# sean-lo/OptimalMatrixCompletion.jl

Measured on AMD Instinct MI355X. Metric: B&B node-relaxations/sec, 100x100 k=1, higher is better.
Workload: dtype f64

## Files before the change

### include/omc.h

```cpp
#ifndef OMC_H
#define OMC_H

#include <stdint.h>

#ifdef __cplusplus
extern "C" {
#endif

#define OMC_VERSION 100

#define OMC_OPTIMAL 0
#define OMC_SLOW_PROGRESS 1
#define OMC_TIME_LIMIT 2
#define OMC_INFEASIBLE 3

#define OMC_CUT_LINEAR 0
#define OMC_CUT_LINEAR2 1
#define OMC_CUT_LINEAR3 2
#define OMC_DIR_LEFT 0
#define OMC_DIR_MIDDLE 1
#define OMC_DIR_RIGHT 2
#define OMC_DIR_INNER_LEFT 3
#define OMC_DIR_INNER_RIGHT 4
#define OMC_SMALLEST_1_EIGVEC 1
// ... 56 lines not shown
                    double* Y, double* U, double* X, double* Theta, double* lambda_min, double* breakpoint_x,
                    double* solve_time);

int omc_relax_stage(omc_instance* h, int B, const omc_relax_params* params, int cut_type, const int* L,
                    const double* cut_x, const double* cut_Uhat, const int8_t* cut_dir, const double* U_lower,
                    const double* U_upper);
int omc_set_node_rho_scales(omc_instance* h, int B, const double* rho_scale);
int omc_relax_solve(omc_instance* h);
int omc_state_pool_create(omc_instance* h, int capacity);
int omc_state_pool_reserve_shor(omc_instance* h, int64_t nq_max);
int omc_relax_set_warm(omc_instance* h, int B, const int* load_from, const int* save_to);
int omc_shor_warm_compat(int64_t n_parent, const int64_t* parent_idx, int64_t n_soc_parent, const int64_t* parent_soc, int64_t n_child,
                         const int64_t* child_idx, int64_t n_soc_child, const int64_t* child_soc);
int omc_last_shor_warm_stats(omc_instance* h, int64_t out[4]);
int omc_state_pool_fetch_shor(omc_instance* h, int entry, int64_t* nq, double* X, double* Theta, double* V);
int omc_relax_submit(omc_instance* h);
int omc_relax_fetch_done(omc_instance* h, int max_nodes, int* node_ids, double* objective, double* dual_bound, int* status, int* iters,
                         double* U, double* lambda_min, double* breakpoint_x, double* Y, int* n_out);
int omc_relax_hold(omc_instance* h, int on);
int omc_relax_reserve(omc_instance* h, int extra_nodes, int max_cuts);
int omc_relax_append(omc_instance* h, int B, const int* L, const double* cut_x, const double* cut_Uhat, const int8_t* cut_dir,
                     const int* load_from, const int* save_to);
int omc_relax_poll(omc_instance* h, int* running, int* nodes_done, int* nodes_total);
int omc_relax_wait(omc_instance* h);
int omc_relax_fetch(omc_instance* h, double* objective, double* dual_bound, int* status, int* iters, double* Y,
                    double* U, double* X, double* Theta, double* lambda_min, double* breakpoint_x,
                    double* solve_time);

int omc_relax_stage_shor(omc_instance* h, int B, const omc_relax_params* params, int cut_type, const int* L,
                         const double* cut_x, const double* cut_Uhat, const int8_t* cut_dir, const double* U_lower,
                         const double* U_upper, const int64_t* n_shor, const int64_t* shor_idx, const int64_t* n_soc,
                         const int64_t* soc_idx);
int omc_relax_fetch_shor(omc_instance* h, double* W );
int omc_set_shor_keep_V(omc_instance* h, int keep);
int omc_relax_fetch_shor_V(omc_instance* h, double* V);
int omc_relax_batch_shor(omc_instance* h, int B, const omc_relax_params* params, int cut_type, const int* L,
                         const double* cut_x, const double* cut_Uhat, const int8_t* cut_dir, const double* U_lower,
                         const double* U_upper, const int64_t* n_shor, const int64_t* shor_idx, const int64_t* n_soc,
                         const int64_t* soc_idx, double* objective, double* dual_bound, int* status, int* iters, double* Y,
                         double* U, double* X, double* Theta, double* W, double* lambda_min, double* breakpoint_x,
                         double* solve_time);
int omc_set_shor_penalties(omc_instance* h, double rho, double r4, double r5);
int omc_relax_reserve_shor(omc_instance* h, int64_t nq_max, int extra_lists);
int omc_relax_append_shor(omc_instance* h, int B, const int* L, const double* cut_x, const double* cut_Uhat, const int8_t* cut_dir,
                          const int64_t* n_shor, const int64_t* shor_idx, const int64_t* n_soc, const int64_t* soc_idx,
                          const int* load_from, const int* save_to);
int omc_relax_fetch_done_shor(omc_instance* h, int n_ids, const int* node_ids, double* X, double* W, double* Theta);

int omc_relax_keep_certificates(omc_instance* h, int on);
int omc_relax_fetch_certificate(omc_instance* h, int n_ids, const int* node_ids, double* Lam, double* lam, int* R, double* Q, int* r,
                                double* Psi3, double* bound);
int omc_certificate_plan(int n, int k, int nnz, int max_cuts, int nonstandard_box_rows, int64_t* out);
int omc_dual_bound_batch(omc_instance* h, int B, int cut_type, int reference_quirk_q1, const int* L, const double* cut_x,
                         const double* cut_Uhat, const int8_t* cut_dir, const double* U_lower, const double* U_upper, const double* Lam,
                         const double* lam, const double* Psi3, double* Q_out, int* r_out, double* bound);

int omc_relax_keep_shor_certificates(omc_instance* h, int on);
int omc_relax_fetch_shor_certificate(omc_instance* h, int n_ids, const int* node_ids, double* scale, double* bound, double* lam, int* R, double* Q,
                                     int* r, double* Psi3, double* Gam, double* zeta, double* xi, double* Xbar, int* nq, int64_t* nq_stride);
int omc_shor_certificate_plan(int n, int m, int k, int64_t nq_stride, int max_cuts, int nonstandard_box_rows, int64_t* out);

int omc_shor_dual_bound_batch(omc_instance* h, int B, int cut_type, int reference_quirk_q1, const int* L, const double* cut_x,
                              const double* cut_Uhat, const int8_t* cut_dir, const double* U_lower, const double* U_upper, const int64_t* n_shor,
                              const int64_t* shor_idx, const int64_t* n_soc, const int64_t* soc_idx, int sanitise, int64_t nq_stride,
                              const double* scale, const double* lam, const double* Psi3, const double* Gam, const double* zeta, const double* xi,
                              const double* Xbar, double* bound, double* defects, double* terms);
int omc_shor_dual_bound_plan(int n, int m, int k, int B, int64_t nq_stride, int max_cuts, int nonstandard_box_rows, int sanitise, int64_t* out);
int omc_last_shor_dual_bound_ms(omc_instance* h, double* ms);

int omc_shor_index_build(omc_instance* h, int where, int64_t nq, const int64_t* shor_idx, int64_t n_soc, const int64_t* soc_idx, int64_t* counts,
                         double* r4, uint64_t* hash, int* mi, int* kid, int* cptr, int* cent, int* v1ptr, int* v1ent, int* v2ptr, int* v2ent,
                         int* slackrow, uint8_t* eclass, uint8_t* ctype);
int omc_shor_index_plan(int n, int m, int64_t nq, int64_t* out);
int omc_last_shor_index_stats(omc_instance* h, double* out);

int omc_altmin_batch(omc_instance* h, int B, int cut_type, int reference_quirk_q1, const int* L,
                     const double* cut_x, const double* cut_Uhat, const int8_t* cut_dir, const double* U_initial,
                     double eps, int max_iters, double time_limit, double* U, double* V, int* converged,
                     int* n_iters, double* objectives, double* solve_time);

int omc_altmin_master_objectives(omc_instance* h, int B, double* objective);
int omc_altmin_plan(int n, int m, int k, int max_cuts, int nolds, int64_t* out);

int omc_evaluate_objective(omc_instance* h, int B, const double* X, double* objective);

int omc_separation_batch(omc_instance* h, int B, int breakpoints, const double* Y, const double* U,
                         double* eigvals, double* x, int* feasible);

int omc_round_Y_batch(omc_instance* h, int B, const double* Y, double* U_rounded);
int omc_left_singular_batch(omc_instance* h, int B, const double* X, double* U_out);

int omc_psd_project_batch(omc_instance* h, int B, int N, const double* M, double lo, double hi, int algo,
                          const double* V0, double* P, double* evals, double* V);
int omc_column_prox_batch(omc_instance* h, int B, int mode, int algo, const double* Y, const double* alpha_old, const double* rho_f,
                          const double* s0, double* alpha, double* s, double* objcol, double* c0col, int* nfact);
int omc_row_project_batch(omc_instance* h, int B, int R, int Rmax, int which, const double* G, const double* c, const double* lam0,
                          double* lam, int* overflow);
int omc_colprox_plan(int n, int cmax, int block_min, int64_t* out);
int omc_last_cone_multi_stats(omc_instance* h, int64_t* out);
int omc_plain_multi_plan(int n, int plain_multi_min, int64_t* out);
double omc_plain_multi_tau(void);
int omc_last_plain_multi_stats(omc_instance* h, int64_t* out);
int omc_cone_multi_budget(int interval_max);
#define OMC_HARVEST_NONE 0
#define OMC_HARVEST_SYNC 1
#define OMC_HARVEST_ASYNC 2
int omc_harvest_plan(int nlive, int nfin, int pending, int check_index, int async_min_live);

int omc_shor_count(omc_instance* h, int n_classes, const int* num_entries_present, int64_t* count_per_class);
int omc_shor_indexes(omc_instance* h, int n_classes, const int* num_entries_present, int64_t capacity, int64_t* out,
                     int64_t* count);
int omc_violated_shor_minors(omc_instance* h, const double* X, int n_classes, const int* num_entries_present,
                             int64_t n_existing, const int64_t* existing, int n_minors, double* scores,
                             int64_t* minors, int* n_out);
int omc_shor_last_stats(omc_instance* h, double* ms, int64_t* candidates);
int omc_shor_last_select_stats(omc_instance* h, int64_t out[4]);

#define OMC_COMM_ID_BYTES 128
int omc_comm_unique_id(void* id_out);
int omc_comm_init(omc_instance* h, int rank, int world_size, const void* id);
int omc_allreduce_bounds(omc_instance* h, double* ub, double* lb, int* owner);
int omc_bcast_incumbent(omc_instance* h, int root, double* X);
int omc_allgather_records(omc_instance* h, const double* rows, int cnt, int width, double* out, int out_capacity_rows, int* counts);
int omc_comm_destroy(omc_instance* h);

#define OMC_KERNEL_COLPROX 0
#define OMC_KERNEL_CONE 1
#define OMC_KERNEL_GLOBAL 2
#define OMC_KERNEL_CHECK 3
#define OMC_KERNEL_SETUP 4
#define OMC_KERNEL_SMALL 5
#define OMC_KERNEL_ACCEL 6
#define OMC_KERNEL_CONESUB 7
#define OMC_KERNEL_CHECK_COL 8
#define OMC_KERNEL_CHECK_BUILD 9
#define OMC_KERNEL_HARVEST 10
#define OMC_KERNEL_SHOR_BIGCONE 11
#define OMC_KERNEL_SHOR_MINORS 12
#define OMC_KERNEL_SHOR_COLS 13
#define OMC_KERNEL_NCLASS 14
int omc_last_solver_info(omc_instance* h, double* info);
#define OMC_RES_CONE_SUB 0
#define OMC_RES_CONE_SUB_CERT 1
#define OMC_RES_CONE_SUB_SEP 2
#define OMC_RES_GLOBAL 3
#define OMC_RES_SMALL 4
#define OMC_RES_COLPROX_PAIR 5
#define OMC_RES_COLPROX_WIDE 6
#define OMC_RES_COLPROX 7
#define OMC_RES_CONE_WS 8
#define OMC_RES_CONE 9
#define OMC_RES_N 10
int omc_kernel_residency(omc_instance* h, int* out);
int omc_last_subspace_stats(omc_instance* h, int64_t* out);
int omc_last_shor_subspace_stats(omc_instance* h, int64_t* out);
int omc_tuning_set(omc_instance* h, const char* name, const char* value);
int omc_tuning_reload_env(omc_instance* h);
int omc_debug_stamps(omc_instance* h, double* out32);
int omc_debug_diag(omc_instance* h, double* out);
int omc_debug_aa(omc_instance* h, int* accepted, int* rejected);
int omc_debug_residuals(omc_instance* h, double* rp, double* rd);
int omc_last_kernel_stats(omc_instance* h, int64_t* launches , double* ms ,
                          int64_t* units );
#define OMC_HOST_CHECK_WAIT 0
#define OMC_HOST_CHECK_SCAN 1
#define OMC_HOST_LIST 2
#define OMC_HOST_EVENT_DRAIN 3
#define OMC_HOST_HARVEST_FLAGS 4
#define OMC_HOST_HARVEST_ENQUEUE 5
#define OMC_HOST_HARVEST_WAIT 6
#define OMC_HOST_HARVEST_BOOK 7
#define OMC_HOST_SETUP_ENQUEUE 8
#define OMC_HOST_CHECK_TOTAL 9
#define OMC_HOST_HARVEST_TOTAL 10
#define OMC_HOST_ASYNC_HARVESTS 11
#define OMC_HOST_QUIET_INTERVALS 12
#define OMC_HOST_BODY_RECORDS 13
#define OMC_HOST_BODY_WAITS 14
#define OMC_HOST_NPHASE 15
int omc_last_host_phases(omc_instance* h, double* ms , int64_t* count );

#ifdef __cplusplus
}
#endif
#endif
```

### optimalmatrixcompletion.jl_amd/_lib.py

```python
from __future__ import annotations

import ctypes as C
import os

import numpy as np

_HERE = os.path.dirname(os.path.abspath(__file__))
LIB_PATH = os.environ.get("OMC_AMD_LIB") or os.path.join(_HERE, "lib", "libomc_hip.so")

EXPORTS = [
    "omc_relax_params_default", "omc_last_error", "omc_version", "omc_device_count", "omc_instance_create",
    "omc_instance_create_bits", "omc_instance_destroy", "omc_relax_batch", "omc_relax_stage", "omc_relax_solve",
    "omc_relax_fetch", "omc_relax_submit", "omc_relax_poll", "omc_relax_wait", "omc_altmin_batch", "omc_evaluate_objective", "omc_separation_batch", "omc_round_Y_batch",
    "omc_last_kernel_stats", "omc_last_host_phases", "omc_kernel_residency", "omc_last_solver_info", "omc_last_subspace_stats", "omc_set_node_rho_scales", "omc_left_singular_batch", "omc_psd_project_batch", "omc_column_prox_batch", "omc_row_project_batch", "omc_colprox_plan", "omc_last_cone_multi_stats", "omc_cone_multi_budget", "omc_plain_multi_plan", "omc_plain_multi_tau", "omc_last_plain_multi_stats", "omc_harvest_plan", "omc_relax_reserve", "omc_relax_append", "omc_relax_fetch_done", "omc_relax_hold", "omc_debug_stamps", "omc_tuning_set", "omc_tuning_reload_env", "omc_debug_residuals", "omc_debug_diag", "omc_debug_aa",
    "omc_shor_count", "omc_shor_indexes", "omc_violated_shor_minors", "omc_shor_last_stats", "omc_shor_last_select_stats",
    "omc_relax_stage_shor", "omc_relax_fetch_shor", "omc_relax_batch_shor", "omc_set_shor_penalties", "omc_set_shor_keep_V", "omc_relax_fetch_shor_V", "omc_last_shor_subspace_stats", "omc_state_pool_create", "omc_relax_set_warm",
    "omc_state_pool_reserve_shor", "omc_shor_warm_compat", "omc_last_shor_warm_stats", "omc_state_pool_fetch_shor",
    "omc_relax_reserve_shor", "omc_relax_append_shor", "omc_relax_fetch_done_shor",
    "omc_relax_keep_certificates", "omc_relax_fetch_certificate", "omc_certificate_plan", "omc_dual_bound_batch",
    "omc_relax_keep_shor_certificates", "omc_relax_fetch_shor_certificate", "omc_shor_certificate_plan",
    "omc_shor_dual_bound_batch", "omc_shor_dual_bound_plan", "omc_last_shor_dual_bound_ms",
    "omc_shor_index_build", "omc_shor_index_plan", "omc_last_shor_index_stats",
    "omc_altmin_master_objectives", "omc_altmin_plan", "omc_comm_unique_id", "omc_comm_init", "omc_allreduce_bounds", "omc_bcast_incumbent", "omc_allgather_records", "omc_comm_destroy",
]


class RelaxParams(C.Structure):
    _fields_ = [("eps_gap", C.c_double), ("eps_feas", C.c_double), ("max_iters", C.c_int), ("check_every", C.c_int),
                ("rho_scale", C.c_double), ("rho_f_ratio", C.c_double), ("relax", C.c_double), ("time_limit", C.c_double),
                ("reference_quirk_q1", C.c_int), ("breakpoints", C.c_int), ("stall_checks", C.c_int), ("bump_max", C.c_int), ("bump_ratio", C.c_double),
                ("bump_factor", C.c_double), ("bump_after", C.c_int), ("bump_window", C.c_int), ("slots", C.c_int),
                ("accel", C.c_int), ("aa_mem", C.c_int), ("aa_every", C.c_int), ("aa_start", C.c_int), ("aa_reg", C.c_double), ("aa_safeguard", C.c_double), ("first_wins", C.c_int),
                ("early_stop_after", C.c_int), ("early_stop_factor", C.c_double)]


class OmcError(RuntimeError):
    def __init__(self, code, msg):
        super().__init__(f"libomc_hip error {code}: {msg}")
        self.code = code


_lib = None


def load():
    global _lib
    if _lib is not None:
        return _lib
    if not os.path.exists(LIB_PATH):
        raise OmcError(-100, f"{LIB_PATH} not found: build it first (__graft_entry__.build()); there is no CPU fallback")
    lib = C.CDLL(LIB_PATH)
    dp = C.POINTER(C.c_double); ip = C.POINTER(C.c_int); vp = C.c_void_p
    lib.omc_last_error.restype = C.c_char_p
    lib.omc_version.restype = C.c_int
    lib.omc_device_count.restype = C.c_int
    lib.omc_relax_params_default.argtypes = [C.POINTER(RelaxParams)]
    lib.omc_instance_create.argtypes = [C.c_int, C.c_int, C.c_int, vp, vp, C.c_double, C.c_int, C.POINTER(vp)]
    lib.omc_instance_create_bits.argtypes = [C.c_int, C.c_int, C.c_int, vp, vp, C.c_double, C.c_int, C.POINTER(vp)]
    lib.omc_instance_destroy.argtypes = [vp]
    lib.omc_instance_destroy.restype = None
    lib.omc_relax_batch.argtypes = [vp, C.c_int, C.POINTER(RelaxParams), C.c_int] + [vp] * 17
    lib.omc_relax_stage.argtypes = [vp, C.c_int, C.POINTER(RelaxParams), C.c_int] + [vp] * 6
    lib.omc_relax_solve.argtypes = [vp]
    lib.omc_relax_stage_shor.argtypes = [vp, C.c_int, C.POINTER(RelaxParams), C.c_int] + [vp] * 10
    lib.omc_relax_fetch_shor.argtypes = [vp, vp]
    lib.omc_relax_batch_shor.argtypes = [vp, C.c_int, C.POINTER(RelaxParams), C.c_int] + [vp] * 22
    lib.omc_set_shor_penalties.argtypes = [vp, C.c_double, C.c_double, C.c_double]
    lib.omc_set_shor_keep_V.argtypes = [vp, C.c_int]
    lib.omc_relax_fetch_shor_V.argtypes = [vp, vp]
    lib.omc_last_shor_subspace_stats.argtypes = [vp, vp]
    lib.omc_state_pool_create.argtypes = [vp, C.c_int]
    lib.omc_relax_set_warm.argtypes = [vp, C.c_int, vp, vp]
    lib.omc_state_pool_reserve_shor.argtypes = [vp, C.c_int64]
    lib.omc_shor_warm_compat.argtypes = [C.c_int64, vp, C.c_int64, vp, C.c_int64, vp, C.c_int64, vp]
    lib.omc_last_shor_warm_stats.argtypes = [vp, vp]
    lib.omc_state_pool_fetch_shor.argtypes = [vp, C.c_int, vp, vp, vp, vp]
    lib.omc_relax_submit.argtypes = [vp]
    lib.omc_relax_poll.argtypes = [vp, vp, vp, vp]
    lib.omc_relax_wait.argtypes = [vp]
    lib.omc_relax_fetch.argtypes = [vp] + [vp] * 11
    lib.omc_altmin_batch.argtypes = [vp, C.c_int, C.c_int, C.c_int, vp, vp, vp, vp, vp, C.c_double, C.c_int, C.c_double,
                                     vp, vp, vp, vp, vp, vp]
    lib.omc_evaluate_objective.argtypes = [vp, C.c_int, vp, vp]
    lib.omc_separation_batch.argtypes = [vp, C.c_int, C.c_int, vp, vp, vp, vp, vp]
    lib.omc_round_Y_batch.argtypes = [vp, C.c_int, vp, vp]
    lib.omc_last_kernel_stats.argtypes = [vp, vp, vp, vp]
    lib.omc_last_solver_info.argtypes = [vp, vp]
    if hasattr(lib, "omc_last_host_phases"):
        lib.omc_last_host_phases.argtypes = [vp, vp, vp]
    if hasattr(lib, "omc_kernel_residency"):
        lib.omc_kernel_residency.argtypes = [vp, vp]
    lib.omc_last_subspace_stats.argtypes = [vp, vp]
    lib.omc_set_node_rho_scales.argtypes = [vp, C.c_int, vp]
    lib.omc_debug_stamps.argtypes = [vp, vp]
    lib.omc_left_singular_batch.argtypes = [vp, C.c_int, vp, vp]
    lib.omc_psd_project_batch.argtypes = [vp, C.c_int, C.c_int, vp, C.c_double, C.c_double, C.c_int, vp, vp, vp, vp]
    if hasattr(lib, "omc_column_prox_batch"):
        lib.omc_column_prox_batch.argtypes = [vp, C.c_int, C.c_int, C.c_int] + [vp] * 9
        lib.omc_colprox_plan.argtypes = [C.c_int, C.c_int, C.c_int, vp]
    if hasattr(lib, "omc_row_project_batch"):
        lib.omc_row_project_batch.argtypes = [vp, C.c_int, C.c_int, C.c_int, C.c_int] + [vp] * 5
    lib.omc_last_cone_multi_stats.argtypes = [vp, vp]
    lib.omc_cone_multi_budget.argtypes = [C.c_int]
    if hasattr(lib, "omc_plain_multi_plan"):
        lib.omc_plain_multi_plan.argtypes = [C.c_int, C.c_int, vp]
        lib.omc_plain_multi_tau.argtypes = []
        lib.omc_plain_multi_tau.restype = C.c_double
        lib.omc_last_plain_multi_stats.argtypes = [vp, vp]
    if hasattr(lib, "omc_harvest_plan"):
        lib.omc_harvest_plan.argtypes = [C.c_int] * 5
    lib.omc_relax_reserve.argtypes = [vp, C.c_int, C.c_int]
    lib.omc_relax_hold.argtypes = [vp, C.c_int]
    lib.omc_relax_fetch_done.argtypes = [vp, C.c_int, vp, vp, vp, vp, vp, vp, vp, vp, vp, vp]
    lib.omc_relax_append.argtypes = [vp, C.c_int, vp, vp, vp, vp, vp, vp]
    lib.omc_relax_reserve_shor.argtypes = [vp, C.c_int64, C.c_int]
    lib.omc_relax_append_shor.argtypes = [vp, C.c_int] + [vp] * 10
    lib.omc_relax_fetch_done_shor.argtypes = [vp, C.c_int, vp, vp, vp, vp]
    if hasattr(lib, "omc_relax_keep_certificates"):
        lib.omc_relax_keep_certificates.argtypes = [vp, C.c_int]
        lib.omc_relax_fetch_certificate.argtypes = [vp, C.c_int] + [vp] * 8
        lib.omc_certificate_plan.argtypes = [C.c_int] * 5 + [vp]
        lib.omc_dual_bound_batch.argtypes = [vp, C.c_int, C.c_int, C.c_int] + [vp] * 12
    if hasattr(lib, "omc_relax_keep_shor_certificates"):
        lib.omc_relax_keep_shor_certificates.argtypes = [vp, C.c_int]
        lib.omc_relax_fetch_shor_certificate.argtypes = [vp, C.c_int] + [vp] * 14
        lib.omc_shor_certificate_plan.argtypes = [C.c_int, C.c_int, C.c_int, C.c_int64, C.c_int, C.c_int, vp]
    if hasattr(lib, "omc_shor_dual_bound_batch"):
        lib.omc_shor_dual_bound_batch.argtypes = [vp, C.c_int, C.c_int, C.c_int] + [vp] * 10 + [C.c_int, C.c_int64] + [vp] * 10
        lib.omc_shor_dual_bound_plan.argtypes = [C.c_int] * 4 + [C.c_int64, C.c_int, C.c_int, C.c_int, vp]
        lib.omc_last_shor_dual_bound_ms.argtypes = [vp, vp]
    if hasattr(lib, "omc_shor_index_build"):
        lib.omc_shor_index_build.argtypes = [vp, C.c_int, C.c_int64, vp, C.c_int64] + [vp] * 15
        lib.omc_shor_index_plan.argtypes = [C.c_int, C.c_int, C.c_int64, vp]
        lib.omc_last_shor_index_stats.argtypes = [vp, vp]
    lib.omc_tuning_set.argtypes = [vp, C.c_char_p, C.c_char_p]
    lib.omc_tuning_reload_env.argtypes = [vp]
    lib.omc_debug_residuals.argtypes = [vp, vp, vp]
    lib.omc_debug_diag.argtypes = [vp, vp]
    lib.omc_debug_aa.argtypes = [vp, vp, vp]
    lib.omc_shor_count.argtypes = [vp, C.c_int, vp, vp]
    lib.omc_shor_indexes.argtypes = [vp, C.c_int, vp, C.c_int64, vp, vp]
    lib.omc_violated_shor_minors.argtypes = [vp, vp, C.c_int, vp, C.c_int64, vp, C.c_int, vp, vp, vp]
    lib.omc_shor_last_stats.argtypes = [vp, vp, vp]
    lib.omc_shor_last_select_stats.argtypes = [vp, vp]
    lib.omc_altmin_master_objectives.argtypes = [vp, C.c_int, vp]
    lib.omc_altmin_plan.argtypes = [C.c_int, C.c_int, C.c_int, C.c_int, C.c_int, vp]
    lib.omc_comm_unique_id.argtypes = [vp]
    lib.omc_comm_init.argtypes = [vp, C.c_int, C.c_int, vp]
    lib.omc_allreduce_bounds.argtypes = [vp, vp, vp, vp]
    lib.omc_bcast_incumbent.argtypes = [vp, C.c_int, vp]
    lib.omc_allgather_records.argtypes = [vp, vp, C.c_int, C.c_int, vp, C.c_int, vp]
    lib.omc_comm_destroy.argtypes = [vp]
    _lib = lib
    return lib


def check(rc):
    if rc != 0:
        raise OmcError(rc, load().omc_last_error().decode("utf-8", "replace"))


def ptr(a):
    return None if a is None else a.ctypes.data_as(C.c_void_p)


def f64(a, order="F"):
    return np.require(np.asarray(a, dtype=np.float64), requirements=["ALIGNED"] + (["F_CONTIGUOUS"] if order == "F" else ["C_CONTIGUOUS"]))
```

### optimalmatrixcompletion.jl_amd/api.py

```python
from __future__ import annotations

import atexit
import weakref
import ctypes as C

import numpy as np

from . import _lib, certificate
from ._lib import RelaxParams, OmcError

CUT_TYPES = {"linear": 0, "linear2": 1, "linear3": 2}
DIR_CODES = {"left": 0, "middle": 1, "right": 2, "inner_left": 3, "inner_right": 4}
BREAKPOINTS = {"smallest_1_eigvec": 1, "smallest_2_eigvec": 2}
STATUS_NAMES = {0: "OPTIMAL", 1: "SLOW_PROGRESS", 2: "TIME_LIMIT", 3: "INFEASIBLE"}
KERNEL_CLASSES = ["colprox", "cone", "global", "check", "setup", "small", "accel", "cone_sub", "check_col", "check_build", "harvest",
                  "shor_bigcone", "shor_minors", "shor_cols"]
HOST_PHASES = ["check_wait", "check_scan", "list", "event_drain", "harvest_flags", "harvest_enqueue", "harvest_wait", "harvest_book",
               "setup_enqueue", "check_total", "harvest_total", "async_harvests", "quiet_intervals", "body_records", "body_waits"]
HOST_BODY_COUNTS = ("body_records", "body_waits")
RESIDENCY_KERNELS = ["k_cone_sub<0>", "k_cone_sub<1>", "k_cone_sub<2>", "k_global", "k_small", "k_colprox_pair", "k_colprox_wide", "k_colprox",
                     "k_cone_ws", "k_cone"]


def default_params(**kw) -> RelaxParams:
# ... 264 lines not shown

    def reserve_shor(self, nq_max, extra_lists):
        _lib.check(self._lib.omc_relax_reserve_shor(self._h, int(nq_max), int(extra_lists)))
        self._reserved_nq = int(nq_max)

    def append_shor(self, nodes, shor_info, disjunctive_cuts_type="linear", load_from=None, save_to=None):
        n, k = self.n, self.k
        if len(shor_info) != len(nodes):
            raise ValueError("one Shor_info per node")
        L, cx, cU, cd = _pack_cuts(nodes, n, k, disjunctive_cuts_type)
        lf = None if load_from is None else np.ascontiguousarray(np.asarray(load_from, dtype=np.int32))
        sv = None if save_to is None else np.ascontiguousarray(np.asarray(save_to, dtype=np.int32))
        if (lf is not None and lf.shape != (len(nodes),)) or (sv is not None and sv.shape != (len(nodes),)):
            raise ValueError("load_from / save_to must hold one pool index per node")
        nsh, nso, shi, soi = _pack_shor(shor_info)
        _lib.check(self._lib.omc_relax_append_shor(self._h, len(nodes), _lib.ptr(L), _lib.ptr(cx), _lib.ptr(cU), _lib.ptr(cd), _lib.ptr(nsh),
                                                   _lib.ptr(shi), _lib.ptr(nso), _lib.ptr(soi), _lib.ptr(lf), _lib.ptr(sv)))
        self._B += len(nodes)

    def fetch_done_shor(self, ids, want_W=False, want_Theta=False):
        n, m = self.n, self.m
        idv = np.ascontiguousarray(np.asarray(list(ids), dtype=np.int32))
        c = len(idv)
        X = np.zeros((max(c, 1), n * m)); W = np.zeros((max(c, 1), n * m)) if want_W else None; Th = np.zeros((max(c, 1), m * m)) if want_Theta else None
        _lib.check(self._lib.omc_relax_fetch_done_shor(self._h, c, _lib.ptr(idv), _lib.ptr(X), _lib.ptr(W), _lib.ptr(Th)))
        out = []
        for i in range(c):
            d = dict(node=int(idv[i]), X=X[i].reshape((n, m), order="F"))
            if want_W:
                d["W"] = W[i].reshape((n, m), order="F")
            if want_Theta:
                d["Theta"] = Th[i].reshape((m, m), order="F")
            out.append(d)
        return out

    def hold(self, on=True):
        _lib.check(self._lib.omc_relax_hold(self._h, 1 if on else 0))

    def fetch_done(self, max_nodes=4096, want_Y=False):
        n, k = self.n, self.k
        key = (int(max_nodes), bool(want_Y))
        if getattr(self, "_fd_key", None) != key:
            self._fd_key = key
            self._fd = (np.zeros(max_nodes, np.int32), np.zeros(max_nodes), np.zeros(max_nodes), np.zeros(max_nodes, np.int32), np.zeros(max_nodes, np.int32),
                        np.zeros((max_nodes, n * k)), np.zeros((max_nodes, 2)), np.zeros((max_nodes, n)), np.zeros(1, np.int32),
                        np.zeros((max_nodes, n * n)) if want_Y else None)
        ids, obj, lb, st, it, U, ev, bx, cnt, Y = self._fd
        _lib.check(self._lib.omc_relax_fetch_done(self._h, int(max_nodes), _lib.ptr(ids), _lib.ptr(obj), _lib.ptr(lb), _lib.ptr(st), _lib.ptr(it),
                                                  _lib.ptr(U), _lib.ptr(ev), _lib.ptr(bx), _lib.ptr(Y), _lib.ptr(cnt)))
        out = []
        for i in range(int(cnt[0])):
            d = dict(node=int(ids[i]), objective=float(obj[i]), dual_bound=float(lb[i]), status_code=int(st[i]), termination_status=STATUS_NAMES[int(st[i])],
                     feasible=int(st[i]) != 3, iters=int(it[i]), U=U[i].reshape((n, k), order="F").copy(), lambda_min=ev[i].copy(), breakpoint_vec=bx[i].copy())
            if want_Y:
                d["Y"] = Y[i].reshape((n, n), order="F").copy()
            out.append(d)
        return out

    def solve(self):
        _lib.check(self._lib.omc_relax_solve(self._h))

    def submit(self):
        _lib.check(self._lib.omc_relax_submit(self._h))

    def poll(self):
        r = np.zeros(3, np.int32)
        _lib.check(self._lib.omc_relax_poll(self._h, _lib.ptr(r[0:1]), _lib.ptr(r[1:2]), _lib.ptr(r[2:3])))
        return dict(running=bool(r[0]), nodes_done=int(r[1]), nodes_total=int(r[2]))

    def wait(self):
        _lib.check(self._lib.omc_relax_wait(self._h))

    def fetch(self, want_Y=True, want_X=True, want_Theta=False):
        B, n, m, k = self._B, self.n, self.m, self.k
        obj = np.zeros(B); lb = np.zeros(B); st = np.zeros(B, np.int32); it = np.zeros(B, np.int32)
        Y = np.zeros((B, n * n)) if want_Y else None
        U = np.zeros((B, n * k))
        X = np.zeros((B, n * m)) if want_X else None
        Th = np.zeros((B, m * m)) if want_Theta else None
        lmin = np.zeros((B, 2)); bx = np.zeros((B, n)); tm = np.zeros(B)
        _lib.check(self._lib.omc_relax_fetch(self._h, _lib.ptr(obj), _lib.ptr(lb), _lib.ptr(st), _lib.ptr(it), _lib.ptr(Y),
                                             _lib.ptr(U), _lib.ptr(X), _lib.ptr(Th), _lib.ptr(lmin), _lib.ptr(bx), _lib.ptr(tm)))
        out = []
        for b in range(B):
            r = {
                "objective": float(obj[b]), "dual_bound": float(lb[b]), "termination_status": STATUS_NAMES[int(st[b])],
                "status_code": int(st[b]), "feasible": int(st[b]) != 3, "iters": int(it[b]), "solve_time": float(tm[b]),
                "U": U[b].reshape((n, k), order="F"), "lambda_min": lmin[b].copy(), "breakpoint_vec": bx[b].copy(),
            }
            if want_Y: r["Y"] = Y[b].reshape((n, n), order="F")
            if want_X: r["X"] = X[b].reshape((n, m), order="F")
            if want_Theta: r["Theta"] = Th[b].reshape((m, m), order="F")
            out.append(r)
        return out

    def matrix_completion_SDP_relaxation(self, nodes, disjunctive_cuts_type="linear", params=None, U_lower=None, U_upper=None,
                                         want_Y=True, want_X=True, want_Theta=False, rho_scales=None, add_Shor_valid_inequalities=False,
                                         shor_info=None, shor_penalties=None, want_V=False, load_from=None, save_to=None):
        if add_Shor_valid_inequalities:
            if shor_info is None:
                raise ValueError("add_Shor_valid_inequalities = true needs node.Shor_info (OMC.jl:1508)")
            self.stage_shor(nodes, shor_info, disjunctive_cuts_type, params, U_lower, U_upper, shor_penalties, keep_V=(want_V and self.k == 1),
                            load_from=load_from, save_to=save_to)
            self.solve()
            out = self.fetch(want_Y, want_X, want_Theta)
            for r, Wb in zip(out, self.fetch_shor()):
                r["W"] = Wb
            if want_V and self.k == 1:
                for r, Vb, (mi, _) in zip(out, self.fetch_shor_V(), shor_info):
                    r["V"] = Vb[:len(np.asarray(mi).reshape(-1, 4))]
            elif want_V:
                for r, (mi, _) in zip(out, shor_info):
                    r.update(shor_rank_k_extension(self.k, r["X"], r["W"], mi))
            return out
        self.stage(nodes, disjunctive_cuts_type, params, U_lower, U_upper, rho_scales, load_from, save_to)
        self.solve()
        return self.fetch(want_Y, want_X, want_Theta)

    def kernel_stats(self):
        nc = len(KERNEL_CLASSES); la = np.zeros(nc, np.int64); ms = np.zeros(nc); un = np.zeros(nc, np.int64)
        _lib.check(self._lib.omc_last_kernel_stats(self._h, _lib.ptr(la), _lib.ptr(ms), _lib.ptr(un)))
        return {KERNEL_CLASSES[i]: dict(launches=int(la[i]), ms=float(ms[i]), units=int(un[i])) for i in range(nc)}

    def host_phases(self):
        if not hasattr(self._lib, "omc_last_host_phases"):
            raise OmcError(-100, "this build of the library has no omc_last_host_phases")
        ms = np.zeros(len(HOST_PHASES)); cnt = np.zeros(len(HOST_PHASES), np.int64)
        _lib.check(self._lib.omc_last_host_phases(self._h, _lib.ptr(ms), _lib.ptr(cnt)))
        return {HOST_PHASES[i]: dict(ms=float(ms[i]), count=int(cnt[i])) for i in range(len(HOST_PHASES)) if HOST_PHASES[i] not in HOST_BODY_COUNTS}

    def event_counts(self):
        if not hasattr(self._lib, "omc_last_host_phases"):
            raise OmcError(-100, "this build of the library has no omc_last_host_phases")
        ms = np.zeros(len(HOST_PHASES)); cnt = np.zeros(len(HOST_PHASES), np.int64)
        _lib.check(self._lib.omc_last_host_phases(self._h, _lib.ptr(ms), _lib.ptr(cnt)))
        return {name[len("body_"):]: int(cnt[HOST_PHASES.index(name)]) for name in HOST_BODY_COUNTS}

    def subspace_stats(self):
        out = np.zeros(8, np.int64)
        _lib.check(self._lib.omc_last_subspace_stats(self._h, _lib.ptr(out)))
        return dict(calls=int(out[0]), power_steps=int(out[1]), fallbacks=int(out[2]), seeds=int(out[3]), fail_positive=int(out[4]),
                    fail_steps=int(out[5]), fail_cholesky=int(out[6]), ritz_passes=int(out[7]))

    def shor_subspace_stats(self):
        out = np.zeros(8, np.int64)
        _lib.check(self._lib.omc_last_shor_subspace_stats(self._h, _lib.ptr(out)))
        return dict(calls=int(out[0]), power_steps=int(out[1]), fallbacks=int(out[2]), seeds=int(out[3]), fail_positive=int(out[4]),
                    fail_steps=int(out[5]), fail_cholesky=int(out[6]), ritz_passes=int(out[7]))

    def kernel_residency(self):
        out = np.zeros(len(RESIDENCY_KERNELS), np.int32)
        _lib.check(self._lib.omc_kernel_residency(self._h, _lib.ptr(out)))
        return {nm: int(v) for nm, v in zip(RESIDENCY_KERNELS, out)}

    def solver_info(self):
        info = np.zeros(8)
        _lib.check(self._lib.omc_last_solver_info(self._h, _lib.ptr(info)))
        return dict(solve_seconds=info[0], jacobi_sweeps=int(info[1]), rho=info[2], r_max=int(info[3]), cone_lds=bool(info[4]),
                    global_lds=bool(info[5]), small_lds=bool(info[6]), R_max=int(info[7]))

    def keep_certificates(self, on=True):
        _lib.check(self._lib.omc_relax_keep_certificates(self._h, 1 if on else 0))

    def certificate_plan(self, max_cuts=0, nonstandard_box_rows=0):
        return certificate_plan(self.n, self.k, int(self.indices.sum()), max_cuts, nonstandard_box_rows)

    def _support(self):
        cols, rows = np.nonzero(self.indices.T)
        return rows, cols

    def fetch_certificate(self, ids):
        n, m, k = self.n, self.m, self.k
        idv = np.ascontiguousarray(np.asarray(list(ids), dtype=np.int32))
        c = len(idv)
        info = self.solver_info()
        Rmax, rmax = max(info["R_max"], 1), max(info["r_max"], 1)
        rows, cols = self._support()
        nnz = rows.size
        ps = (rmax + k) ** 2
        Lam = np.zeros((max(c, 1), max(nnz, 1))); lam = np.zeros((max(c, 1), Rmax)); R = np.zeros(max(c, 1), np.int32)
        Q = np.zeros((max(c, 1), n * rmax)); r = np.zeros(max(c, 1), np.int32); Psi = np.zeros((max(c, 1), ps)); bd = np.zeros(max(c, 1))
        if nnz:
            Lam = np.zeros((max(c, 1), nnz))
        _lib.check(self._lib.omc_relax_fetch_certificate(self._h, c, _lib.ptr(idv), _lib.ptr(Lam), _lib.ptr(lam), _lib.ptr(R), _lib.ptr(Q),
                                                         _lib.ptr(r), _lib.ptr(Psi), _lib.ptr(bd)))
        out = []
        for i in range(c):
            ri = int(r[i]); N3 = ri + k
            dense = np.zeros((n, m)); dense[rows, cols] = Lam[i, :nnz]
            out.append(certificate.Certificate(Lam=dense, lam=lam[i, :int(R[i])].copy(), Q=Q[i, :n * ri].reshape((n, ri), order="F").copy(),
                                               Psi3=Psi[i, :N3 * N3].reshape((N3, N3), order="F").copy(), bound=float(bd[i])))
        return out

    def keep_shor_certificates(self, on=True):
        _lib.check(self._lib.omc_relax_keep_shor_certificates(self._h, 1 if on else 0))

    def shor_certificate_plan(self, nq_stride, max_cuts=0, nonstandard_box_rows=0):
        return shor_certificate_plan(self.n, self.m, self.k, nq_stride, max_cuts, nonstandard_box_rows)

    def fetch_shor_certificate(self, ids):
        n, m, k = self.n, self.m, self.k
        idv = np.ascontiguousarray(np.asarray(list(ids), dtype=np.int32))
        c = len(idv); c1 = max(c, 1)
        stride = np.zeros(1, np.int64)
        _lib.check(self._lib.omc_relax_fetch_shor_certificate(self._h, 0, None, *([None] * 12), _lib.ptr(stride)))
        ns = int(stride[0])
        info = self.solver_info()
        Rmax, rmax = max(info["R_max"], 1), max(info["r_max"], 1)
        ps = (rmax + k) ** 2
        sc = np.zeros(c1); bd = np.zeros(c1); lam = np.zeros((c1, Rmax)); R = np.zeros(c1, np.int32); Q = np.zeros((c1, n * rmax)); r = np.zeros(c1, np.int32)
        Psi = np.zeros((c1, ps)); Gam = np.zeros((c1, 15 * max(ns, 1))); zeta = np.zeros((c1, m)); xi = np.zeros((c1, n * m)); Xb = np.zeros((c1, n * m))
        nq = np.zeros(c1, np.int32)
        _lib.check(self._lib.omc_relax_fetch_shor_certificate(self._h, c, _lib.ptr(idv), _lib.ptr(sc), _lib.ptr(bd), _lib.ptr(lam), _lib.ptr(R), _lib.ptr(Q),
                                                              _lib.ptr(r), _lib.ptr(Psi), _lib.ptr(Gam) if ns else None, _lib.ptr(zeta), _lib.ptr(xi), _lib.ptr(Xb),
                                                              _lib.ptr(nq), None))
        out = []
        for i in range(c):
            ri = int(r[i]); N3 = ri + k
            G = certificate.unpack_gam(Gam[i, :15 * ns].reshape(15, ns), int(nq[i])) if ns else np.zeros((0, 5, 5))
            out.append(certificate.ShorCertificate(scale=float(sc[i]), lam=lam[i, :int(R[i])].copy(), Q=Q[i, :n * ri].reshape((n, ri), order="F").copy(),
                                                   Psi3=Psi[i, :N3 * N3].reshape((N3, N3), order="F").copy(), Gam=G, zeta=zeta[i].copy(),
                                                   xi=xi[i].reshape((n, m), order="F").copy(), Xbar=Xb[i].reshape((n, m), order="F").copy(),
                                                   bound=float(bd[i])))
        return out

    def _bounds_flat(self, B, U_lower, U_upper):
        lo = hi = None
        if U_lower is not None:
            lo = np.ascontiguousarray(np.stack([np.asfortranarray(np.asarray(u, float)).ravel(order="F") for u in U_lower]))
        if U_upper is not None:
            hi = np.ascontiguousarray(np.stack([np.asfortranarray(np.asarray(u, float)).ravel(order="F") for u in U_upper]))
        for a in (lo, hi):
            if a is not None and a.shape != (B, self.n * self.k):
                raise ValueError("U_lower / U_upper: one (n, k) matrix per node")
        return lo, hi

    def row_basis(self, nodes, disjunctive_cuts_type="linear", U_lower=None, U_upper=None, reference_quirk_q1=True):
        n, k, B = self.n, self.k, len(nodes)
        L, cx, cU, cd = _pack_cuts(nodes, n, k, disjunctive_cuts_type)
        lo, hi = self._bounds_flat(B, U_lower, U_upper)
        args = (self._h, B, CUT_TYPES[disjunctive_cuts_type], int(bool(reference_quirk_q1)), _lib.ptr(L), _lib.ptr(cx), _lib.ptr(cU), _lib.ptr(cd),
                _lib.ptr(lo), _lib.ptr(hi), None, None, None)
        r = np.zeros(B, np.int32)
        _lib.check(self._lib.omc_dual_bound_batch(*args, None, _lib.ptr(r), None))
        rmax = max(1, int(r.max()))
        Q = np.zeros((B, n * rmax))
        _lib.check(self._lib.omc_dual_bound_batch(*args, _lib.ptr(Q), _lib.ptr(r), None))
        return [Q[b, :n * int(r[b])].reshape((n, int(r[b])), order="F").copy() for b in range(B)]

    def dual_bound(self, nodes, certs, disjunctive_cuts_type="linear", U_lower=None, U_upper=None, reference_quirk_q1=True):
        n, m, k, B = self.n, self.m, self.k, len(nodes)
        if len(certs) != B:
            raise ValueError("one certificate per node")
        L, cx, cU, cd = _pack_cuts(nodes, n, k, disjunctive_cuts_type)
        lo, hi = self._bounds_flat(B, U_lower, U_upper)
        dlo, dhi = certificate.default_U_bounds(n, k)
        Rb = []
        for b in range(B):
            lb_ = dlo if lo is None else lo[b]; hb_ = dhi if hi is None else hi[b]
            Rb.append(1 + int((np.asarray(lb_) > -1.0).sum()) + int((np.asarray(hb_) < 1.0).sum()) + int(L[b]) * (2 * k + 1))
        rb = [int(np.asarray(c.Q).shape[1]) for c in certs]
        Rmax, rmax = max(Rb), max(1, max(rb))
        rows, cols = self._support()
        nnz = rows.size
        ps = (rmax + k) ** 2
        Lam = np.zeros((B, max(nnz, 1))); lam = np.zeros((B, Rmax)); Psi = np.zeros((B, ps))
        for b, c in enumerate(certs):
            if np.asarray(c.Lam).shape != (n, m) or len(c.lam) != Rb[b] or np.asarray(c.Psi3).shape != (rb[b] + k, rb[b] + k):
                raise ValueError(f"certificate {b}: Lam must be n x m, lam hold {Rb[b]} multipliers and Psi3 be of order r + k")
            Lam[b, :nnz] = np.asarray(c.Lam, float)[rows, cols]; lam[b, :Rb[b]] = c.lam
            Psi[b, :(rb[b] + k) ** 2] = np.asarray(c.Psi3, float).ravel(order="F")
        r = np.zeros(B, np.int32); bd = np.zeros(B)
        _lib.check(self._lib.omc_dual_bound_batch(self._h, B, CUT_TYPES[disjunctive_cuts_type], int(bool(reference_quirk_q1)), _lib.ptr(L), _lib.ptr(cx),
                                                  _lib.ptr(cU), _lib.ptr(cd), _lib.ptr(lo), _lib.ptr(hi), None, None, None, None, _lib.ptr(r), None))
        if [int(v) for v in r] != rb:
            raise ValueError(f"Q of the certificates has {rb} columns, the library's row basis {[int(v) for v in r]}: build Psi3 in the basis of row_basis()")
        _lib.check(self._lib.omc_dual_bound_batch(self._h, B, CUT_TYPES[disjunctive_cuts_type], int(bool(reference_quirk_q1)), _lib.ptr(L), _lib.ptr(cx),
                                                  _lib.ptr(cU), _lib.ptr(cd), _lib.ptr(lo), _lib.ptr(hi), _lib.ptr(Lam), _lib.ptr(lam), _lib.ptr(Psi),
                                                  None, None, _lib.ptr(bd)))
        return bd

    def shor_dual_bound(self, nodes, shor_info, certs, disjunctive_cuts_type="linear", U_lower=None, U_upper=None, reference_quirk_q1=True,
                        sanitise=True, want_defects=False, want_terms=False, nq_stride=None):
        if not hasattr(self._lib, "omc_shor_dual_bound_batch"):
            raise _lib.OmcError(-100, "this libomc_hip.so has no omc_shor_dual_bound_batch")
        n, m, k, B = self.n, self.m, self.k, len(nodes)
        if len(certs) != B or len(shor_info) != B:
            raise ValueError("one certificate and one (minors, SOC list) pair per node")
        L, cx, cU, cd = _pack_cuts(nodes, n, k, disjunctive_cuts_type)
        lo, hi = self._bounds_flat(B, U_lower, U_upper)
        nsh, nso, shi, soi = _pack_shor(shor_info)
        dlo, dhi = certificate.default_U_bounds(n, k)
        Rb = []
        for b in range(B):
            lb_ = dlo if lo is None else lo[b]; hb_ = dhi if hi is None else hi[b]
            Rb.append(1 + int((np.asarray(lb_) > -1.0).sum()) + int((np.asarray(hb_) < 1.0).sum()) + int(L[b]) * (2 * k + 1))
        rb = [int(np.asarray(c.Q).shape[1]) for c in certs]
        Rmax, rmax = max(Rb), max(1, max(rb))
        ns = int(nsh.max()) if nq_stride is None else int(nq_stride)
        ps = (rmax + k) ** 2
        sc = np.zeros(B); lam = np.zeros((B, Rmax)); Psi = np.zeros((B, ps)); Gam = np.zeros((B, 15, max(ns, 1)))
        zeta = np.zeros((B, m)); xi = np.zeros((B, n * m)); Xb = np.zeros((B, n * m))
        for b, c in enumerate(certs):
            G = np.asarray(c.Gam, float).reshape(-1, 5, 5)
            if len(c.lam) != Rb[b] or np.asarray(c.Psi3).shape != (rb[b] + k, rb[b] + k) or len(G) != int(nsh[b]):
                raise ValueError(f"certificate {b}: lam must hold {Rb[b]} multipliers, Psi3 be of order r + k and Gam hold {int(nsh[b])} blocks")
# ... 286 lines not shown
```

### optimalmatrixcompletion.jl_amd/csrc/omc_api.cpp

```cpp
#include <hip/hip_runtime.h>
#include <stdint.h>
#include <limits.h>
#include <stdio.h>
#include <stdlib.h>
#include <string.h>
#include <math.h>
#include <string>
#include <vector>
#include <algorithm>
#include <atomic>
#include <thread>
#include <mutex>
#include <execinfo.h>
#include <signal.h>
#include <unistd.h>

#include "omc_altmin.h"
#include "omc_api_internal.h"

thread_local std::string g_err;

static void knob_set(Tuning& t, const Knob& kb, const char* value) {
  if (kb.flag) t.*kb.flag = value != nullptr;
  else t.*kb.num = value ? atoi(value) : Tuning{}.*kb.num;
// ... 382 lines not shown
  if (!(w.rho > 0.0)) w.rho = 1.0;
  w.clip_hi = 1.0; w.inv_s2 = 1.0; w.shor = 0;
  w.rho_f_ratio = P.rho_f_ratio;
  w.bump_max = P.bump_max; w.bump_ratio = P.bump_ratio; w.bump_factor = P.bump_factor; w.bump_after = P.bump_after;
  w.bump_gap = P.bump_window * std::max(1, P.check_every);
  w.accel = P.accel ? 1 : 0; w.aa_mem = std::max(2, std::min(P.aa_mem, AA_MAXMEM)); w.aa_every = std::max(1, P.aa_every);
  w.aa_start = std::max(2, P.aa_start); w.aa_reg = P.aa_reg; w.aa_safeguard = P.aa_safeguard;
  {
    std::vector<double> hr((size_t)B + extra_nodes, w.rho);
    if (h->rho_scale_per_node.size() == (size_t)B)
      for (int b = 0; b < B; ++b) hr[b] = w.rho / P.rho_scale * h->rho_scale_per_node[b];
    h->rho_scale_per_node.clear();
    int r0 = upload(h->brhon, hr.data(), sizeof(double) * hr.size(), h->stream); if (r0) return r0;
    HIPCHK(hipStreamSynchronize(h->stream));
    w.rho_node = h->brhon.as<double>();
    BIND(h->brho, w.rho_b, (size_t)S);
  }
  w.relax = P.relax; w.eps_gap = P.eps_gap; w.eps_feas = P.eps_feas;
  w.check_every = std::max(1, P.check_every); w.early_stop_after = P.early_stop_after; w.early_stop_factor = (P.first_wins ? 0.0 : P.early_stop_factor);
  const StageDims sd = {(size_t)S, (size_t)B + (size_t)extra_nodes, (size_t)n, (size_t)m, (size_t)k, (size_t)h->nnz, (size_t)rmax, (size_t)Rmax};
  {
    ENS_CARVE(h->bgap, [&](Carve& c) { walk_gap(c, sd, w); });
    BIND(h->bvotes, w.slow_votes, (size_t)S);
    ENS(h->bslotlist, sizeof(int) * (size_t)S);
    w.slot_list = nullptr;
  }
  std::vector<double> wY((size_t)n * n);
  for (size_t e = 0; e < (size_t)n * n; ++e) wY[e] = shor ? 3.0 : P.rho_f_ratio * h->Ncnt[e] + 2.0;
  int rc_ = 0;
  if ((rc_ = upload(h->dwY, wY.data(), sizeof(double) * n * n, h->stream))) return rc_;
  w.col_ptr = h->dcol_ptr.as<int>(); w.col_idx = h->dcol_idx.as<int>(); w.col_val = h->dcol_val.as<double>();
  {
    const bool pair_on = !h->tun.no_colprox_pair && mode.colprox_force != 2;
    if ((rc_ = build_colprox_lists(h, mode.colprox_force == 1 ? INT_MAX : mode.colprox_force == 2 ? 1 : h->tun.colprox_block_min, pair_on))) return rc_;
    w.cp_pair = pair_on ? 1 : 0;
  }
  w.cp_nblock = h->nblock; w.cp_block = h->nblock ? h->dblock.as<int>() : nullptr;
  w.cp_nslab = h->nslab; w.cp_slab = h->nslab ? h->dslab.as<int>() : nullptr;
  w.cp_isblock = (h->nblock + h->nslab) ? h->disblock.as<unsigned char>() : nullptr; w.cp_nrest = h->nrest; w.cp_nfact = nullptr;
  w.cone_512 = h->tun.cone_512 ? 1 : 0; w.cp_series = CP_SERIES; w.cp_maxpass = CP_MAXPASS; w.cp_xcd = h->tun.colprox_no_xcd ? 0 : 1;
  w.cp_dpp = h->tun.colprox_dpp ? 1 : 0;
  w.cp_nsolo = h->nsolo; w.cp_solo = h->nsolo ? h->dsolo.as<int>() : nullptr;
  w.cp_nwide = h->nwide; w.cp_wide = h->nwide ? h->dwide.as<int>() : nullptr;
  w.Ncnt = h->dNcnt.as<double>(); w.wY1 = h->dwY.as<double>();
  w.row_ptr = h->drow_ptr.as<int>(); w.row_idx = h->drow_idx.as<int>();
  const size_t sB = (size_t)S;
  const size_t sN = (size_t)B + (size_t)extra_nodes;
  hipStream_t s0 = h->stream;
  const size_t nn = (size_t)n * n, nk = (size_t)n * k, nz = (size_t)h->nnz;
  BIND(h->bY, w.Y, sB * nn); BIND(h->bYp, w.Yp, sB * nn); BIND(h->bU, w.U, sB * nk);
  BIND(h->bD1, w.D1, sB * nn); BIND(h->bD3, w.D3, sB * nn); BIND(h->bW1, w.W1, sB * nn); BIND(h->bE3, w.E3, sB * nn);
  BIND(h->bdS, w.dS, sB * rmax * rmax);
  ENS_CARVE(h->bsm, [&](Carve& c) { walk_small_cone(c, sd, w); });
  BIND(h->balpha, w.alpha, sB * nz); BIND(h->balphaX, w.alphaX, sB * nz); BIND(h->bsval, w.sval, sB * m);
  BIND(h->bMchk, w.Mchk, sB * nn);
  size_t chk_bytes = 0;
  ENS_CARVE(h->bchk, [&](Carve& c) { walk_check(c, sd, w); }, &chk_bytes);
  BIND(h->bG, w.G, sB * Rmax * Rmax); BIND(h->blam, w.lam, sB * Rmax);
  ENS_CARVE(h->bscal, [&](Carve& c) { walk_scalars(c, sd, w); });
  BIND(h->bbx, w.bx, sB * n);
  ENS_CARVE(h->bint, [&](Carve& c) { walk_slot_ints(c, sd, w); });
  w.np16 = (n + 15) & ~15;
  const size_t pp = (size_t)w.np16 * w.np16, p16 = (size_t)w.np16 * 16;
  BIND(h->bMbuf, w.Mbuf, sB * pp); BIND(h->bVrow, w.Vrow, sB * pp);
  BIND(h->blamD, w.lamD, sB * m * n, s0);
  w.lamDX = nullptr;
  if (n > 144 || shor) BIND(h->blamDX, w.lamDX, sB * m * n, s0);
  {
    size_t subS_bytes = 0, subI_bytes = 0;
    BIND(h->bXs, w.Xs, sB * p16, s0);
    ENS_CARVE(h->bsubS, [&](Carve& c) { walk_sub_doubles(c, sd, w); }, &subS_bytes);
    ENS_CARVE(h->bsubI, [&](Carve& c) { walk_sub_ints(c, sd, w); }, &subI_bytes);
    HIPCHK(hipMemsetAsync(h->bsubS.p, 0, subS_bytes, s0));
    HIPCHK(hipMemsetAsync(h->bsubI.p, 0, subI_bytes, s0));
    w.ws_phase = 0;
    w.sub_guard = SUB_GUARD; w.sub_qmax = h->tun.sub_qmax; w.sub_chunk = SUB_CHUNK;
    w.sub_tol = SUB_TOL; w.sub_adapt = SUB_ADAPT; w.sub_debug = h->tun.sub_debug;
    w.sub_enable = 0;
    size_t subSC_bytes = 0, subIC_bytes = 0;
    BIND(h->bXsC, w.XsC, sB * p16, s0);
    ENS_CARVE(h->bsubSC, [&](Carve& c) { walk_subC_doubles(c, sd, w); }, &subSC_bytes);
    ENS_CARVE(h->bsubIC, [&](Carve& c) { walk_subC_ints(c, sd, w); }, &subIC_bytes);
    HIPCHK(hipMemsetAsync(h->bsubSC.p, 0, subSC_bytes, s0));
    HIPCHK(hipMemsetAsync(h->bsubIC.p, 0, subIC_bytes, s0));
    w.cert_enable = 0;
  }
  BIND(h->bMbufC, w.MbufC, sB * pp, s0); BIND(h->bVrowC, w.VrowC, sB * pp, s0); BIND(h->bchkS, w.fro2c, sB); BIND(h->bchkI, w.vvalidC, sB, s0);
  w.Yx = nullptr;
  if (!shor && !P.accel) BIND(h->bYx, w.Yx, sB * nn);
  w.skip_yp = (w.Yx && !h->tun.dense_proj) ? 1 : 0;
  ENS_CARVE(h->bobjcol, [&](Carve& c) { walk_objcol(c, sd, w); });
  if (w.accel) {
    w.aa_dim = 4 * n * n + 2 * rmax * k + k * k + h->nnz;
    const size_t ring = sB * (size_t)(w.aa_mem + 1) * w.aa_dim;
    size_t aaI_bytes = 0;
    BIND(h->baaF, w.aa_F, ring); BIND(h->baaG, w.aa_G, ring); BIND(h->baaZ, w.aa_zin, sB * (size_t)w.aa_dim); BIND(h->baaS, w.aa_fn, sB);
    ENS_CARVE(h->baaI, [&](Carve& c) { walk_aa_ints(c, sd, w); }, &aaI_bytes);
    HIPCHK(hipMemsetAsync(h->baaI.p, 0, aaI_bytes, s0));
  }
  HIPCHK(hipMemsetAsync(w.ws_need, 0, sizeof(int), s0));
  {
    size_t map_bytes = 0;
    ENS_CARVE(h->bslotint, [&](Carve& c) { walk_slot_map(c, sd, w.node_of, w.init, w.fin); }, &map_bytes);
    std::vector<int> hs(map_bytes / sizeof(int));
    int *h_node = nullptr, *h_init = nullptr, *h_fin = nullptr;
    { Carve hc(hs.data()); walk_slot_map(hc, sd, h_node, h_init, h_fin); }
    for (size_t b = 0; b < sB; ++b) { h_node[b] = (int)b; h_init[b] = 1; h_fin[b] = 1; }
    HIPCHK(hipMemcpyAsync(h->bslotint.p, hs.data(), map_bytes, hipMemcpyHostToDevice, h->stream));
    HIPCHK(hipStreamSynchronize(h->stream));
    BIND(h->boY, w.oY, sN * nn); BIND(h->boU, w.oU, sN * nk); BIND(h->boal, w.oalphaX, sN * nz); BIND(h->bobx, w.obx, sN * n);
    ENS_CARVE(h->boscal, [&](Carve& c) { walk_out_scalars(c, sd, w); });
    ENS_CARVE(h->boint, [&](Carve& c) { walk_out_ints(c, sd, w); });
  }
  if ((h->keep_cert && !shor) || (h->keep_shor_cert && shor)) {
    const size_t cnnz = shor ? 0 : (size_t)h->nnz;
    size_t cbD_bytes = 0, cbI_bytes = 0, ocD_bytes = 0;
    ENS_CARVE(h->bcbD, [&](Carve& c) { walk_cert_slot(c, sd, cnnz, w); }, &cbD_bytes);
    ENS_CARVE(h->bcbI, [&](Carve& c) { walk_cert_flags(c, sd, w); }, &cbI_bytes);
    ENS_CARVE(h->bocD, [&](Carve& c) { walk_cert_node(c, sd, cnnz, w); }, &ocD_bytes);
    BIND(h->bocI, w.ocHave, sN, s0);
    HIPCHK(hipMemsetAsync(h->bcbD.p, 0, cbD_bytes, s0)); HIPCHK(hipMemsetAsync(h->bcbI.p, 0, cbI_bytes, s0));
    HIPCHK(hipMemsetAsync(h->bocD.p, 0, ocD_bytes, s0));
    if (shor) { w.cbLam = nullptr; w.ocLam = nullptr; }
  }
  w.load_from = nullptr; w.save_to = nullptr;
  const bool warm_ok = !shor || mode.warm_filtered;
  if (h->pool_cap > 0 && warm_ok && extra_nodes > 0) {
    if (h->warm_load.size() != (size_t)B) h->warm_load.assign(B, -1);
    if (h->warm_save.size() != (size_t)B) h->warm_save.assign(B, -1);
    h->warm_load.resize(sN, -1); h->warm_save.resize(sN, -1);
  } else if (extra_nodes == 0) {
    if (h->warm_load.size() != (size_t)B) h->warm_load.clear();
    if (h->warm_save.size() != (size_t)B) h->warm_save.clear();
  }
  h->save_host.assign(sN, -1);
  if (h->pool_cap > 0 && !shor && h->warm_load.size() == sN) {
    std::lock_guard<std::mutex> lk(h->sig_mu);
    for (int& e : h->warm_load) if (e >= 0 && (size_t)e < h->pool_sig.size() && h->pool_sig[e].kind == 2) e = -1;
  }
  if (h->pool_cap > 0 && warm_ok && (h->warm_load.size() == sN || h->warm_save.size() == sN)) {
    if (h->warm_save.size() == sN) h->save_host = h->warm_save;
    if (h->warm_load.size() == sN) { if ((rc_ = upload(h->bwarmL, h->warm_load.data(), sizeof(int) * sN, h->stream))) return rc_; w.load_from = h->bwarmL.as<int>(); }
    if (h->warm_save.size() == sN) { if ((rc_ = upload(h->bwarmS, h->warm_save.data(), sizeof(int) * sN, h->stream))) return rc_; w.save_to = h->bwarmS.as<int>(); }
    HIPCHK(hipStreamSynchronize(h->stream));
    w.pY = h->pY.as<double>(); w.pD1 = h->pD1.as<double>(); w.pD3 = h->pD3.as<double>(); w.pU = h->pU.as<double>(); w.palpha = h->palpha.as<double>();
    w.psval = h->psval.as<double>(); w.pXs = h->pXs.as<double>(); w.ptheta = h->ptheta.as<double>(); w.pscal = h->pscal.as<double>();
  }
  h->warm_load.clear(); h->warm_save.clear();
  BIND(h->bQb, w.Qb, sN * n * rmax); BIND(h->brr, w.rr, sN); BIND(h->bR, w.R, sN);
  BIND(h->brkind, w.rkind, sN * Rmax); BIND(h->brcut, w.rcut, sN * Rmax); BIND(h->brbi, w.rbi, sN * Rmax); BIND(h->brbj, w.rbj, sN * Rmax);
  BIND(h->brcoef, w.rcoef, sN * Rmax * k); BIND(h->brrhs, w.rrhs, sN * Rmax); BIND(h->bcutx, w.cutx, sN * w.Lmax * n);
  if ((rc_ = put_descriptors(w, pk, B, sN, 0, L, cut_x, h->stream))) return rc_;
  w.geo = omc_plan_geometry(n, w.np16, k, rmax, Rmax, h->cmax, h->tun.global_nolds, h->tun.cone_multi_min, h->tun.plain_multi_min);
  BIND(h->bmwstat, w.mw_stat, sB * 4, s0);
  w.mw_budget = MAX_SWEEPS; w.ev_out = nullptr;
  w.pmw_stat = nullptr;
  if (w.geo.plain_mw) BIND(h->bpmwstat, w.pmw_stat, sB * 4, s0);
  geom_set_cpblock(w.geo, h->cpb_cl, h->cpb_cs);
  w.geo.cp_scratch_stride = h->crest_max > w.geo.cp_lds_c ? cp_body_layout(h->crest_max).doubles : 0;
  if (w.geo.cpb_slab_stride && !shor) BIND(h->bcpb, w.cp_bslab, sB * h->nslab * w.geo.cpb_slab_stride);
  if (w.geo.cp_scratch_stride) BIND(h->bcp, w.cp_scratch, sB * m * w.geo.cp_scratch_stride);
  if (w.geo.ws.slab_stride) BIND(h->bcone, w.cone_scratch, sB * w.geo.ws.slab_stride);
  if (w.geo.glob.slab_stride) BIND(h->bglob, w.glob_scratch, sB * w.geo.glob.slab_stride);
  if (w.geo.small.slab_stride) BIND(h->bsmall, w.small_scratch, sB * w.geo.small.slab_stride);
  w.sub_enable = (w.geo.ws_lpp && n >= 48 && w.geo.sub_lds <= OMC_MAX_DYN_LDS && !h->tun.no_subspace) ? 1 : 0;
  w.sub_zscratch = nullptr;
  if (w.sub_enable && w.np16 > 512) BIND(h->bsubz, w.sub_zscratch, sB * 16 * (size_t)(w.np16 + 2));
  w.cert_enable = (w.sub_enable && w.np16 > 512) ? 1 : 0;
  if (!w.sub_enable) w.sep_done = nullptr;
  if (!(!shor && w.sub_enable && w.geo.glob.use_lds && glob_w1_fits(n) && !h->tun.dense_proj)) w.w1_fac = nullptr;
  HIPCHK(hipMemsetAsync(w.sweeps, 0, sizeof(int) * S, s0));
  HIPCHK(hipMemsetAsync(w.stamps, 0, (size_t)((char*)h->bchk.p + chk_bytes - (char*)w.stamps), s0));
  HIPCHK(hipStreamSynchronize(h->stream));
  h->staged = true;
  return 0;
}

int omc_relax_stage(omc_instance* h, int B, const omc_relax_params* params, int cut_type, const int* L,
                    const double* cut_x, const double* cut_Uhat, const int8_t* cut_dir, const double* U_lower,
                    const double* U_upper) {
  return stage_base(h, B, params, cut_type, L, cut_x, cut_Uhat, cut_dir, U_lower, U_upper, StageMode{});
}

int omc_set_node_rho_scales(omc_instance* h, int B, const double* rho_scale) {
  if (!h || B <= 0 || !rho_scale) return fail(OMC_ERR_ARGUMENT, "NULL argument");
  for (int b = 0; b < B; ++b) if (!(rho_scale[b] > 0.0)) return fail(OMC_ERR_ARGUMENT, "rho_scale must be positive");
  h->rho_scale_per_node.assign(rho_scale, rho_scale + B);
  return 0;
}

int omc_state_pool_create(omc_instance* h, int capacity) {
  if (!h) return fail(OMC_ERR_ARGUMENT, "handle is NULL");
  if (capacity < 0) return fail(OMC_ERR_ARGUMENT, "capacity must be non-negative");
  HIPCHK(hipSetDevice(h->device));
  const size_t c = (size_t)capacity, n = h->n, k = h->k, np16 = (h->n + 15) & ~15;
  if (capacity > 0) {
    ENS(h->pY, c * n * n * 8); ENS(h->pD1, c * n * n * 8); ENS(h->pD3, c * n * n * 8); ENS(h->pU, c * n * k * 8); ENS(h->palpha, c * (size_t)h->nnz * 8);
    ENS(h->psval, c * (size_t)h->m * 8); ENS(h->pXs, c * np16 * 16 * 8); ENS(h->ptheta, c * 16 * 8); ENS(h->pscal, c * 4 * 8);
  }
  h->pool_cap = capacity;
  { std::lock_guard<std::mutex> lk(h->sig_mu); h->pool_sig.assign(c, omc_instance::PoolSig{}); }
  h->pool_shor = false; h->pool_nqmax = 0;
  return 0;
}

int omc_relax_set_warm(omc_instance* h, int B, const int* load_from, const int* save_to) {
  if (!h || B <= 0) return fail(OMC_ERR_ARGUMENT, "omc_relax_set_warm: bad arguments");
  if (h->pool_cap <= 0) return fail(OMC_ERR_ARGUMENT, "omc_relax_set_warm: no state pool (omc_state_pool_create)");
  h->warm_load.clear(); h->warm_save.clear();
  for (int b = 0; b < B; ++b) {
    if (load_from && load_from[b] >= h->pool_cap) return fail(OMC_ERR_ARGUMENT, "load_from index beyond the pool");
    if (save_to && save_to[b] >= h->pool_cap) return fail(OMC_ERR_ARGUMENT, "save_to index beyond the pool");
  }
  if (load_from) h->warm_load.assign(load_from, load_from + B);
  if (save_to) h->warm_save.assign(save_to, save_to + B);
  return 0;
}

int omc_relax_reserve(omc_instance* h, int extra_nodes, int max_cuts) {
  if (!h) return fail(OMC_ERR_ARGUMENT, "handle is NULL");
  if (extra_nodes < 0 || max_cuts < 0) return fail(OMC_ERR_ARGUMENT, "omc_relax_reserve: negative argument");
  h->reserve_nodes = extra_nodes; h->reserve_cuts = max_cuts;
  return 0;
}

int append_nodes(omc_instance* h, const char* who, int B2, const int* L, const double* cut_x, const double* cut_Uhat, const int8_t* cut_dir,
                 const int* load_from, const int* save_to, const ShorAppendLists* lists) {
  const std::string pre = std::string(who) + ": ";
  HIPCHK(hipSetDevice(h->device));
  std::lock_guard<std::mutex> lk(h->append_mu);
  if (h->append_closed) return fail(OMC_ERR_ARGUMENT, pre + "the solve of this batch has ended (stage a new batch)");
  const OmcWS& w = h->ws;
  const int first = h->Btot_live.load();
  if (first + B2 > h->node_cap) return fail(OMC_ERR_ARGUMENT, pre + (lists ? "beyond the node capacity given to omc_relax_reserve" : "beyond the capacity given to omc_relax_reserve"));
  NodePack pk;
  { int rcp = pack_nodes(h, h->params, h->staged_cut_type, B2, L, cut_x, cut_Uhat, cut_dir, nullptr, nullptr, pk); if (rcp) return rcp; }
  if (pk.Rmax > w.Rmax || pk.rmax > w.rmax || pk.Lmax > w.Lmax) return fail(OMC_ERR_ARGUMENT, pre + "a node has more cuts than omc_relax_reserve allowed for");
  if ((load_from || save_to) && !(w.load_from && w.save_to))
    return fail(OMC_ERR_ARGUMENT, pre + (lists ? "warm-start indices need a state pool with its Shor extension (omc_state_pool_reserve_shor) before the batch was staged"
                                               : "warm-start indices need a state pool created before the batch was staged"));
  for (int b = 0; b < B2; ++b) {
    if (load_from && load_from[b] >= h->pool_cap) return fail(OMC_ERR_ARGUMENT, "load_from index beyond the pool");
    if (save_to && save_to[b] >= h->pool_cap) return fail(OMC_ERR_ARGUMENT, "save_to index beyond the pool");
  }
  std::vector<int> lfv, svv;
  ShorGrouping grouping;
  if (!h->append_stream) HIPCHK(hipStreamCreateWithFlags(&h->append_stream, hipStreamNonBlocking));
  if (lists) {
    if (w.load_from && w.save_to) {
      lfv.assign(B2, -1); svv.assign(B2, -1);
      if (load_from) lfv.assign(load_from, load_from + B2);
      if (save_to) svv.assign(save_to, save_to + B2);
    }
    int rcl = shor_append_plan(h, first, B2, *lists, lfv, svv, grouping); if (rcl) return rcl;
  } else {
    if (load_from) {
      lfv.assign(load_from, load_from + B2);
      std::lock_guard<std::mutex> lk2(h->sig_mu);
      for (int& e : lfv) if (e >= 0 && (size_t)e < h->pool_sig.size() && h->pool_sig[e].kind == 2) e = -1;
    }
    if (save_to) svv.assign(save_to, save_to + B2);
  }
  hipStream_t as = h->append_stream;
  const size_t f = (size_t)first;
  ShorGroupImages img;
  if (lists) { int rcw = shor_append_write(h, grouping, first, as, img); if (rcw) return rcw; }
  { int rc = put_descriptors(w, pk, B2, B2, f, L, cut_x, as); if (rc) return rc; }
  std::vector<double> hrho(B2, w.rho);
  HIPCHK(hipMemcpyAsync(const_cast<double*>(w.rho_node) + f, hrho.data(), 8 * (size_t)B2, hipMemcpyHostToDevice, as));
  if (!lfv.empty()) HIPCHK(hipMemcpyAsync(const_cast<int*>(w.load_from) + f, lfv.data(), sizeof(int) * B2, hipMemcpyHostToDevice, as));
  if (!svv.empty()) {
    HIPCHK(hipMemcpyAsync(const_cast<int*>(w.save_to) + f, svv.data(), sizeof(int) * B2, hipMemcpyHostToDevice, as));
    for (int b = 0; b < B2; ++b) h->save_host[f + b] = svv[b];
  }
  HIPCHK(hipStreamSynchronize(as));
  if (lists) shor_append_commit(h, grouping);
  h->Btot_live.store(first + B2); h->Btot = first + B2;
  if (!h->worker_running.load()) { h->ws.Btot = first + B2; if (lists) h->sh.Btot = first + B2; }
  return 0;
}

int omc_relax_append(omc_instance* h, int B2, const int* L, const double* cut_x, const double* cut_Uhat, const int8_t* cut_dir,
                     const int* load_from, const int* save_to) {
  if (!h || !h->staged) return fail(OMC_ERR_ARGUMENT, "omc_relax_append: nothing staged");
  if (B2 <= 0) return fail(OMC_ERR_ARGUMENT, "B must be positive");
  if (h->shor_on) return fail(OMC_ERR_UNSUPPORTED, "omc_relax_append: the staged batch is in Shor mode (omc_relax_append_shor)");
  return append_nodes(h, "omc_relax_append", B2, L, cut_x, cut_Uhat, cut_dir, load_from, save_to, nullptr);
}

int omc_relax_hold(omc_instance* h, int on) {
  if (!h) return fail(OMC_ERR_ARGUMENT, "handle is NULL");
  h->hold.store(on ? 1 : 0);
  return 0;
}

int omc_relax_fetch_done(omc_instance* h, int max_nodes, int* node_ids, double* objective, double* dual_bound, int* status, int* iters,
                         double* U, double* lambda_min, double* breakpoint_x, double* Y, int* n_out) {
  if (!h || !h->staged || !node_ids || !n_out) return fail(OMC_ERR_ARGUMENT, "omc_relax_fetch_done: nothing staged or NULL argument");
  if (max_nodes < 0) return fail(OMC_ERR_ARGUMENT, "max_nodes is negative");
  HIPCHK(hipSetDevice(h->device));
  std::vector<int> ids;
  {
    std::lock_guard<std::mutex> lk(h->done_mu);
    const size_t avail = h->done_q.size() - h->done_read, take = std::min(avail, (size_t)max_nodes);
    ids.assign(h->done_q.begin() + h->done_read, h->done_q.begin() + h->done_read + take);
    h->done_read += take;
// ... 29 lines not shown
  for (size_t i = 0; i < upto; ++i) if ((size_t)h->done_q[i] < seen.size()) seen[h->done_q[i]] = 1;
  for (int i = 0; i < n_ids; ++i)
    if (ids[i] < 0 || (size_t)ids[i] >= seen.size() || !seen[ids[i]])
      return fail(OMC_ERR_ARGUMENT, std::string(who) + ": node " + std::to_string(ids[i]) +
                                        (upto_read_only ? " is out of range or has not been returned by omc_relax_fetch_done"
                                                        : " is out of range or has not finished (omc_relax_fetch_done has not returned it)"));
  return 0;
}

int require_certificates(const OmcWS& w, int n_ids, const int* ids, hipStream_t fs, const char* who) {
  std::vector<int> have(n_ids, 0);
  for (int i = 0; i < n_ids; ++i) HIPCHK(hipMemcpyAsync(&have[i], w.ocHave + ids[i], sizeof(int), hipMemcpyDeviceToHost, fs));
  HIPCHK(hipStreamSynchronize(fs));
  for (int i = 0; i < n_ids; ++i)
    if (!have[i]) return fail(OMC_ERR_ARGUMENT, std::string(who) + ": node " + std::to_string(ids[i]) + " never reached a rigorous check (no certificate)");
  return 0;
}

int omc_relax_submit(omc_instance* h) {
  if (!h || !h->staged) return fail(OMC_ERR_ARGUMENT, "omc_relax_submit: nothing staged");
  if (h->worker.joinable()) return fail(OMC_ERR_ARGUMENT, "omc_relax_submit: a solve is already in flight (call omc_relax_wait first)");
  h->nodes_done.store(0); h->worker_running.store(1); h->worker_rc = 0; h->worker_err.clear();
  h->worker = std::thread([h]() {
    const int rc = omc_relax_solve(h);
    h->worker_rc = rc;
    if (rc) h->worker_err = g_err;
    h->worker_running.store(0);
  });
  return 0;
}

int omc_relax_poll(omc_instance* h, int* running, int* nodes_done, int* nodes_total) {
  if (!h) return fail(OMC_ERR_ARGUMENT, "handle is NULL");
  if (running) *running = h->worker_running.load();
  if (nodes_done) *nodes_done = h->nodes_done.load();
  if (nodes_total) *nodes_total = h->Btot_live.load();
  return 0;
}

int omc_relax_wait(omc_instance* h) {
  if (!h) return fail(OMC_ERR_ARGUMENT, "handle is NULL");
  if (!h->worker.joinable()) return fail(OMC_ERR_ARGUMENT, "omc_relax_wait: no solve in flight");
  h->worker.join();
  if (h->worker_rc) g_err = h->worker_err;
  return h->worker_rc;
}

int omc_relax_fetch(omc_instance* h, double* objective, double* dual_bound, int* status, int* iters, double* Y,
                    double* U, double* X, double* Theta, double* lambda_min, double* breakpoint_x, double* solve_time) {
  if (!h || !h->staged) return fail(OMC_ERR_ARGUMENT, "omc_relax_fetch: nothing staged");
  HIPCHK(hipSetDevice(h->device));
  const OmcWS& w = h->ws;
  const size_t B = w.Btot, n = w.n, m = w.m, k = w.k;
  hipStream_t s = h->stream;
  if (objective) HIPCHK(hipMemcpyAsync(objective, w.oobj, 8 * B, hipMemcpyDeviceToHost, s));
  if (dual_bound) HIPCHK(hipMemcpyAsync(dual_bound, w.olb, 8 * B, hipMemcpyDeviceToHost, s));
  if (status) HIPCHK(hipMemcpyAsync(status, w.ostatus, 4 * B, hipMemcpyDeviceToHost, s));
  if (iters) HIPCHK(hipMemcpyAsync(iters, w.oiters, 4 * B, hipMemcpyDeviceToHost, s));
  if (Y) HIPCHK(hipMemcpyAsync(Y, w.oY, 8 * B * n * n, hipMemcpyDeviceToHost, s));
  if (U) HIPCHK(hipMemcpyAsync(U, w.oU, 8 * B * n * k, hipMemcpyDeviceToHost, s));
  if (lambda_min) HIPCHK(hipMemcpyAsync(lambda_min, w.olmin, 8 * 2 * B, hipMemcpyDeviceToHost, s));
  if (breakpoint_x) HIPCHK(hipMemcpyAsync(breakpoint_x, w.obx, 8 * B * n, hipMemcpyDeviceToHost, s));
  if (h->shor_on) {
    if (X) HIPCHK(hipMemcpyAsync(X, h->sh.oX, 8 * B * n * m, hipMemcpyDeviceToHost, s));
    if (Theta) HIPCHK(hipMemcpyAsync(Theta, h->sh.oTh, 8 * B * m * m, hipMemcpyDeviceToHost, s));
  } else if (X || Theta) {
    double *dX = nullptr, *dTh = nullptr;
    BIND(h->bXout, dX, B * n * m);
    omc_launch_make_X(&w, dX, s);
    if (X) HIPCHK(hipMemcpyAsync(X, dX, 8 * B * n * m, hipMemcpyDeviceToHost, s));
    if (Theta) {
      BIND(h->bThout, dTh, B * m * m);
      omc_launch_make_Theta(&w, dX, dTh, s);
      HIPCHK(hipMemcpyAsync(Theta, dTh, 8 * B * m * m, hipMemcpyDeviceToHost, s));
    }
  }
  HIPCHK(hipStreamSynchronize(s));
  if (solve_time) for (size_t b = 0; b < B; ++b) solve_time[b] = h->last_solve_seconds;
  return 0;
}

int omc_relax_batch(omc_instance* h, int B, const omc_relax_params* params, int cut_type, const int* L,
                    const double* cut_x, const double* cut_Uhat, const int8_t* cut_dir, const double* U_lower,
                    const double* U_upper, double* objective, double* dual_bound, int* status, int* iters, double* Y,
                    double* U, double* X, double* Theta, double* lambda_min, double* breakpoint_x, double* solve_time) {
  int rc = omc_relax_stage(h, B, params, cut_type, L, cut_x, cut_Uhat, cut_dir, U_lower, U_upper);
  if (rc) return rc;
  rc = omc_relax_solve(h);
  if (rc) return rc;
  return omc_relax_fetch(h, objective, dual_bound, status, iters, Y, U, X, Theta, lambda_min, breakpoint_x, solve_time);
}

int omc_debug_residuals(omc_instance* h, double* rp, double* rd) {
  if (!h || !rp || !rd || !h->ws.rp) return fail(OMC_ERR_ARGUMENT, "nothing staged");
  HIPCHK(hipMemcpy(rp, h->ws.rp, 8 * (size_t)h->ws.B, hipMemcpyDeviceToHost));
  HIPCHK(hipMemcpy(rd, h->ws.rd, 8 * (size_t)h->ws.B, hipMemcpyDeviceToHost));
  return 0;
}

int omc_tuning_set(omc_instance* h, const char* name, const char* value) {
  if (!h || !name) return fail(OMC_ERR_ARGUMENT, "omc_tuning_set: handle or name is NULL");
  for (const Knob& kb : OMC_KNOBS) if (!strcmp(kb.name, name)) { knob_set(h->tun, kb, value); return 0; }
  return fail(OMC_ERR_ARGUMENT, "omc_tuning_set: unknown knob");
}

int omc_tuning_reload_env(omc_instance* h) {
  if (!h) return fail(OMC_ERR_ARGUMENT, "handle is NULL");
  tuning_from_env(h->tun);
  return 0;
}

int omc_debug_stamps(omc_instance* h, double* out32) {
  if (!h || !out32 || !h->ws.stamps) return fail(OMC_ERR_ARGUMENT, "no stamps");
  if (h->tun.sub_debug == 3 && h->ws.B >= 8) {
    HIPCHK(hipMemcpy(out32, h->ws.stamps, 96 * 8, hipMemcpyDeviceToHost));
    return 0;
  }
  HIPCHK(hipMemcpy(out32, h->ws.stamps, 32 * 8, hipMemcpyDeviceToHost));
  return 0;
}

int omc_debug_aa(omc_instance* h, int* accepted, int* rejected) {
  if (!h || !accepted || !rejected || !h->ws.accel || !h->ws.aa_nacc) return fail(OMC_ERR_ARGUMENT, "acceleration is off or nothing staged");
  HIPCHK(hipMemcpy(accepted, h->ws.aa_nacc, 4 * (size_t)h->ws.B, hipMemcpyDeviceToHost));
  HIPCHK(hipMemcpy(rejected, h->ws.aa_nrej, 4 * (size_t)h->ws.B, hipMemcpyDeviceToHost));
  return 0;
}

int omc_debug_diag(omc_instance* h, double* out ) {
  if (!h || !out || !h->ws.stamps) return fail(OMC_ERR_ARGUMENT, "no diagnostics");
  HIPCHK(hipMemcpy(out, h->ws.stamps + 32, 8 * 8 * (size_t)h->ws.B, hipMemcpyDeviceToHost));
  return 0;
}

int omc_last_host_phases(omc_instance* h, double* ms, int64_t* count) {
  if (!h || !ms || !count) return fail(OMC_ERR_ARGUMENT, "NULL argument");
  for (int q = 0; q < OMC_HOST_NPHASE; ++q) { ms[q] = h->host_ms[q]; count[q] = h->host_cnt[q]; }
  return 0;
}

int omc_last_solver_info(omc_instance* h, double* info) {
  if (!h || !info) return fail(OMC_ERR_ARGUMENT, "NULL argument");
  info[0] = h->last_solve_seconds; info[1] = (double)h->total_sweeps; info[2] = h->ws.rho; info[3] = (double)h->ws.rmax;
  info[4] = (double)h->ws.geo.cone.use_lds; info[5] = (double)h->ws.geo.glob.use_lds; info[6] = (double)h->ws.geo.small.use_lds; info[7] = (double)h->ws.Rmax;
  return 0;
}

int omc_last_subspace_stats(omc_instance* h, int64_t* out) {
  if (!h || !out) return fail(OMC_ERR_ARGUMENT, "NULL argument");
  for (int q = 0; q < 8; ++q) out[q] = h->sub_tot[q];
  return 0;
}

int omc_kernel_residency(omc_instance* h, int* out) {
  if (!h || !out) return fail(OMC_ERR_ARGUMENT, "NULL argument");
  if (!h->ws.geo.sub_lds) return fail(OMC_ERR_ARGUMENT, "omc_kernel_residency: nothing staged yet (the geometry is planned by omc_relax_stage)");
  HIPCHK(hipSetDevice(h->device));
  omc_query_residency(&h->ws, out);
  return 0;
}

int omc_last_kernel_stats(omc_instance* h, int64_t* launches, double* ms, int64_t* units) {
  if (!h) return fail(OMC_ERR_ARGUMENT, "handle is NULL");
  for (int c = 0; c < OMC_KERNEL_NCLASS; ++c) {
    if (launches) launches[c] = h->launches[c];
    if (ms) ms[c] = h->ms[c];
    if (units) units[c] = h->units[c];
  }
  return 0;
}
```

### optimalmatrixcompletion.jl_amd/csrc/omc_api_shor.cpp

```cpp
#include <hip/hip_runtime.h>
#include <stdint.h>
#include <string.h>
#include <math.h>
#include <algorithm>
#include <string>
#include <vector>

#include "omc_api_internal.h"
#include <chrono>
#include <mutex>
#include <unordered_map>

#include "omc_shor_relax.h"
#include "omc_shor_index.h"

static uint64_t fnv1a(const void* p, size_t bytes, uint64_t hsh) {
  const uint8_t* c = (const uint8_t*)p;
  for (size_t e = 0; e < bytes; ++e) { hsh ^= c[e]; hsh *= 1099511628211ull; }
  return hsh;
}
static constexpr uint64_t FNV_SEED = 1469598103934665603ull;

static int shor_warm_rule(int64_t n_parent, int64_t n_soc_parent, int64_t n_child, int64_t n_soc_child, bool same_head, bool same_soc) {
  if (n_parent < 0 || n_child < 0 || n_parent > n_child || !same_head) return 0;
// ... 456 lines not shown
    HIPCHK(back(mi, w.mi, 16 * q)); HIPCHK(back(kid, w.kid, 16 * q)); HIPCHK(back(cptr, w.cptr, 4 * (nm + 1))); HIPCHK(back(cent, w.cent, 16 * q));
    HIPCHK(back(v1ptr, w.v1ptr, 4 * ((size_t)G.nv1 + 1))); HIPCHK(back(v1ent, w.v1ent, 8 * q));
    HIPCHK(back(v2ptr, w.v2ptr, 4 * ((size_t)G.nv2 + 1))); HIPCHK(back(v2ent, w.v2ent, 8 * q));
    HIPCHK(back(slackrow, w.slackrow, 4 * m)); HIPCHK(back(eclass, w.eclass, nm)); HIPCHK(back(ctype, w.ctype, m));
    HIPCHK(hipStreamSynchronize(s));
  }
  if (counts) { counts[0] = G.nq; counts[1] = G.nv1; counts[2] = G.nv2; counts[3] = where == 1 ? (int64_t)h->shidx_stats[4] : 0; }
  if (r4) *r4 = G.r4;
  if (hash) *hash = G.hash;
  return 0;
}

int omc_relax_stage_shor(omc_instance* h, int B, const omc_relax_params* params, int cut_type, const int* L, const double* cut_x,
                         const double* cut_Uhat, const int8_t* cut_dir, const double* U_lower, const double* U_upper,
                         const int64_t* n_shor, const int64_t* shor_idx, const int64_t* n_soc, const int64_t* soc_idx) {
  if (!h) return fail(OMC_ERR_ARGUMENT, "handle is NULL");
  if (B <= 0) return fail(OMC_ERR_ARGUMENT, "B must be positive");
  if (!n_shor || !n_soc) return fail(OMC_ERR_ARGUMENT, "n_shor / n_soc is NULL");
  if (h->keep_shor_cert && h->k > 1)
    return fail(OMC_ERR_UNSUPPORTED, "omc_relax_stage_shor: Shor-mode certificates are kept (omc_relax_keep_shor_certificates) and rank k > 1 has no certificate layout (its minors are vacuous, quirk Q5)");
  if (h->keep_cert && !h->keep_shor_cert) return fail(OMC_ERR_UNSUPPORTED, "omc_relax_stage_shor: certificates are kept (omc_relax_keep_certificates) and the Shor-mode bound has multipliers the certificate layout does not hold");
  const int n = h->n, m = h->m;
  if ((long long)n * m >= (1ll << 30)) return fail(OMC_ERR_UNSUPPORTED, "Shor mode: n * m too large for the 32-bit index structures");
  ShorGrouping grp;
  { int rc0 = shor_list_offsets(B, n_shor, shor_idx, n_soc, soc_idx, grp.so, grp.co); if (rc0) return rc0; }
  for (int q = 0; q < 5; ++q) h->shidx_stats[q] = 0.0;
  h->sh_index_min = h->k == 1 ? std::max(h->tun.shor_index_device_min, 0) : 0;
  if (h->sh_index_min > 0) {
    HIPCHK(hipSetDevice(h->device));
    grp.index_min = h->sh_index_min; grp.stream = h->stream;
    if (h->reserve_shor_set) {
      int64_t nq_all = h->reserve_shor_nq;
      for (int b = 0; b < B; ++b) nq_all = std::max(nq_all, n_shor[b]);
      grp.room_nq = (size_t)nq_all;
      grp.room_ints = (size_t)h->reserve_shor_lists * shor_stage_ints((size_t)nq_all, (size_t)n * m, (size_t)m);
      grp.room_bytes = (size_t)h->reserve_shor_lists * shor_stage_bytes((size_t)n * m, (size_t)m);
      if (grp.room_ints) { int rcr = shor_index_room(h, grp.room_nq, grp.room_ints, grp.room_bytes, true); if (rcr) return rcr; }
    }
  }
  { int rc0 = group_shor_lists(h, B, n_shor, shor_idx, n_soc, soc_idx, nullptr, grp); if (rc0) return rc0; }
  const std::vector<size_t>& so = grp.so; const std::vector<size_t>& co = grp.co;
  const std::vector<ShorGroupHost>& gh = grp.groups; const std::vector<int>& node_group = grp.node_group;
  const int NG = (int)gh.size();
  int nqmax = grp.nqmax, nv1max = grp.nv1max, nv2max = grp.nv2max;
  const size_t tot_int = grp.tot_int, tot_byte = grp.tot_byte;
  const bool res_set = h->reserve_shor_set; const int64_t res_nq = res_set ? h->reserve_shor_nq : 0; const int res_lists = res_set ? h->reserve_shor_lists : 0;
  h->reserve_shor_set = false; h->reserve_shor_nq = 0; h->reserve_shor_lists = 0;
  if (h->k > 1) {
    bool all_free = true;
    for (int g = 0; g < NG && all_free; ++g) for (int j = 0; j < m; ++j) if (gh[g].ctype[j] != 0) { all_free = false; break; }
    if (all_free && !h->tun.shor_explicit) {
      h->warm_load.clear(); h->warm_save.clear();
      int rc0 = omc_relax_stage(h, B, params, cut_type, L, cut_x, cut_Uhat, cut_dir, U_lower, U_upper);
      if (rc0) return rc0;
      h->shor_via_base = true;
      h->shor_slackrow = gh[0].slackrow;
      return 0;
    }
  }
  for (int q = 0; q < 4; ++q) h->shor_warm_stats[q] = 0;
  StageMode mode;
  mode.shor = true;
  const int extra_nodes = h->reserve_nodes;
  if (h->pool_cap > 0 && h->pool_shor && h->k == 1 && (h->warm_load.size() == (size_t)B || h->warm_save.size() == (size_t)B || extra_nodes > 0)) {
    std::lock_guard<std::mutex> lk(h->sig_mu);
    h->node_sig.assign((size_t)B + (size_t)extra_nodes, omc_instance::PoolSig{});
    for (int b = 0; b < B; ++b) {
      omc_instance::PoolSig& sg = h->node_sig[b];
      sg.kind = 2; sg.nq = n_shor[b]; sg.nsoc = n_soc[b]; sg.hlist = gh[node_group[b]].hash;
      sg.hsoc = n_soc[b] > 0 ? fnv1a(soc_idx + 2 * co[b], 16 * (size_t)n_soc[b], FNV_SEED) : 0;
      shor_warm_filter(h, sg, shor_idx + 4 * so[b], h->warm_load.size() == (size_t)B ? &h->warm_load[b] : nullptr,
                       h->warm_save.size() == (size_t)B ? &h->warm_save[b] : nullptr);
    }
    mode.warm_filtered = true;
  } else {
    h->warm_load.clear(); h->warm_save.clear();
  }
  int rc = stage_base(h, B, params, cut_type, L, cut_x, cut_Uhat, cut_dir, U_lower, U_upper, mode);
  if (rc) return rc;
  h->staged = false;
  OmcWS& w = h->ws;
  const int S = w.B, N = n + m;
  hipStream_t s = h->stream;
  if (res_set) {
    nqmax = (int)std::max<int64_t>(nqmax, res_nq);
    nv1max = std::max(nv1max, 2 * nqmax); nv2max = std::max(nv2max, 2 * nqmax);
  }
  const size_t int_cap = tot_int + (size_t)res_lists * shor_stage_ints((size_t)res_nq, (size_t)n * m, (size_t)m);
  const size_t byte_cap = tot_byte + (size_t)res_lists * shor_stage_bytes((size_t)n * m, (size_t)m);
  ShWS& sh = h->sh;
  memset(&sh, 0, sizeof(sh));
  {
    int *arena_int = nullptr, *node_group_dev = nullptr; uint8_t* arena_byte = nullptr; ShorGroupDev* groups_dev = nullptr;
    BIND(h->sgInts, arena_int, int_cap); BIND(h->sgBytes, arena_byte, byte_cap);
    BIND(h->sgGroups, groups_dev, (size_t)NG + (size_t)res_lists); BIND(h->sgNodeGroup, node_group_dev, (size_t)h->node_cap);
    sh.groups = groups_dev; sh.node_group = node_group_dev;
    ShorGroupImages img;
    if ((rc = upload_shor_groups(h, grp, arena_int, arena_byte, groups_dev, node_group_dev, s, img))) return rc;
    HIPCHK(hipStreamSynchronize(s));
  }
  h->sh_byhash = std::move(grp.byhash); h->sh_lists = std::move(grp.lists);
  h->sh_group_cap = NG + res_lists; h->sh_int_used = tot_int; h->sh_int_cap = int_cap; h->sh_byte_used = tot_byte; h->sh_byte_cap = byte_cap;
  const double sc = shor_scale(h);
  {
    std::vector<double> Ah((size_t)n * m);
    for (size_t e = 0; e < Ah.size(); ++e) Ah[e] = h->A[e] * sc;
    if ((rc = upload(h->sAh, Ah.data(), 8 * Ah.size(), s))) return rc;
    HIPCHK(hipStreamSynchronize(s));
  }
  const size_t sB = (size_t)S, sN = (size_t)h->node_cap, nm = (size_t)n * m;
  const int NPb = (N + 15) & ~15;
  const int nmb = std::max(1, (nqmax + 255) / 256);
  const size_t nq1 = (size_t)std::max(nqmax, 1), nv11 = (size_t)std::max(nv1max, 1), nv21 = (size_t)std::max(nv2max, 1);
  BIND(h->sX, sh.X, sB * nm); BIND(h->sW, sh.W, sB * nm); BIND(h->sTh, sh.Th, sB * m * m);
  BIND(h->sV1, sh.V1, sB * nv11); BIND(h->sV2, sh.V2, sB * nv21); BIND(h->sV3, sh.V3, sB * nq1);
  BIND(h->sD0, sh.D0, sB * N * N); BIND(h->sP0, sh.P0, sB * N * N); BIND(h->sMbufB, sh.MbufB, sB * NPb * NPb, s); BIND(h->sVrowB, sh.VrowB, sB * NPb * NPb, s);
  BIND(h->sTq, sh.Tq, sB * 15 * nq1); BIND(h->sPq, sh.Pq, sB * 15 * nq1); BIND(h->sNq, sh.Nq, sB * 15 * nq1);
  BIND(h->sD5x, sh.D5x, sB * nm); BIND(h->sD5t, sh.D5t, sB * m); BIND(h->snu5, sh.nu5, sB * m); BIND(h->sP5x, sh.P5x, sB * nm);
  BIND(h->scolpart, sh.colpart, sB * m * 4); BIND(h->sminpart, sh.minpart, sB * nmb, s); BIND(h->sminpart2, sh.minpart2, sB * nmb, s);
  ENS_CARVE(h->sfroB, [&](Carve& c) { walk_shor_fro(c, sB, sh); }); BIND(h->svvB, sh.vvalidB, sB); BIND(h->se1, sh.e1, sB * nv11); BIND(h->se2, sh.e2, sB * nv21);
  BIND(h->soX, sh.oX, sN * nm, s); BIND(h->soW, sh.oW, sN * nm, s); BIND(h->soTh, sh.oTh, sN * m * m, s);
  sh.n = n; sh.m = m; sh.k = h->k; sh.N = N; sh.NPb = NPb; sh.S = S; sh.Btot = B; sh.nqmax = nqmax; sh.nv1max = nv1max; sh.nv2max = nv2max; sh.nmb = nmb;
  sh.rx = w.relax; sh.r4 = h->shor_r4; sh.r5 = h->shor_r5; sh.gamma = h->gamma; sh.sc = sc;
  sh.node_of = w.node_of; sh.done = w.done; sh.init = w.init; sh.fin = w.fin; sh.rho_b = w.rho_b; sh.bfac = w.bfac;
  sh.Ah = h->sAh.as<double>(); sh.mask = h->dmask.as<uint8_t>();
  sh.Y = w.Y; sh.Yp = w.Yp; sh.rp = w.rp; sh.rd = w.rd;
  sh.objcol = w.objcol; sh.c0col = w.c0col; sh.lamDX = w.lamDX;
  sh.oV = nullptr;
  if (w.load_from || w.save_to) {
    const ShorPoolLayout PL = shor_pool_layout(n, m, (int)h->pool_nqmax);
    sh.load_from = w.load_from; sh.save_to = w.save_to; sh.pscal = w.pscal; sh.pY = w.pY; sh.rho_node = w.rho_node;
    sh.pS = h->pShor.as<double>(); sh.pShdr = h->pShorHdr.as<long long>(); sh.pstride = PL.stride; sh.pnq = (int)h->pool_nqmax;
    BIND(h->sloadpart, sh.loadpart, sB * NPb * 2);
  }
  if (h->keep_shor_cert) {
    size_t cb_bytes = 0, oc_bytes = 0;
    if (carve_ensure(h->scbD, [&](Carve& c) { walk_shor_cert(c, sB, nq1, m, nm, sh.cbGam, sh.cbZeta, sh.cbXi, sh.cbXbar); }, &cb_bytes) ||
        carve_ensure(h->socD, [&](Carve& c) { walk_shor_cert(c, sN, nq1, m, nm, sh.ocGam, sh.ocZeta, sh.ocXi, sh.ocXbar); }, &oc_bytes) ||
        bind(h->socNq, sh.ocNq, sN)) {
      (void)hipGetLastError();
      return fail(OMC_ERR_ALLOC, "omc_relax_stage_shor: the Shor-mode certificates need " + std::to_string(cb_bytes / sB) + " bytes per slot (" + std::to_string(S) +
                                 ") and per node of the capacity (" + std::to_string(h->node_cap) + "), which the device does not have (" + g_err + ")");
    }
    HIPCHK(hipMemsetAsync(h->scbD.p, 0, cb_bytes, s)); HIPCHK(hipMemsetAsync(h->socD.p, 0, oc_bytes, s)); HIPCHK(hipMemsetAsync(sh.ocNq, 0, sN * sizeof(int), s));
    sh.cert_flag = w.cert_flag; sh.cb_rho = w.cb_rho;
  }
  if (h->shor_keep_V) BIND(h->soV, sh.oV, sN * 5 * nq1, s);
  w.shor = 1; w.shN = N; w.shP0 = sh.P0; w.shD0 = sh.D0; w.inv_s2 = 1.0 / (sc * sc);
  OmcWS& wb = h->wbig;
  wb = w;
  wb.n = N; wb.np16 = NPb; wb.Mbuf = sh.MbufB; wb.Vrow = sh.VrowB; wb.vvalid = sh.vvalidB; wb.fro2 = sh.fro2B; wb.W1 = sh.P0;
  wb.sub_enable = 0; wb.cert_enable = 0; wb.ws_mode = 0; wb.clip_hi = 1e300; wb.sub_debug = 0; wb.ws_first = nullptr; wb.ws_need = nullptr; wb.ws_phase = 0;
  wb.geo = omc_plan_geometry(N, NPb, wb.k, wb.rmax, wb.Rmax, h->cmax, h->tun.global_nolds, h->tun.cone_multi_min, MW_MAX_ORDER + 1);
  BIND(h->sbigmw, wb.mw_stat, sB * 4, s);
  if (wb.geo.ws.slab_stride) BIND(h->sbigscr, wb.cone_scratch, sB * wb.geo.ws.slab_stride);
  wb.trM = sh.trB;
  if (wb.geo.ws_lpp && N >= 48 && wb.geo.sub_lds <= OMC_MAX_DYN_LDS && !h->tun.no_subspace && !h->tun.shor_no_subspace) {
    size_t subI_bytes = 0;
    BIND(h->sXsB, wb.Xs, sB * NPb * 16, s); BIND(h->ssubSB, wb.sub_theta, sB * 16, s);
    ENS_CARVE(h->ssubIB, [&](Carve& c) { walk_shor_sub_ints(c, sB, sh, wb); }, &subI_bytes);
    HIPCHK(hipMemsetAsync(h->ssubIB.p, 0, subI_bytes, s));
    wb.sub_enable = 1;
    wb.sub_zscratch = nullptr;
    if (NPb > 512) BIND(h->bsubz, wb.sub_zscratch, sB * 16 * (size_t)(NPb + 2));
    wb.ws_first = nullptr; wb.ws_need = nullptr; wb.ws_phase = 0; wb.sub_on = sh.sub_onB; wb.cone_done = sh.cone_doneB; wb.sub_wait = sh.sub_waitB; wb.sub_nfail = sh.sub_nfailB;
    wb.sep_done = nullptr;
  }
  HIPCHK(hipStreamSynchronize(s));
  h->shor_on = true;
  h->staged = true;
  return 0;
}

int omc_set_shor_keep_V(omc_instance* h, int keep) {
  if (!h) return fail(OMC_ERR_ARGUMENT, "handle is NULL");
  h->shor_keep_V = keep != 0;
  return 0;
}

int omc_relax_fetch_shor_V(omc_instance* h, double* V) {
  if (!h || !h->staged || !h->shor_on) return fail(OMC_ERR_ARGUMENT, "omc_relax_fetch_shor_V: no Shor-mode batch staged");
  if (!h->sh.oV) return fail(OMC_ERR_ARGUMENT, "omc_relax_fetch_shor_V: V was not kept (call omc_set_shor_keep_V(h, 1) before staging)");
  if (!V) return fail(OMC_ERR_ARGUMENT, "V is NULL");
  HIPCHK(hipSetDevice(h->device));
  HIPCHK(hipMemcpyAsync(V, h->sh.oV, 8 * (size_t)h->sh.Btot * 5 * (size_t)std::max(h->sh.nqmax, 1), hipMemcpyDeviceToHost, h->stream));
  HIPCHK(hipStreamSynchronize(h->stream));
  return 0;
}

int omc_last_shor_subspace_stats(omc_instance* h, int64_t* out) {
  if (!h || !out) return fail(OMC_ERR_ARGUMENT, "NULL argument");
  for (int q = 0; q < 8; ++q) out[q] = h->big_sub_tot[q];
  return 0;
}

int omc_relax_fetch_shor(omc_instance* h, double* W) {
  if (h && h->staged && h->shor_via_base) {
    if (!W) return 0;
    const size_t B = h->ws.Btot, n = h->n, m = h->m;
    std::vector<double> X(B * n * m), Th(B * m * m);
    int rc = omc_relax_fetch(h, nullptr, nullptr, nullptr, nullptr, nullptr, nullptr, X.data(), Th.data(), nullptr, nullptr, nullptr);
    if (rc) return rc;
    for (size_t b = 0; b < B; ++b)
      for (size_t j = 0; j < m; ++j) {
        double s2 = 0.0;
        for (size_t i = 0; i < n; ++i) { const double x = X[(b * m + j) * n + i]; W[(b * m + j) * n + i] = x * x; s2 += x * x; }
        W[(b * m + j) * n + h->shor_slackrow[j]] += Th[(b * m + j) * m + j] - s2;
      }
    return 0;
  }
  if (!h || !h->staged || !h->shor_on) return fail(OMC_ERR_ARGUMENT, "omc_relax_fetch_shor: no Shor-mode batch staged");
  HIPCHK(hipSetDevice(h->device));
  if (W) HIPCHK(hipMemcpyAsync(W, h->sh.oW, 8 * (size_t)h->sh.Btot * h->n * h->m, hipMemcpyDeviceToHost, h->stream));
  HIPCHK(hipStreamSynchronize(h->stream));
  return 0;
}

int omc_relax_batch_shor(omc_instance* h, int B, const omc_relax_params* params, int cut_type, const int* L, const double* cut_x,
                         const double* cut_Uhat, const int8_t* cut_dir, const double* U_lower, const double* U_upper,
                         const int64_t* n_shor, const int64_t* shor_idx, const int64_t* n_soc, const int64_t* soc_idx, double* objective,
                         double* dual_bound, int* status, int* iters, double* Y, double* U, double* X, double* Theta, double* W,
                         double* lambda_min, double* breakpoint_x, double* solve_time) {
  int rc = omc_relax_stage_shor(h, B, params, cut_type, L, cut_x, cut_Uhat, cut_dir, U_lower, U_upper, n_shor, shor_idx, n_soc, soc_idx);
  if (rc) return rc;
  rc = omc_relax_solve(h);
  if (rc) return rc;
  rc = omc_relax_fetch(h, objective, dual_bound, status, iters, Y, U, X, Theta, lambda_min, breakpoint_x, solve_time);
  if (rc) return rc;
  return omc_relax_fetch_shor(h, W);
}

int omc_relax_append_shor(omc_instance* h, int B2, const int* L, const double* cut_x, const double* cut_Uhat, const int8_t* cut_dir,
                          const int64_t* n_shor, const int64_t* shor_idx, const int64_t* n_soc, const int64_t* soc_idx,
                          const int* load_from, const int* save_to) {
  if (!h) return fail(OMC_ERR_ARGUMENT, "handle is NULL");
  if (h->k > 1) return fail(OMC_ERR_UNSUPPORTED, "omc_relax_append_shor: rank k > 1 is not supported (a batch served by the base engine takes omc_relax_append)");
  if (!h->staged) return fail(OMC_ERR_ARGUMENT, "omc_relax_append_shor: nothing staged");
  if (!h->shor_on) return fail(OMC_ERR_ARGUMENT, "omc_relax_append_shor: the staged batch is not in Shor mode (omc_relax_append)");
  if (B2 <= 0) return fail(OMC_ERR_ARGUMENT, "B must be positive");
  if (!n_shor || !n_soc) return fail(OMC_ERR_ARGUMENT, "n_shor / n_soc is NULL");
  const ShorAppendLists lists = {n_shor, shor_idx, n_soc, soc_idx};
  return append_nodes(h, "omc_relax_append_shor", B2, L, cut_x, cut_Uhat, cut_dir, load_from, save_to, &lists);
}

int shor_append_plan(omc_instance* h, int first, int B2, const ShorAppendLists& l, std::vector<int>& load, std::vector<int>& save, ShorGrouping& g) {
  const ShWS& sh = h->sh;
  const ShorKnownLists known = {&h->sh_byhash, &h->sh_lists, h->sh_group_cap, h->sh_int_cap - h->sh_int_used, h->sh_byte_cap - h->sh_byte_used,
                                sh.nqmax, sh.nv1max, sh.nv2max};
  { int rc0 = shor_list_offsets(B2, l.n_shor, l.shor_idx, l.n_soc, l.soc_idx, g.so, g.co); if (rc0) return rc0; }
  g.index_min = h->sh_index_min; g.stream = h->append_stream; g.grow = false;
  { int rc0 = group_shor_lists(h, B2, l.n_shor, l.shor_idx, l.n_soc, l.soc_idx, &known, g); if (rc0) return rc0; }
  if (load.empty()) return 0;
  const int NG0 = (int)h->sh_lists.size();
  std::lock_guard<std::mutex> lk2(h->sig_mu);
  for (int b = 0; b < B2; ++b) {
    omc_instance::PoolSig sg;
    sg.kind = 2; sg.nq = l.n_shor[b]; sg.nsoc = l.n_soc[b];
    sg.hlist = g.node_group[b] < NG0 ? h->sh_lists[g.node_group[b]].hlist : g.lists[g.node_group[b] - NG0].hlist;
    sg.hsoc = l.n_soc[b] > 0 ? fnv1a(l.soc_idx + 2 * g.co[b], 16 * (size_t)l.n_soc[b], FNV_SEED) : 0;
    shor_warm_filter(h, sg, l.shor_idx + 4 * g.so[b], &load[b], &save[b]);
    h->node_sig[(size_t)first + b] = sg;
  }
  return 0;
}

int shor_append_write(omc_instance* h, const ShorGrouping& g, int first, hipStream_t s, ShorGroupImages& img) {
  return upload_shor_groups(h, g, h->sgInts.as<int>() + h->sh_int_used, h->sgBytes.as<uint8_t>() + h->sh_byte_used,
                            h->sgGroups.as<ShorGroupDev>() + h->sh_lists.size(), h->sgNodeGroup.as<int>() + first, s, img);
}

void shor_append_commit(omc_instance* h, ShorGrouping& g) {
  for (size_t q = 0; q < g.lists.size(); ++q) {
    h->sh_byhash[g.hashes[q]].push_back((int)h->sh_lists.size());
    h->sh_lists.push_back(std::move(g.lists[q]));
  }
  h->sh_int_used += g.tot_int; h->sh_byte_used += g.tot_byte;
}

int omc_relax_fetch_done_shor(omc_instance* h, int n_ids, const int* node_ids, double* X, double* W, double* Theta) {
  if (!h) return fail(OMC_ERR_ARGUMENT, "handle is NULL");
  if (!h->staged || !h->shor_on) return fail(OMC_ERR_ARGUMENT, "omc_relax_fetch_done_shor: no Shor-mode batch staged");
  if (n_ids < 0 || (n_ids > 0 && !node_ids)) return fail(OMC_ERR_ARGUMENT, "omc_relax_fetch_done_shor: bad arguments");
  if (n_ids == 0) return 0;
  { int rcf = require_finished_ids(h, n_ids, node_ids, true, "omc_relax_fetch_done_shor"); if (rcf) return rcf; }
  HIPCHK(hipSetDevice(h->device));
  if (!h->fetch_stream) HIPCHK(hipStreamCreateWithFlags(&h->fetch_stream, hipStreamNonBlocking));
  hipStream_t fs = h->fetch_stream;
  const size_t nm = (size_t)h->n * h->m, mm = (size_t)h->m * h->m;
  for (int i = 0; i < n_ids; ++i) {
    const size_t nb = (size_t)node_ids[i];
    if (X) HIPCHK(hipMemcpyAsync(X + i * nm, h->sh.oX + nb * nm, 8 * nm, hipMemcpyDeviceToHost, fs));
    if (W) HIPCHK(hipMemcpyAsync(W + i * nm, h->sh.oW + nb * nm, 8 * nm, hipMemcpyDeviceToHost, fs));
    if (Theta) HIPCHK(hipMemcpyAsync(Theta + i * mm, h->sh.oTh + nb * mm, 8 * mm, hipMemcpyDeviceToHost, fs));
  }
  HIPCHK(hipStreamSynchronize(fs));
  return 0;
}
```

### optimalmatrixcompletion.jl_amd/csrc/omc_device.hip

```cpp
#include <hip/hip_runtime.h>
#include <type_traits>
#include <stdint.h>
#include "omc_device.h"
#include "omc.h"

#include "omc_wave.h"


#ifdef OMC_STAMPS
#define STAMP(slot) do { __syncthreads(); if (blockIdx.x == 0 && threadIdx.x == 0) { long long t_ = __builtin_amdgcn_s_memtime(); w.stamps[slot] += (double)(t_ - t_prev_); t_prev_ = t_; } } while (0)
#define STAMP_BEGIN() long long t_prev_ = __builtin_amdgcn_s_memtime()
#define DIAG_T0() long long t_diag0_ = __builtin_amdgcn_s_memtime()
#define DIAG_ADD(cls, b, v) atomicAdd(&w.stamps[32 + (size_t)(cls) * w.B + (b)], (double)(v))
#define DIAG_CYC(cls, b) DIAG_ADD(cls, b, __builtin_amdgcn_s_memtime() - t_diag0_)
#define WSTAMP_BEGIN() long long tw_prev_ = __builtin_amdgcn_s_memtime()
#define WSTAMP_BEGIN2() tw_prev_ = __builtin_amdgcn_s_memtime()
#define WSTAMP(slot) do { if (b == 0 && j == 0 && lane == 0) { long long t_ = __builtin_amdgcn_s_memtime(); w.stamps[slot] += (double)(t_ - tw_prev_); tw_prev_ = t_; } } while (0)
#else
#define WSTAMP_BEGIN() do {} while (0)
#define WSTAMP_BEGIN2() do {} while (0)
#define WSTAMP(slot) do {} while (0)
#define STAMP(slot) do {} while (0)
#define STAMP_BEGIN() do {} while (0)
#define DIAG_T0() do {} while (0)
// ... 935 lines not shown
          for (int i = 0; i < R2; ++i) {
            if (RPL2 || i < rpl2) { cp_[i] = gp[i * LPP]; cq_[i] = gq[i * LPP]; gm0 += cp_[i].x * cq_[i].x; gm1 += cp_[i].y * cq_[i].y; }
          }
          double gm = (LPP == 64) ? wave_sum(gm0 + gm1) : group_sum_dpp<(LPP == 64) ? 16 : LPP>(gm0 + gm1);
          const double a = ev[p], bb = ev[q];
          const double g2 = gm * gm, ab = a * bb;
          if (g2 > tau2 * ab && ab > 0.0) {
            const float df = (float)(bb - a), gf = (float)gm;
            const float rtf = __builtin_sqrtf(df * df + 4.0f * gf * gf);
            const float den = (df >= 0.0f) ? (df + rtf) : (df - rtf);
            const double tt = (den != 0.0f) ? (double)((2.0f * gf) / den) : 0.0;
            const double cs = rsqrt(1.0 + tt * tt), sn = cs * tt;
#pragma unroll
            for (int i = 0; i < R2; ++i) {
              if (RPL2 || i < rpl2) {
                double2v np_, nq_;
                np_.x = cs * cp_[i].x - sn * cq_[i].x; np_.y = cs * cp_[i].y - sn * cq_[i].y;
                nq_.x = sn * cp_[i].x + cs * cq_[i].x; nq_.y = sn * cp_[i].y + cs * cq_[i].y;
                gp[i * LPP] = np_; gq[i * LPP] = nq_;
              }
            }
            if (lg == 0) { ev[p] = a - tt * gm; ev[q] = bb + tt * gm; }
#ifdef OMC_STAMPS
            if (lg == 0 && b == 0 && !evals_only) atomicAdd(&w.stamps[32 + (size_t)6 * w.B + (sweeps < 8 ? sweeps : 7)], 1.0);
#endif
            if (g2 > tau * ab) big = 1;
          }
        }
        __syncthreads();
      }
      if (!__syncthreads_or(big)) { ++sweeps; break; }
    }
    if (tid == 0) w.sweeps[b] += sweeps;
#ifdef OMC_STAMPS
    if (tid == 0 && b == 0 && !evals_only) atomicAdd(&w.stamps[32 + (size_t)7 * w.B + (sweeps < 8 ? sweeps : 7)], 1.0);
#endif
  }
  STAMP(1);
  for (int t = wv; t < N; t += nw) {
    double a = 0.0;
    for (int r = lane; r < Nrp; r += WAVE) { double x = Gm[(size_t)t * ld + r]; a += x * x; }
    a = wave_sum(a);
    if (lane == 0) ev[t] = a;
  }
  __syncthreads();
  for (int e = tid; e < N * N; e += T) {
    int t = e % N, kk = e / N;
    Vr[(size_t)kk * NP + t] = Gm[(size_t)t * ld + kk] * rsqrt(ev[t]);
  }
  if (tid == 0) vvalid[b] = 1;
  STAMP(2);
  if (evals_only) {
    if (w.cert_enable && N >= 3 * SUBP) {
      double* lam_s = (double*)(sel + Np + (Np & 1));
      for (int t = tid; t < N; t += T) lam_s[t] = sqrt(ev[t]) - sigma;
      __syncthreads();
      if (tid == 0) {
        for (int j = 0; j < SUBP; ++j) {
          int bi = -1; double bl = 1e300;
          for (int t = 0; t < N; ++t) {
            bool used = false;
            for (int q = 0; q < j; ++q) if (s_top[q] == t) used = true;
            if (!used && lam_s[t] < bl) { bl = lam_s[t]; bi = t; }
          }
          s_top[j] = bi;
          w.sub_thetaC[(size_t)b * SUBP + j] = -bl;
        }
        w.sub_onC[b] = 1;
      }
      __syncthreads();
      double* Xg = w.XsC + (size_t)b * NP * SUBP;
      for (int e = tid; e < SUBP * NP; e += T) {
        const int j = e / NP, r = e - j * NP;
        Xg[e] = (r < N) ? Gm[(size_t)s_top[j] * ld + r] * rsqrt(ev[s_top[j]]) : 0.0;
      }
    }
    if (tid == 0) {
      const int k = w.k;
      double best[8]; const int kk2 = (k < 8) ? k : 8;
      for (int i = 0; i < kk2; ++i) best[i] = 1e300;
      for (int t = 0; t < N; ++t) {
        double lamv = sqrt(ev[t]) - sigma;
        for (int i = 0; i < kk2; ++i) if (lamv < best[i]) { const double tmp = best[i]; best[i] = lamv; lamv = tmp; }
      }
      double s2 = 0.0;
      for (int i = 0; i < kk2; ++i) s2 += fmin(best[i], 0.0);
      w.evsum[b] = s2;
    }
    return;
  }
  double* lamv_s = (double*)(sel + Np + (Np & 1));
  for (int t = tid; t < N; t += T) lamv_s[t] = sqrt(ev[t]) - sigma;
  __syncthreads();
  const double hi = w.clip_hi;
  if (tid == 0) {
    int ndef = 0, nkeep = 0;
    for (int t = 0; t < N; ++t) {
      const double lamv = lamv_s[t];
      if (lamv < 0.0 || lamv > hi) ++ndef;
      if (lamv > 0.0) ++nkeep;
    }
    s_nkeep = nkeep;
    if (w.sub_debug == 3) { const int mn = (ndef < nkeep) ? ndef : nkeep; atomicAdd(&w.stamps[32 + ((ndef < 31) ? ndef : 31)], 1.0); atomicAdd(&w.stamps[64 + ((mn < 31) ? mn : 31)], 1.0); }
    int c = 0;
    if (ndef <= nkeep) {
      for (int t = 0; t < N; ++t) {
        const double lamv = lamv_s[t];
        if (lamv < 0.0) { sel[c] = t; wgt[c] = -lamv; ++c; }
        else if (lamv > hi) { sel[c] = t; wgt[c] = -(lamv - hi); ++c; }
      }
      s_base = 1.0;
    } else {
      for (int t = 0; t < N; ++t) {
        const double lamv = lamv_s[t];
        if (lamv > 0.0) { sel[c] = t; wgt[c] = fmin(lamv, hi); ++c; }
      }
      s_base = 0.0;
    }
    s_nsel = c;
  }
  __syncthreads();
  if (w.sub_enable) {
    const bool seed = s_nkeep <= SUBP - w.sub_guard && N >= 3 * SUBP;
    if (w.sub_debug == 3 && tid == 0) atomicAdd(&w.stamps[(s_nkeep < 31) ? s_nkeep : 31], 1.0);
    if (seed) {
      for (int t = tid; t < N; t += T) {
        const double lt = lamv_s[t];
        int rk = 0;
        for (int u = 0; u < N; ++u) { const double lu = lamv_s[u]; rk += (lu > lt || (lu == lt && u < t)) ? 1 : 0; }
        if (rk < SUBP) { s_top[rk] = t; w.sub_theta[(size_t)b * SUBP + rk] = lt; }
      }
      __syncthreads();
      double* Xg = w.Xs + (size_t)b * NP * SUBP;
      for (int e = tid; e < SUBP * NP; e += T) {
        const int j = e / NP, r = e - j * NP;
        Xg[e] = (r < N) ? Gm[(size_t)s_top[j] * ld + r] * rsqrt(ev[s_top[j]]) : 0.0;
      }
      if (tid == 0) atomicAdd(&w.sub_stat[8 * b + 3], 1);
    }
    if (tid == 0) w.sub_on[b] = seed ? 1 : 0;
  }
  for (int c2 = tid; c2 < s_nsel; c2 += T) wgt[c2] /= ev[sel[c2]];
  __syncthreads();
  double* Wout = w.W1 + (size_t)b * n * n;
  auto entry2 = [&](int i, int j) { return Mb[(size_t)j * NP + i]; };
  auto store = [&](int i, int j, double v, double) { Wout[(size_t)j * n + i] = v; Wout[(size_t)i * n + j] = v; };
  STAMP(3);
  spectral_rebuild(Gm, ld, N, sel, wgt, s_nsel, s_base, entry2, store);
  STAMP(4);
  if (tid == 0) { DIAG_CYC(2, b); DIAG_ADD(3, b, 1); if (w.ws_phase == 1) w.cone_done[b] = 1; }
}


template <int MODE>
__global__ void __launch_bounds__(256, 2) k_cone_sub(OmcWS w) {
  extern __shared__ double smem[];
  __shared__ int s_flag, s_nsel, s_cond;
  __shared__ double s_shift, s_cs[SUBP];
  const int b = (MODE == 0) ? slot_of(w, blockIdx.x) : (int)blockIdx.x, tid = threadIdx.x, T = blockDim.x;
  if (MODE == 2) {
    if (!w.fin[b] || !w.sub_on[b]) return;
  } else {
    if (w.done[b]) return;
    if (MODE == 0) {
      if (w.ws_first) {
        if (w.ws_first[b]) { if (threadIdx.x == 0 && w.sub_wait[b] > 0) w.sub_wait[b] -= 1; return; }
      } else {
        if (!w.sub_on[b]) return;
        if (w.sub_wait[b] > 0) { if (threadIdx.x == 0) w.sub_wait[b] -= 1; return; }
      }
    } else {
      if (!w.sub_onC[b]) { if (threadIdx.x == 0) w.confirm[b] = 1; return; }
    }
  }
  const SubLayout L = sub_layout(w.np16);
  const int n = w.n, NP = w.np16, nt = NP >> 4, LD = L.LD;
  const int wv = tid >> 6, lane = tid & 63, li = lane & 15, lk = lane >> 4;
  double* Xa = smem;
  double* Za = L.zglob ? w.sub_zscratch + (size_t)b * SUBP * LD : Xa + L.Za;
  double* Cs = Xa + L.Cs, *Hs = Xa + L.Hs, *Gj = Xa + L.Gj, *th = Xa + L.th, *evj = Xa + L.evj, *red = Xa + L.red, *wgt = Xa + L.wgt;
  int* sel = (int*)(Xa + L.sel);
  const double* Mb = ((MODE == 1) ? w.MbufC : w.Mbuf) + (size_t)b * NP * NP;
  double* Xg = ((MODE == 1) ? w.XsC : w.Xs) + (size_t)b * NP * SUBP;
  double* thg = ((MODE == 1) ? w.sub_thetaC : w.sub_theta) + (size_t)b * SUBP;
  constexpr double sgn = (MODE == 1) ? -1.0 : 1.0;
  const double fro2 = (MODE == 1) ? w.fro2c[b] : w.fro2[b], nF = sqrt(fro2), trM = (MODE == 1) ? -w.trMc[b] : w.trM[b];
  const double tol_eff = (MODE == 2) ? 1e-11 : (MODE == 1) ? 1e-9 : fmin(1e-6, fmax(w.sub_tol, w.sub_adapt * w.rd[b] / fmax(nF, 1e-300)));
  for (int e = tid; e < SUBP * NP; e += T) { const int j = e / NP, r = e - j * NP; Xa[(size_t)j * LD + r] = Xg[e]; }
  if (tid < SUBP) th[tid] = thg[tid];
  __syncthreads();

  auto mul_MX = [&](double shift, bool back, bool scaled) {
    const double* Xi = Xa + (back ? L.Za : 0);
    double* Zo = back ? Xa : Za;
    for (int tb = 0; tb < nt; tb += 12) {
      const int b0 = tb + wv;
      if (b0 >= nt) break;
      const int t0 = b0, t1 = (b0 + 4 < nt) ? b0 + 4 : b0, t2 = (b0 + 8 < nt) ? b0 + 8 : b0;
      const bool v1 = b0 + 4 < nt, v2 = b0 + 8 < nt;
      double4v acc0 = {0.0, 0.0, 0.0, 0.0}, acc1 = acc0, acc2 = acc0;
      const unsigned m0 = (t0 << 4) + li, m1 = (t1 << 4) + li, m2 = (t2 << 4) + li;
      const double* Xb = Xi + (size_t)li * LD;
      double a0[4], a1[4], a2[4];
#pragma unroll
      for (int u = 0; u < 4; ++u) { const unsigned o = (unsigned)(4 * u + lk) * (unsigned)NP; a0[u] = Mb[m0 + o]; a1[u] = Mb[m1 + o]; a2[u] = Mb[m2 + o]; }
      for (int k0 = 0; k0 < NP; k0 += 16) {
#pragma unroll
        for (int u = 0; u < 4; ++u) {
          const double x0 = sgn * a0[u], x1 = sgn * a1[u], x2 = sgn * a2[u], bv = Xb[k0 + 4 * u + lk];
          int kn = k0 + 16 + 4 * u + lk;
          kn = (kn < NP) ? kn : kn - NP;
          const unsigned o = (unsigned)kn * (unsigned)NP;
          a0[u] = Mb[m0 + o]; a1[u] = Mb[m1 + o]; a2[u] = Mb[m2 + o];
          acc0 = __builtin_amdgcn_mfma_f64_16x16x4f64(x0, bv, acc0, 0, 0, 0);
          acc1 = __builtin_amdgcn_mfma_f64_16x16x4f64(x1, bv, acc1, 0, 0, 0);
          if (nt > 8) acc2 = __builtin_amdgcn_mfma_f64_16x16x4f64(x2, bv, acc2, 0, 0, 0);
        }
      }
      const double cs = scaled ? s_cs[li] : 1.0;
#pragma unroll
      for (int r = 0; r < 4; ++r) {
        const size_t a = (size_t)li * LD + lk + 4 * r;
        const double z0 = acc0[r] + shift * Xi[a + (t0 << 4)];
        Zo[a + (t0 << 4)] = scaled ? cs * z0 : z0;
        if (v1) { const double z1 = acc1[r] + shift * Xi[a + (t1 << 4)]; Zo[a + (t1 << 4)] = scaled ? cs * z1 : z1; }
        if (v2) { const double z2 = acc2[r] + shift * Xi[a + (t2 << 4)]; Zo[a + (t2 << 4)] = scaled ? cs * z2 : z2; }
      }
    }
  };
  auto gram = [&](const double* P, const double* Q) {
    double4v acc = {0.0, 0.0, 0.0, 0.0};
    const double* Pa = P + (size_t)li * LD;
    const double* Qa = Q + (size_t)li * LD;
    for (int u = wv; u < (NP >> 2); u += 4) {
      const int row = 4 * u + lk;
      acc = __builtin_amdgcn_mfma_f64_16x16x4f64(Pa[row], Qa[row], acc, 0, 0, 0);
    }
#pragma unroll
    for (int r = 0; r < 4; ++r) Cs[wv * 256 + (lk + 4 * r) * 16 + li] = acc[r];
    __syncthreads();
    Hs[(tid >> 4) * 17 + (tid & 15)] = (Cs[tid] + Cs[256 + tid]) + (Cs[512 + tid] + Cs[768 + tid]);
    __syncthreads();
  };

  int steps = 0, ok = 0, fail = 0, nrr = 0;
  const int qmax = (MODE == 2) ? 4 * w.sub_qmax : w.sub_qmax, chunk = w.sub_chunk;
  const bool prof = (w.sub_debug == 2) && b == 0;
  long long tprev = prof ? __builtin_amdgcn_s_memtime() : 0;
#define SUBSTAMP(slot) do { if (prof) { __syncthreads(); if (tid == 0) { const long long t_ = __builtin_amdgcn_s_memtime(); w.stamps[slot] += (double)(t_ - tprev); tprev = t_; } } } while (0)
  SUBSTAMP(0);
  bool skip_steps = (MODE == 2);
  while (true) {
    if (wv == 0 && !skip_steps) {
      const double tj = (lane < SUBP) ? th[lane] : 0.0;
      const double st = wave_sum(tj), st2 = wave_sum(tj * tj);
      const double nr = (double)(n - SUBP);
      const double mu = (trM - st) / nr;
      const double var = fmax((fro2 - st2) / nr - mu * mu, 0.0);
      double hi = (lane < SUBP && tj > mu) ? tj : 1e300, lo_t = (lane < SUBP && !(tj > mu)) ? tj : 1e300;
      for (int o = 32; o > 0; o >>= 1) { hi = fmin(hi, __shfl_xor(hi, o, WAVE)); lo_t = fmin(lo_t, __shfl_xor(lo_t, o, WAVE)); }
      if (hi > 1e299) hi = mu;
      double lo = fmax(mu - sqrt(var * (nr - 1.0)), mu - 3.0 * sqrt(var));
      if (lo_t < 1e299) lo = fmin(lo, lo_t - 0.05 * (hi - lo_t));
      double tmax = (lane < SUBP) ? tj : -1e300;
      for (int o = 32; o > 0; o >>= 1) tmax = fmax(tmax, __shfl_xor(tmax, o, WAVE));
      const double sh = -0.5 * (lo + hi);
      if (lane < SUBP) s_cs[lane] = 1.0 / fmax(fabs(tj + sh), 1e-3 * fmax(fabs(tmax + sh), 1e-300));
      if (lane == 0) s_shift = sh;
    }
    __syncthreads();
    const double shift = s_shift;
    SUBSTAMP(1);
    for (int c = 0; c < chunk && !fail && !skip_steps; ++c) {
      const bool inner = MODE != 2 && c + 1 < chunk, pp = MODE == 0 && !L.zglob, back = inner && pp && c > 0 && ((chunk - 1 - c) & 1);
      const bool copy = inner && !back && (!pp || ((chunk - 1 - c) & 1));
      mul_MX(shift, back, inner && !copy);
      __syncthreads();
      SUBSTAMP(2);
      if (inner) {
        if (copy) {
          for (int e = tid; e < SUBP * NP; e += T) { const int j = e / NP, r = e - j * NP; Xa[(size_t)j * LD + r] = s_cs[j] * Za[(size_t)j * LD + r]; }
          __syncthreads();
        }
        SUBSTAMP(5);
        ++steps;
        continue;
      }
      for (int pass = 0; pass < 2; ++pass) {
        gram(Za, Za);
        SUBSTAMP(3);
        if (wv == 0) {
          double c[SUBP], dinv[SUBP];
          const int i = (lane < SUBP) ? lane : SUBP - 1;
#pragma unroll
          for (int q = 0; q < SUBP; ++q) c[q] = Hs[i * 17 + q];
          int bad = 0;
          double dmin = 1e300, dmax = 0.0;
#pragma unroll
          for (int j = 0; j < SUBP; ++j) {
            const double d = readlane_d(c[j], j);
            if (!(d > 1e-280)) bad = 1;
            dmin = fmin(dmin, d); dmax = fmax(dmax, d);
            const double inv = rsqrt(fmax(d, 1e-280));
            dinv[j] = inv;
            const double lj = c[j] * inv;
#pragma unroll
            for (int q = j + 1; q < SUBP; ++q) c[q] = fma(-lj, readlane_d(lj, q), c[q]);
            c[j] = lj;
          }
          double z[SUBP];
#pragma unroll
          for (int r = 0; r < SUBP; ++r) {
            double v = (r == i) ? 1.0 : 0.0;
#pragma unroll
            for (int q = 0; q < SUBP; ++q) if (q < r) v = fma(-readlane_d(c[q], r), z[q], v);
            z[r] = v * dinv[r];
          }
          if (lane < SUBP) {
#pragma unroll
            for (int r = 0; r < SUBP; ++r) Hs[r * 17 + lane] = (r >= lane) ? z[r] : 0.0;
          }
          if (lane == 0) { s_flag = bad; s_cond = (pass == 0 && dmin < 1e-6 * dmax) ? 1 : 0; }
        }
        __syncthreads();
        SUBSTAMP(4);
        if (s_flag) { fail = 3; break; }
        const bool again = s_cond != 0;
        {
          double* Xo = again ? Za : Xa;
          for (int ti = wv; ti < nt; ti += 4) {
            const int i0 = ti << 4;
            double4v a1 = {0.0, 0.0, 0.0, 0.0};
#pragma unroll
            for (int u = 0; u < 4; ++u)
              a1 = __builtin_amdgcn_mfma_f64_16x16x4f64(Za[(size_t)(4 * u + lk) * LD + i0 + li], Hs[li * 17 + 4 * u + lk], a1, 0, 0, 0);
            WAVE_SYNC();
#pragma unroll
            for (int r = 0; r < 4; ++r) Xo[(size_t)li * LD + i0 + lk + 4 * r] = a1[r];
          }
        }
        __syncthreads();
        SUBSTAMP(5);
        if (!again) break;
      }
      if (fail) break;
      ++steps;
    }
    if (fail) break;
    skip_steps = false;
    mul_MX(0.0, false, false);
    __syncthreads();
    gram(Xa, Za);
    SUBSTAMP(6);
    {
      const int i = tid >> 4, j = tid & 15;
      const double hv = 0.5 * (Hs[i * 17 + j] + Hs[j * 17 + i]);
      const double f2 = block_sum(hv * hv, red);
      if (tid == 0) s_shift = 1.5 * sqrt(f2) + 1e-300;
      __syncthreads();
      Gj[j * 17 + i] = hv + ((i == j) ? s_shift : 0.0);
      __syncthreads();
      if (wv == 0) {
        jacobi16_fast(Gj, evj, 17, 1e-13, 12);
        if (lane < 16) { double a = 0.0;
#pragma unroll
          for (int r = 0; r < 16; ++r) { const double x = Gj[lane * 17 + r]; a += x * x; }
          evj[lane] = a; }
      }
      __syncthreads();
    }
    const double sigma = s_shift;
    if (tid < SUBP) th[tid] = sqrt(evj[tid]) - sigma;
    __syncthreads();
    SUBSTAMP(7);
    Hs[(tid >> 4) * 17 + (tid & 15)] = Gj[(tid & 15) * 17 + (tid >> 4)] * rsqrt(evj[tid & 15]);
    __syncthreads();
    {
      for (int ti = wv; ti < nt; ti += 4) {
        const int i0 = ti << 4;
        double4v a1 = {0.0, 0.0, 0.0, 0.0}, a2 = {0.0, 0.0, 0.0, 0.0};
#pragma unroll
        for (int u = 0; u < 4; ++u) {
          const double bw = Hs[(4 * u + lk) * 17 + li];
          a1 = __builtin_amdgcn_mfma_f64_16x16x4f64(Xa[(size_t)(4 * u + lk) * LD + i0 + li], bw, a1, 0, 0, 0);
          a2 = __builtin_amdgcn_mfma_f64_16x16x4f64(Za[(size_t)(4 * u + lk) * LD + i0 + li], bw, a2, 0, 0, 0);
        }
        WAVE_SYNC();
#pragma unroll
        for (int r = 0; r < 4; ++r) { const size_t a = (size_t)li * LD + i0 + lk + 4 * r; Xa[a] = a1[r]; Za[a] = a2[r]; }
      }
      __syncthreads();
    }
    SUBSTAMP(8);
    for (int c = 0; c < 4; ++c) {
      const int t = 4 * wv + c;
      const double tv = th[t];
      double a = 0.0;
      for (int r = lane; r < NP; r += WAVE) { const double d = Za[(size_t)t * LD + r] - tv * Xa[(size_t)t * LD + r]; a += d * d; }
      a = wave_sum(a);
      if (lane == 0) evj[t] = sqrt(a);
    }
    __syncthreads();
// ... 1547 lines not shown
    const int i = e % n, j = e / n;
    double v = 0.0;
    for (int rr = 0; rr < R; ++rr) {
      const double lv = lam[rr];
      if (lv != 0.0 && w.rkind[(size_t)b * w.Rmax + rr] == ROW_CUT) {
        const double* x = cutx + (size_t)w.rcut[(size_t)b * w.Rmax + rr] * n;
        v += lv * x[i] * x[j];
      }
    }
    if (Psi) for (int a = 0; a < r; ++a) v -= T1[(size_t)a * n + i] * Q[(size_t)a * n + j];
    M[e] = v;
  }
  for (int e = tid; e < n * k; e += T) {
    const int i = e % n, j = e / n;
    double cu = 0.0;
    for (int rr = 0; rr < R; ++rr) { const double lv = lam[rr]; if (lv != 0.0) cu += lv * rowU_entry(w, b, rr, i, j); }
    cU[e] = cu;
  }
  __syncthreads();
  if (w.lamDX) {
    double* D = w.lamDX + (size_t)b * m * n;
    if (Lam) {
      for (int j = tid; j < m; j += T) {
        const int off = w.col_ptr[j], c = w.col_ptr[j + 1] - off;
        for (int p = 0; p < c; ++p) D[(size_t)j * n + w.col_idx[off + p]] = Lam[off + p];
      }
      __syncthreads();
      __threadfence_block();
    }
    mfma_LLt<1>(D, n, m, [&](int i, int j, double v) {
      const double t = 0.5 * g * v;
      M[(size_t)j * n + i] -= t;
      if (i != j) M[(size_t)i * n + j] -= t;
    });
    __syncthreads();
  } else {
    for (int j = 0; j < m; ++j) {
      const int off = w.col_ptr[j], c = w.col_ptr[j + 1] - off;
      for (int e = tid; e < c * c; e += T) {
        const int p = e % c, q = e / c;
        M[(size_t)w.col_idx[off + q] * n + w.col_idx[off + p]] -= 0.5 * g * Lam[off + p] * Lam[off + q];
      }
      __syncthreads();
    }
  }
  if (poison) {
    for (int e = tid; e < n * n; e += T) M[e] = (e % n == e / n) ? -1.0 : 0.0;
    __syncthreads();
  }
  double pen = 0.0;
  for (int j = 0; j < k; ++j) {
    double acc = 0.0;
    for (int a = tid; a < r; a += T) {
      double cv = Psi ? -2.0 * Psi[(size_t)(r + j) * N3 + a] : 0.0;
      for (int i = 0; i < n; ++i) cv += Q[(size_t)a * n + i] * cU[(size_t)j * n + i];
      acc += cv * cv;
    }
    pen += sqrt(block_sum(acc, red));
  }
  const int NP = w.np16;
  double fr2 = 0.0;
  for (int e = tid; e < n * n; e += T) {
    const int i = e % n, j = e / n;
    const double mv = 0.5 * (M[e] + M[(size_t)i * n + j]);
    w.MbufC[(size_t)b * NP * NP + (size_t)j * NP + i] = mv; fr2 += mv * mv;
  }
  fr2 = block_sum(fr2, red);
  if (tid == 0) {
    double cst = 0.0;
    for (int rr = 0; rr < R; ++rr)
      if (w.rkind[(size_t)b * w.Rmax + rr] != ROW_TRACE) cst -= lam[rr] * w.rrhs[(size_t)b * w.Rmax + rr];
    if (Psi) for (int j = 0; j < k; ++j) cst -= Psi[(size_t)(r + j) * N3 + r + j];
    w.c0[b] = c0; w.cpen[b] = pen; w.cst[b] = cst; w.fro2c[b] = fr2;
  }
}

template <int LPP>
static void launch_ws_lds(const OmcWS* w, hipStream_t s) {
  const size_t lds_bytes = w->geo.ws.lds_bytes;
  switch (w->geo.ws_rpl2) {
    case 4: hipLaunchKernelGGL((k_cone_ws<LPP, true, 4>), dim3(w->nB), dim3(512), lds_bytes, s, *w); break;
    case 5: hipLaunchKernelGGL((k_cone_ws<LPP, true, 5>), dim3(w->nB), dim3(512), lds_bytes, s, *w); break;
    case 6: hipLaunchKernelGGL((k_cone_ws<LPP, true, 6>), dim3(w->nB), dim3(512), lds_bytes, s, *w); break;
    case 7: hipLaunchKernelGGL((k_cone_ws<LPP, true, 7>), dim3(w->nB), dim3(512), lds_bytes, s, *w); break;
    case 8: hipLaunchKernelGGL((k_cone_ws<LPP, true, 8>), dim3(w->nB), dim3(512), lds_bytes, s, *w); break;
    default: hipLaunchKernelGGL((k_cone_ws<LPP, true, 0>), dim3(w->nB), dim3(512), lds_bytes, s, *w); break;
  }
}
static int residency_of(const void* kern, int threads, size_t lds) {
  int nb = 0;
  return hipOccupancyMaxActiveBlocksPerMultiprocessor(&nb, kern, threads, lds) == hipSuccess ? nb : -1;
}
template <int LPP>
static const void* ws_lds_kernel(int rpl2) {
  switch (rpl2) {
    case 4: return (const void*)k_cone_ws<LPP, true, 4>;
    case 5: return (const void*)k_cone_ws<LPP, true, 5>;
    case 6: return (const void*)k_cone_ws<LPP, true, 6>;
    case 7: return (const void*)k_cone_ws<LPP, true, 7>;
    case 8: return (const void*)k_cone_ws<LPP, true, 8>;
    default: return (const void*)k_cone_ws<LPP, true, 0>;
  }
}
__global__ void __launch_bounds__(256) k_gram_XXt(OmcWS w, const double* X) {
  const int b = blockIdx.x, n = w.n;
  double* Y = w.Y + (size_t)b * n * n;
  mfma_LLt<1>(X + (size_t)b * n * w.m, n, w.m, [&](int i, int j, double v) { Y[(size_t)j * n + i] = v; Y[(size_t)i * n + j] = v; });
}
extern "C" {
void omc_launch_gram_XXt(const OmcWS* w, const double* X, int B, hipStream_t s) { hipLaunchKernelGGL(k_gram_XXt, dim3(B), dim3(256), 0, s, *w, X); }
void omc_launch_setup(const OmcWS* w, hipStream_t s) { hipLaunchKernelGGL(k_setup, dim3(w->B), dim3(256), 0, s, *w); }
void omc_launch_setup_gram(const OmcWS* w, const int* jobs, int njobs, int nnodes, hipStream_t s) {
  const int chunks = gram_chunks(w->Rmax);
  if (njobs <= 0 || chunks <= 0) return;
  for (int q0 = 0; q0 < njobs; q0 += 65535) {
    const int nq = njobs - q0 < 65535 ? njobs - q0 : 65535;
    hipLaunchKernelGGL(k_setup_gram, dim3(chunks, nq), dim3(256), 0, s, *w, jobs + 2 * (size_t)q0, nq, nnodes);
  }
}
void omc_launch_colprox(const OmcWS* w, int mode, hipStream_t s) {
  const int wpb = 4;
  omc_launch_colprox_block(w, mode, s);
  if (mode == 0 && !w->cp_pair && w->cp_nrest == 0) return;
  if (mode == 0 && w->cp_pair) {
    omc_launch_colprox_sweep(w, s);
    if (w->cp_nsolo == 0) return;
  }
  const int waves = w->nB * ((mode == 0 && w->cp_pair) ? w->cp_nsolo : w->m);
  const int blocks = (waves + wpb - 1) / wpb;
  hipLaunchKernelGGL(k_colprox, dim3(blocks), dim3(wpb * 64), (size_t)wpb * w->geo.cp_lds_doubles * sizeof(double), s, *w, mode);
}
void omc_launch_cone(const OmcWS* w, int mode, hipStream_t s) {
  if (w->geo.plain_mw && (mode == CONE_SEP || mode == CONE_TOPK)) { omc_launch_cone_plain_mw(w, mode, s); return; }
  if (w->geo.cone.use_lds) hipLaunchKernelGGL(k_cone<true>, dim3(w->nB), dim3(512), w->geo.cone.lds_bytes, s, *w, mode);
  else hipLaunchKernelGGL(k_cone<false>, dim3(w->nB), dim3(512), 0, s, *w, mode);
}
void omc_launch_cone_ws(const OmcWS* w, hipStream_t s) {
  if (w->geo.mw) { omc_launch_cone_mw(w, s); return; }
  const int lpp = w->geo.ws_lpp, rpl2 = w->geo.ws_rpl2;
  if (w->geo.ws.use_lds) {
    if (lpp == 16) launch_ws_lds<16>(w, s);
    else if (lpp == 8) launch_ws_lds<8>(w, s);
    else launch_ws_lds<4>(w, s);
  } else {
    if (lpp == 64) {
      if (rpl2 == 8) hipLaunchKernelGGL((k_cone_ws<64, false, 8, 1024>), dim3(w->nB), dim3(1024), 0, s, *w);
      else hipLaunchKernelGGL((k_cone_ws<64, false, 0, 1024>), dim3(w->nB), dim3(1024), 0, s, *w);
    } else if (rpl2 == 7 && !w->cone_512) hipLaunchKernelGGL((k_cone_ws<16, false, 7, 1024>), dim3(w->nB), dim3(1024), 0, s, *w);
    else if (rpl2 == 8 && !w->cone_512) hipLaunchKernelGGL((k_cone_ws<16, false, 8, 1024>), dim3(w->nB), dim3(1024), 0, s, *w);
    else hipLaunchKernelGGL((k_cone_ws<16, false, 0>), dim3(w->nB), dim3(512), 0, s, *w);
  }
}
void omc_launch_cone_sub(const OmcWS* w, hipStream_t s) {
  hipLaunchKernelGGL(k_cone_sub<0>, dim3(w->nB), dim3(256), w->geo.sub_lds, s, *w);
}
void omc_launch_sep_sub(const OmcWS* w, hipStream_t s) {
  hipLaunchKernelGGL(k_sep_prepare, dim3(w->B), dim3(256), 0, s, *w);
  hipLaunchKernelGGL(k_cone_sub<2>, dim3(w->B), dim3(256), w->geo.sub_lds, s, *w);
}
void omc_launch_cert_sub(const OmcWS* w, hipStream_t s) {
  hipLaunchKernelGGL(k_cone_sub<1>, dim3(w->B), dim3(256), w->geo.sub_lds, s, *w);
}
void omc_launch_small(const OmcWS* w, int mode, hipStream_t s) {
  if (w->geo.small.use_lds) hipLaunchKernelGGL(k_small<true>, dim3(w->nB), dim3(256), w->geo.small.lds_bytes, s, *w, mode);
  else hipLaunchKernelGGL(k_small<false>, dim3(w->nB), dim3(256), 0, s, *w, mode);
}
void omc_launch_global(const OmcWS* w, hipStream_t s) {
  if (w->geo.glob.use_lds) hipLaunchKernelGGL(k_global<true>, dim3(w->nB), dim3(512), w->geo.glob.lds_bytes, s, *w);
  else hipLaunchKernelGGL(k_global<false>, dim3(w->nB), dim3(512), 0, s, *w);
}
void omc_launch_row_project(int B, int R, int Rmax, int which, const double* G, const double* c, double* lam, int* overflow, hipStream_t s) {
  if (which) hipLaunchKernelGGL(k_row_project<1>, dim3(B), dim3(WAVE), 0, s, G, c, lam, overflow, R, Rmax);
  else hipLaunchKernelGGL(k_row_project<0>, dim3(B), dim3(WAVE), 0, s, G, c, lam, overflow, R, Rmax);
}
void omc_launch_check_zero(const OmcWS* w, hipStream_t s) { hipLaunchKernelGGL(k_zero_check, dim3((w->B + 63) / 64), dim3(64), 0, s, *w); }
void omc_launch_check_build(const OmcWS* w, hipStream_t s) { hipLaunchKernelGGL(k_check_build, dim3(w->B), dim3(512), 0, s, *w); }
void omc_launch_check_final(const OmcWS* w, int last, int phase, hipStream_t s) {
  hipLaunchKernelGGL(k_check_final, dim3((w->B + 63) / 64), dim3(64), 0, s, *w, last, phase);
}
void omc_launch_rho_rescale(const OmcWS* w, hipStream_t s) { hipLaunchKernelGGL(k_rho_rescale, dim3(w->B), dim3(256), 0, s, *w); }
void omc_launch_harvest(const OmcWS* w, hipStream_t s) { hipLaunchKernelGGL(k_harvest, dim3(w->B), dim3(256), 0, s, *w); }
void omc_launch_dual_assemble(const OmcWS* w, const OmcDualIn* in, hipStream_t s) { hipLaunchKernelGGL(k_dual_assemble, dim3(w->B), dim3(512), 0, s, *w, *in); }
void omc_launch_cert_snapshot(const OmcWS* w, hipStream_t s) { hipLaunchKernelGGL(k_cert_snapshot, dim3(w->B), dim3(256), 0, s, *w); }
void omc_launch_cert_harvest(const OmcWS* w, hipStream_t s) { hipLaunchKernelGGL(k_cert_harvest, dim3(w->B), dim3(256), 0, s, *w); }
void omc_launch_state_save(const OmcWS* w, hipStream_t s) { hipLaunchKernelGGL(k_state_save, dim3(w->B), dim3(256), 0, s, *w); }
void omc_launch_aa(const OmcWS* w, hipStream_t s) { hipLaunchKernelGGL(k_aa, dim3(w->nB), dim3(512), 0, s, *w); }
void omc_launch_make_X(const OmcWS* w, double* X, hipStream_t s) { hipLaunchKernelGGL(k_make_X, dim3(64, w->Btot), dim3(256), 0, s, *w, X); }
void omc_launch_make_Theta(const OmcWS* w, const double* X, double* Th, hipStream_t s) {
  hipLaunchKernelGGL(k_make_Theta, dim3(64, w->Btot), dim3(256), 0, s, *w, X, Th);
}
void omc_launch_eval_objective(int B, int n, int m, double gamma, const double* A, const uint8_t* mask, const double* X,
                               double* out, hipStream_t s) {
  hipLaunchKernelGGL(k_eval_objective, dim3(B), dim3(256), 0, s, n, m, gamma, A, mask, X, out);
}
int omc_set_max_lds(void) {
  hipError_t e1 = hipFuncSetAttribute((const void*)k_cone<true>, hipFuncAttributeMaxDynamicSharedMemorySize, OMC_MAX_DYN_LDS);
  hipError_t e2 = hipFuncSetAttribute((const void*)k_global<true>, hipFuncAttributeMaxDynamicSharedMemorySize, OMC_MAX_DYN_LDS - 8 * 1024);
  hipError_t e3 = hipFuncSetAttribute((const void*)k_colprox, hipFuncAttributeMaxDynamicSharedMemorySize, OMC_MAX_DYN_LDS);
  hipError_t e4 = hipFuncSetAttribute((const void*)k_small<true>, hipFuncAttributeMaxDynamicSharedMemorySize, OMC_MAX_DYN_LDS);
  (void)hipFuncSetAttribute((const void*)k_cone_sub<0>, hipFuncAttributeMaxDynamicSharedMemorySize, OMC_MAX_DYN_LDS);
  (void)hipFuncSetAttribute((const void*)k_cone_sub<1>, hipFuncAttributeMaxDynamicSharedMemorySize, OMC_MAX_DYN_LDS);
  (void)hipFuncSetAttribute((const void*)k_cone_sub<2>, hipFuncAttributeMaxDynamicSharedMemorySize, OMC_MAX_DYN_LDS);
#define WS_ATTR(L, R) (void)hipFuncSetAttribute((const void*)k_cone_ws<L, true, R>, hipFuncAttributeMaxDynamicSharedMemorySize, OMC_MAX_DYN_LDS)
#define WS_ATTR_ALL(L) WS_ATTR(L, 0); WS_ATTR(L, 4); WS_ATTR(L, 5); WS_ATTR(L, 6); WS_ATTR(L, 7); WS_ATTR(L, 8)
  WS_ATTR_ALL(4); WS_ATTR_ALL(8); WS_ATTR_ALL(16);
  if (e1 != hipSuccess) return 1000 + (int)e1;
  if (e2 != hipSuccess) return 2000 + (int)e2;
  if (e3 != hipSuccess) return 3000 + (int)e3;
  if (e4 != hipSuccess) return 4000 + (int)e4;
  { const int e5 = omc_colprox_block_set_lds(); if (e5) return 6000 + e5; }
  return 0;
}
void omc_query_residency(const OmcWS* w, int* out) {
  const OmcGeom& g = w->geo;
  out[OMC_RES_CONE_SUB] = residency_of((const void*)k_cone_sub<0>, 256, g.sub_lds);
  out[OMC_RES_CONE_SUB_CERT] = residency_of((const void*)k_cone_sub<1>, 256, g.sub_lds);
  out[OMC_RES_CONE_SUB_SEP] = residency_of((const void*)k_cone_sub<2>, 256, g.sub_lds);
  out[OMC_RES_GLOBAL] = g.glob.use_lds ? residency_of((const void*)k_global<true>, 512, g.glob.lds_bytes) : residency_of((const void*)k_global<false>, 512, 0);
  out[OMC_RES_SMALL] = g.small.use_lds ? residency_of((const void*)k_small<true>, 256, g.small.lds_bytes) : residency_of((const void*)k_small<false>, 256, 0);
  omc_colprox_sweep_residency(w, &out[OMC_RES_COLPROX_PAIR], &out[OMC_RES_COLPROX_WIDE]);
  out[OMC_RES_COLPROX] = residency_of((const void*)k_colprox, 256, (size_t)4 * g.cp_lds_doubles * sizeof(double));
  out[OMC_RES_CONE] = g.cone.use_lds ? residency_of((const void*)k_cone<true>, 512, g.cone.lds_bytes) : residency_of((const void*)k_cone<false>, 512, 0);
  const int lpp = g.ws_lpp, rpl2 = g.ws_rpl2;
  int ws = -1;
  if (g.mw || !lpp) ;
  else if (g.ws.use_lds) ws = residency_of(lpp == 16 ? ws_lds_kernel<16>(rpl2) : lpp == 8 ? ws_lds_kernel<8>(rpl2) : ws_lds_kernel<4>(rpl2), 512, g.ws.lds_bytes);
  else if (lpp == 64) ws = rpl2 == 8 ? residency_of((const void*)k_cone_ws<64, false, 8, 1024>, 1024, 0) : residency_of((const void*)k_cone_ws<64, false, 0, 1024>, 1024, 0);
  else if (rpl2 == 7 && !w->cone_512) ws = residency_of((const void*)k_cone_ws<16, false, 7, 1024>, 1024, 0);
  else if (rpl2 == 8 && !w->cone_512) ws = residency_of((const void*)k_cone_ws<16, false, 8, 1024>, 1024, 0);
  else ws = residency_of((const void*)k_cone_ws<16, false, 0>, 512, 0);
  out[OMC_RES_CONE_WS] = ws;
}
}
```

### optimalmatrixcompletion.jl_amd/csrc/omc_host.h

```cpp
#pragma once
#include <hip/hip_runtime.h>
#include <stdint.h>
#include <atomic>
#include <mutex>
#include <string>
#include <thread>
#include <unordered_map>
#include <vector>

#include "omc.h"
#include "omc_carve.h"
#include "omc_device.h"
#include "omc_shor_relax.h"
#include "omc_shor_index.h"
#include "omc_walks.h"

extern thread_local std::string g_err;
static inline int fail(int code, const std::string& msg) { g_err = msg; return code; }
#define HIPCHK(x)                                                                                         \
  do {                                                                                                    \
    hipError_t e_ = (x);                                                                                  \
    if (e_ != hipSuccess) {                                                                               \
      g_err = std::string(#x) + ": " + hipGetErrorString(e_);                                             \
      return (int)e_ > 0 ? (int)e_ : 999;                                                                 \
    }                                                                                                     \
  } while (0)

struct DevBuf {
  void* p = nullptr; size_t cap = 0;
  DevBuf() = default;
  DevBuf(const DevBuf&) = delete;
  DevBuf& operator=(const DevBuf&) = delete;
  ~DevBuf() { release(); }
  int ensure(size_t bytes) {
    if (bytes <= cap) return 0;
    if (p) (void)hipFree(p);
    p = nullptr; cap = 0;
    size_t want = bytes + bytes / 4 + 256;
    hipError_t e = hipMalloc(&p, want);
    if (e != hipSuccess) { g_err = std::string("hipMalloc: ") + hipGetErrorString(e); return (int)e; }
    cap = want;
    return 0;
  }
  void release() { if (p) (void)hipFree(p); p = nullptr; cap = 0; }
  template <class T> T* as() { return (T*)p; }
};
#define ENS(buf, bytes) do { int r_ = (buf).ensure(bytes); if (r_) return r_; } while (0)

template <class F> static inline int carve_ensure(DevBuf& b, F&& walk, size_t* bytes = nullptr) {
  Carve measure;
  walk(measure);
  if (bytes) *bytes = measure.bytes();
  const int rc = b.ensure(measure.bytes());
  if (rc) return rc;
  Carve place(b.p);
  walk(place);
  return 0;
}
#define ENS_CARVE(buf, ...) do { int r_ = carve_ensure(buf, __VA_ARGS__); if (r_) return r_; } while (0)

template <class T> static inline int bind(DevBuf& b, T*& field, size_t count) {
  field = nullptr;
  const int rc = b.ensure(count * sizeof(T));
  if (rc) return rc;
  field = (T*)b.p;
  return 0;
}
template <class T> static inline int bind(DevBuf& b, T*& field, size_t count, hipStream_t zero_on) {
  const int rc = bind(b, field, count);
  if (rc) return rc;
  HIPCHK(hipMemsetAsync(b.p, 0, count * sizeof(T), zero_on));
  return 0;
}
#define BIND(...) do { int r_ = bind(__VA_ARGS__); if (r_) return r_; } while (0)

struct PinBuf {
  void* p = nullptr; size_t cap = 0;
  PinBuf() = default;
  PinBuf(const PinBuf&) = delete;
  PinBuf& operator=(const PinBuf&) = delete;
  ~PinBuf() { if (p) (void)hipHostFree(p); }
  int ensure(size_t bytes) {
    if (bytes <= cap) return 0;
    if (p) (void)hipHostFree(p);
    p = nullptr; cap = 0;
    hipError_t e = hipHostMalloc(&p, bytes, hipHostMallocDefault);
    if (e != hipSuccess) { g_err = std::string("hipHostMalloc: ") + hipGetErrorString(e); return (int)e; }
    cap = bytes;
    return 0;
  }
  template <class T> T* as() { return (T*)p; }
};

struct Tuning {
  bool altmin_nolds = false;
  bool colprox_no_xcd = false;
  bool cone_512 = false;
  bool dense_proj = false;
  bool host_phases = false;
  bool global_nolds = false;
  bool no_colprox_pair = false;
  bool no_graph = false;
  bool no_subspace = false;
  bool no_ws_split = false;
  bool segv_trace = false;
  bool setup_gram_inline = false;
  bool shor_explicit = false;
  bool shor_no_subspace = false;
  int check_xs = 16;
  int colprox_dpp = 1;
  int colprox_block_min = 65;
  int cone_multi_min = 1025;
  int event_merge = 1;
  int graph_max = 16;
  int harvest_async = 1;
  int harvest_async_min_live = 256;
  int plain_multi_min = 1025;
  int shor_index_device_min = 0;
  int small_chain = 1;
  int shor_select_kb = 1048576;
  int streams = 4;
  int sub_debug = 0;
  int sub_qmax = 24;
  int timing_stride = 1;
  int ws_quiet = 1;
};
struct Knob { const char* name; bool Tuning::*flag; int Tuning::*num; };
inline const Knob OMC_KNOBS[] = {
  {"OMC_ALTMIN_NOLDS", &Tuning::altmin_nolds, nullptr},      {"OMC_COLPROX_NO_XCD", &Tuning::colprox_no_xcd, nullptr},
  {"OMC_CONE_512", &Tuning::cone_512, nullptr},              {"OMC_DENSE_PROJ", &Tuning::dense_proj, nullptr},
  {"OMC_GLOBAL_NOLDS", &Tuning::global_nolds, nullptr},      {"OMC_HOST_PHASES", &Tuning::host_phases, nullptr},
  {"OMC_NO_COLPROX_PAIR", &Tuning::no_colprox_pair, nullptr},
  {"OMC_NO_GRAPH", &Tuning::no_graph, nullptr},              {"OMC_NO_SUBSPACE", &Tuning::no_subspace, nullptr},
  {"OMC_NO_WS_SPLIT", &Tuning::no_ws_split, nullptr},        {"OMC_SEGV_TRACE", &Tuning::segv_trace, nullptr},
  {"OMC_SETUP_GRAM_INLINE", &Tuning::setup_gram_inline, nullptr},
  {"OMC_SHOR_EXPLICIT", &Tuning::shor_explicit, nullptr},    {"OMC_SHOR_NO_SUBSPACE", &Tuning::shor_no_subspace, nullptr},
  {"OMC_COLPROX_BLOCK_MIN", nullptr, &Tuning::colprox_block_min},  {"OMC_COLPROX_DPP", nullptr, &Tuning::colprox_dpp},
  {"OMC_CHECK_XS", nullptr, &Tuning::check_xs},              {"OMC_CONE_MULTI_MIN", nullptr, &Tuning::cone_multi_min},
  {"OMC_EVENT_MERGE", nullptr, &Tuning::event_merge},
  {"OMC_GRAPH_MAX", nullptr, &Tuning::graph_max},            {"OMC_SHOR_SELECT_KB", nullptr, &Tuning::shor_select_kb},
  {"OMC_SHOR_INDEX_DEVICE_MIN", nullptr, &Tuning::shor_index_device_min},
  {"OMC_HARVEST_ASYNC", nullptr, &Tuning::harvest_async},    {"OMC_HARVEST_ASYNC_MIN_LIVE", nullptr, &Tuning::harvest_async_min_live},
  {"OMC_WS_QUIET", nullptr, &Tuning::ws_quiet},
  {"OMC_STREAMS", nullptr, &Tuning::streams},                {"OMC_PLAIN_MULTI_MIN", nullptr, &Tuning::plain_multi_min},
  {"OMC_SUB_DEBUG", nullptr, &Tuning::sub_debug},            {"OMC_SUB_QMAX", nullptr, &Tuning::sub_qmax},
  {"OMC_SMALL_CHAIN", nullptr, &Tuning::small_chain},
  {"OMC_TIMING_STRIDE", nullptr, &Tuning::timing_stride},
};

struct omc_instance {
  int n = 0, m = 0, k = 0, device = 0, nnz = 0, cmax = 0;
  double gamma = 0, sumA2 = 0;
  std::vector<int> col_ptr, col_idx; std::vector<double> col_val;
  std::vector<double> A; std::vector<uint8_t> mask;
  std::vector<double> Ncnt;
  std::vector<int> row_ptr, row_idx; std::vector<double> row_val;
  DevBuf drow_ptr, drow_idx, drow_val, aR, arkind, arcut, arbi, arbj, arcoef, arrhs, acutx, aU0, aU, aV, aobj, aint, aG, aG2;
  hipStream_t stream = nullptr;
  Tuning tun;
  hipStream_t gs[3] = {};
  hipEvent_t gev[5] = {};
  hipEvent_t gevc[5] = {};
  hipEvent_t ev_main = nullptr;
  PinBuf pin_flags[2], pin_list[2], pin_done, pin_jobs; DevBuf bgramjobs;
  hipEvent_t ev_up[4] = {}; bool ev_up_rec[4] = {}; hipEvent_t ev_gram = nullptr; bool ev_gram_rec = false;
  double host_ms[OMC_HOST_NPHASE] = {0}; int64_t host_cnt[OMC_HOST_NPHASE] = {0};
  DevBuf dA, dmask, dcol_ptr, dcol_idx, dcol_val, dNcnt, dwY, dsolo, dwide;
  int nwide = 0;
  int nsolo = 0;
  DevBuf dblock, dslab, disblock, bcpb, bnfact;
  int nblock = 0, nslab = 0, nrest = 0, cpb_cl = 0, cpb_cs = 0, crest_max = 0;
  bool lists_valid = false; int lists_block_min = 0; bool lists_pair = true;
  DevBuf bYx, bY, bYp, bU, bD1, bD3, bW1, bE3, bQb, brr, bsm, bdS, balpha, balphaX, bsval, bMchk, bsmall, bchk;
  DevBuf bR, brkind, brcut, brbi, brbj, brcoef, brrhs, bcutx, bG, blam;
  DevBuf bobjcol, baaF, baaG, baaZ, baaS, baaI, bMbufC, bVrowC, bchkS, bchkI;
  DevBuf bslotlist, bgap, bvotes, blamDX, bXsC, bsubSC, bsubIC;
  DevBuf bsubz, bscal, bbx, bint, bcp, bcone, bglob, bXout, bThout, bXin, bMbuf, bVrow, bXs, bsubS, bsubI;
  long long sub_tot[8] = {0};
  DevBuf bmwstat, sbigmw, pjM, pjV, pjW, pjS, pjD, pjI;
  long long mw_tot[5] = {0};
  DevBuf bpmwstat; long long pmw_tot[4] = {0};
  OmcWS ws{};
  omc_relax_params params{};
  bool staged = false;
  double last_solve_seconds = 0; long long total_sweeps = 0; int last_iters_total = 0;
  std::thread worker; std::atomic<int> worker_running{0}, nodes_done{0}; int worker_rc = 0; std::string worker_err;
  int reserve_nodes = 0, reserve_cuts = 0, node_cap = 0, staged_cut_type = 0; std::atomic<int> Btot_live{0}; bool append_closed = true; std::mutex append_mu; hipStream_t append_stream = nullptr;
  std::atomic<int> hold{0};
  std::vector<int> done_q; size_t done_read = 0; std::mutex done_mu; hipStream_t fetch_stream = nullptr;
  void* comm = nullptr; int comm_rank = 0, comm_world = 1; DevBuf bcomm, amobj; int amobj_B = 0;
  int wall_khz = 0;
  std::vector<double> rho_scale_per_node; DevBuf brho, brhon, blamD, bslotint, boY, boU, boal, bobx, boscal, boint;
  int Btot = 0;
  bool keep_cert = false; DevBuf bcbD, bcbI, bocD, bocI;
  bool keep_shor_cert = false; DevBuf scbD, socD, socNq;
  DevBuf dbD, dbI, dbM, dbS, dbL;
  DevBuf sdD, sdI, sdGi, sdGb, sdGr; double sdb_ms = 0.0;
  DevBuf sbits, scb, scx, scz, soff, stot, sout, shi, slo, sexist, shist, sohi, solo, scnt;
  bool shor_ready = false; int shor_W = 0; long long shor_pairs = 0;
  double shor_last_ms = 0; long long shor_last_candidates = 0;
  int64_t shor_sel[4] = {0, 0, 0, 0};
  bool shor_on = false, shor_keep_V = false, shor_via_base = false; std::vector<int> shor_slackrow; DevBuf soV; double shor_rho = 0.05, shor_r4 = 0.0, shor_r5 = 2.0;
  ShWS sh{}; OmcWS wbig{};
  DevBuf sgInts, sgBytes, sgGroups, sgNodeGroup, sAh, sX, sW, sTh, sV1, sV2, sV3, sD0, sP0, sMbufB, sVrowB, sTq, sPq, sNq, sD5x, sD5t, snu5, sP5x,
      scolpart, sminpart, sminpart2, sfroB, svvB, se1, se2, soX, soW, soTh, sbigscr, sXsB, ssubSB, ssubIB;
  long long big_sub_tot[8] = {0};
  struct ShorListKey { int64_t nq = 0, nsoc = 0; uint64_t hlist = 0; std::vector<int64_t> idx, soc; };
  int64_t reserve_shor_nq = 0; int reserve_shor_lists = 0; bool reserve_shor_set = false;
  std::unordered_map<uint64_t, std::vector<int>> sh_byhash; std::vector<ShorListKey> sh_lists;
  int sh_group_cap = 0; size_t sh_int_used = 0, sh_int_cap = 0, sh_byte_used = 0, sh_byte_cap = 0;
  DevBuf sxD; ShorIndexDims sx_dims{}; ShorIndexWS sx{}; int* sx_stage_int = nullptr; uint8_t* sx_stage_byte = nullptr;
  int sh_index_min = 0; double shidx_stats[5] = {0, 0, 0, 0, 0};
  int pool_cap = 0; DevBuf pY, pD1, pD3, pU, palpha, psval, pXs, ptheta, pscal, bwarmL, bwarmS; std::vector<int> warm_load, warm_save;
  struct PoolSig { int kind = 0; int64_t nq = 0, nsoc = 0; uint64_t hlist = 0, hsoc = 0; };
  bool pool_shor = false; int64_t pool_nqmax = 0; DevBuf pShor, pShorHdr, sloadpart;
  std::vector<PoolSig> pool_sig, node_sig; std::mutex sig_mu;
  std::vector<int> save_host;
  int64_t shor_warm_stats[4] = {0, 0, 0, 0};
  int64_t launches[OMC_KERNEL_NCLASS] = {0}; double ms[OMC_KERNEL_NCLASS] = {0}; int64_t units[OMC_KERNEL_NCLASS] = {0};
  size_t nnz_rows() const { return row_idx.size(); }
  std::vector<hipEvent_t> ev_pool[2];
};

static constexpr int MAX_SWEEPS = 30;
```

### optimalmatrixcompletion.jl_amd/csrc/omc_layout.h

```cpp
#ifndef OMC_LAYOUT_H
#define OMC_LAYOUT_H
#include <hip/hip_runtime.h>
#include <stddef.h>

#define NNQP_PMAX 64
#define NNQP_GP_DOUBLES (NNQP_PMAX * (NNQP_PMAX + 1) / 2)
#define NNQP_STATIC_BYTES ((NNQP_GP_DOUBLES + 2 * NNQP_PMAX) * 8 + NNQP_PMAX * 4)
#define OMC_MAX_DYN_LDS (144 * 1024)
#define SUBP 16
#define GL_XS 16
#define OMC_HD __host__ __device__ inline
struct ConeLayout { int Np, ld; size_t ev, wgt, sel; };
OMC_HD ConeLayout cone_carve(int N, int ld) { const int Np = (N + 1) & ~1; const size_t ev = (size_t)Np * ld; return {Np, ld, ev, ev + Np, ev + 2 * Np}; }
OMC_HD ConeLayout cone_layout(int N) { return cone_carve(N, ((N + 1) & ~1) | 1); }
OMC_HD size_t cone_bytes(int N) { const ConeLayout L = cone_layout(N); return L.sel * 8 + (size_t)L.Np * 4 + 16; }
OMC_HD size_t ws_bytes(int N, int ld) { const ConeLayout L = cone_carve(N, ld); return (L.sel + L.Np) * 8 + (size_t)(L.Np + 2) * 4 + 64; }
OMC_HD int ws_rpl(int N, int lpp) { return (((N + lpp - 1) / lpp) + 1) & ~1; }
struct WsGeometry { int lpp, rpl, ld, use_lds; size_t bytes; };
OMC_HD WsGeometry ws_geometry(int N) {
  const int Np2 = (N + 1) & ~1;
  int lpp = 16; while (lpp > 4 && lpp * (Np2 / 2) > 512) lpp >>= 1;
  int rpl = ws_rpl(N, lpp), Nrp = rpl * lpp;
  int ld = Nrp + ((16 - (Nrp & 31)) & 31);
  if (ws_bytes(N, ld) > OMC_MAX_DYN_LDS) ld = Nrp + 2;
  const int use_lds = ws_bytes(N, ld) <= OMC_MAX_DYN_LDS;
  if (!use_lds) {
    lpp = 16; rpl = ws_rpl(N, 16);
    if (rpl > 32 && N <= 1024) { lpp = 64; rpl = ws_rpl(N, 64); }
    ld = rpl * lpp + 2;
  }
  return {rpl <= 32 ? lpp : 0, rpl, ld, use_lds, ws_bytes(N, ld)};
}
#define GRAM_CHUNK 8
#define CB_XS 4096
OMC_HD int gram_npairs(int R) { return R * (R + 1) / 2; }
OMC_HD int gram_chunks(int R) { return (gram_npairs(R) + GRAM_CHUNK - 1) / GRAM_CHUNK; }
OMC_HD void gram_pair_of(int p, int R, int* r, int* s) {
  int rr = 0;
  while (p >= R - rr) { p -= R - rr; ++rr; }
  *r = rr; *s = rr + p;
}
OMC_HD void gram_pair_next(int R, int* r, int* s) { if (++*s == R) { ++*r; *s = *r; } }
#define MW_B 16
#define MW_MAXSW 32
#define MW_MIN_ORDER 145
#define MW_MAX_ORDER 4096
#define MW_TAU_PLAIN 1e-14
#define MW_PLAIN_SWEEPS 30
struct MwLayout { int ld, Ncp, nb; size_t ev, lam, wgt, sel, smax, head, bytes, fro; };
OMC_HD MwLayout mw_layout(int N) {
  const int NP = (N + 15) & ~15, Ncp = (N + 2 * MW_B - 1) & ~(2 * MW_B - 1), ld = NP + 4;
  static_assert(2 * MW_B >= 16, "fro: the NP / 16 partial sums of the plain sequence lie in the Ncp words of wgt, NP <= Ncp");
  const size_t ev = (size_t)Ncp * ld, sel = ev + 3 * (size_t)Ncp, smax = sel + Ncp / 2, head = smax + MW_MAXSW;
  return {ld, Ncp, Ncp / MW_B, ev, ev + Ncp, ev + 2 * (size_t)Ncp, sel, smax, head, (head + 4) * 8, ev + 2 * (size_t)Ncp};
}
OMC_HD int mw_plain_launches(const MwLayout& L, int sweeps) { return sweeps * (L.nb - 1) + 4; }
struct SubLayout { int LD, zglob; size_t Za, Cs, Hs, Gj, th, evj, red, wgt, sel, bytes; };
OMC_HD SubLayout sub_layout(int np16) {
  const int LD = np16 + 2, zglob = np16 > 512; const size_t blk = (size_t)SUBP * LD, Cs = (zglob ? 1 : 2) * blk, th = Cs + 4 * 256 + 2 * 16 * 17;
  return {LD, zglob, blk, Cs, Cs + 4 * 256, Cs + 4 * 256 + 16 * 17, th, th + 16, th + 32, th + 64, th + 80, (th + 80 + 8) * 8};
}
#define SMALL_STATIC_LDS 1024
#define SMALL_CS 512
struct SmallLayout { int ld3; size_t M3, Gm, ev, wgt, sel, Cc, Qs, Cs, bytes; };
OMC_HD SmallLayout small_layout(int n, int rmax, int k) {
  const int ld3 = rmax + k, Npm = (ld3 + 1) & ~1, ldm = Npm | 1;
  const size_t M3 = (size_t)n * rmax, Gm = M3 + (size_t)ld3 * ld3, ev = Gm + (size_t)Npm * ldm, sel = ev + 2 * Npm, Cc = sel + Npm / 2, Qs = Cc + (size_t)rmax * k + 2;
  const size_t Cs = Qs + (size_t)n * 16;
  return {ld3, M3, Gm, ev, ev + Npm, sel, Cc, Qs, Cs, (Cs + SMALL_CS) * 8 + 104};
}
#define GLOB_STATIC_LDS ((size_t)NNQP_STATIC_BYTES + 2560)
struct GlobLayout { size_t tU, tV, cvec, mu, xs, qrow, bytes; };
OMC_HD GlobLayout glob_layout(int n, int k, int rmax, int Rmax) {
  const size_t tU = (size_t)n * (n + 1) / 2, tV = tU + (size_t)n * k, cvec = tV + (size_t)rmax * k, xs = cvec + 2 * Rmax, qrow = xs + (size_t)GL_XS * n;
  return {tU, tV, cvec, cvec + Rmax, xs, qrow, (qrow + Rmax) * 8 + 80};
}
OMC_HD bool glob_w1_fits(int n) { return (size_t)SUBP * n <= (size_t)NNQP_GP_DOUBLES; }
struct CpRegLayout { int Lm, vo, pinv, sidx, doubles; };
OMC_HD CpRegLayout cp_reg_layout(int c, int keepB) { const int tri = (c * (c + 1)) >> 1, vo = (keepB ? 2 : 1) * tri; return {keepB ? tri : 0, vo, vo + c, vo + 2 * c, vo + 4 * c + 8}; }
struct CpBodyLayout { size_t Lm, va, vy, vz, vo, doubles; };
OMC_HD CpBodyLayout cp_body_layout(int c) { const size_t tri = (size_t)c * (c + 1) / 2, va = 2 * tri; return {tri, va, va + c, va + 2 * c, va + 3 * c, va + 4 * c + 8}; }
#define CPB_TILE 256
#define CPB_STATIC_LDS 4352
struct CpBlockLayout { int nb, ntiles; size_t panel, va, vy, vz, vw, vo, sidx, doubles, slab; };
OMC_HD int cpb_tile(int I, int J) { return ((I * (I + 1)) >> 1) + J; }
OMC_HD CpBlockLayout cp_block_layout(int c, int lds) {
  const int nb = c > 0 ? (c + 15) >> 4 : 1, nt = (nb * (nb + 1)) >> 1;
  const size_t cp = (size_t)16 * nb, va = (size_t)CPB_TILE * (lds ? nt : (nb > 1 ? nb - 1 : 1));
  return {nb, nt, 0, va, va + cp, va + 2 * cp, va + 3 * cp, va + 4 * cp, va + 5 * cp, va + 5 * cp + cp / 2, lds ? 0 : (size_t)CPB_TILE * nt};
}
OMC_HD int cp_block_fits(int c, int lds) { return cp_block_layout(c, lds).doubles * 8 <= (size_t)OMC_MAX_DYN_LDS; }
OMC_HD int cp_block_lds_cmax() { int nb = 1; while (cp_block_fits(16 * (nb + 1), 1)) ++nb; return 16 * nb; }
OMC_HD int cp_block_cmax() { int nb = 1; while (cp_block_fits(16 * (nb + 1), 0)) ++nb; return 16 * nb; }
OMC_HD void cp_block_plan(int cmax, int block_min, long long* out) {
  const int ldsc = cp_block_lds_cmax(), on = cmax >= block_min && cmax >= 1 && cmax <= cp_block_cmax();
  const CpBlockLayout L = cp_block_layout(cmax, cmax <= ldsc);
  out[0] = ldsc; out[1] = on ? (long long)(L.doubles * 8) : 0; out[2] = on ? (long long)L.slab : 0;
  out[3] = on ? (long long)((160 * 1024) / (L.doubles * 8 + CPB_STATIC_LDS)) : 0; out[4] = on;
}
struct Altmin1Layout { size_t v, h, g, u0, cvec, mu, bytes; };
OMC_HD Altmin1Layout altmin1_layout(int n, int m, int Rmax) { const size_t h = (size_t)n + m, cvec = h + 3 * n; return {(size_t)n, h, h + n, h + 2 * n, cvec, cvec + Rmax, (cvec + 2 * Rmax + 8) * 8}; }
struct AltminKLayout { size_t ut, u0, g, H, Hinv, v, cvec, mu, bytes; };
OMC_HD AltminKLayout altmink_layout(int n, int m, int k, int Rmax) {
  const size_t nk = (size_t)n * k, H = 4 * nk, v = H + 2 * nk * k, cvec = v + (size_t)k * m;
  return {nk, 2 * nk, 3 * nk, H, H + nk * k, v, cvec, cvec + Rmax, (cvec + 2 * Rmax + 8) * 8};
}
struct AltminWLayout { size_t ut, u0, g, H, Hinv, v, cvec, mu, th, th2, q, qt, step, tmp, act, J, P, Lc, bytes; };
OMC_HD AltminWLayout altminw_layout(int n, int m, int k, int Rmax) {
  const size_t nk = (size_t)n * k, mq = (size_t)k * k, H = 4 * nk, v = H + 2 * nk * k, cvec = v + (size_t)k * m, th = cvec + 2 * Rmax, J = th + 7 * mq, Lc = J + 2 * mq * mq;
  return {nk, 2 * nk, 3 * nk, H, H + nk * k, v, cvec, cvec + Rmax, th, th + mq, th + 2 * mq, th + 3 * mq, th + 4 * mq, th + 5 * mq, th + 6 * mq, J, J + mq * mq, Lc,
          (Lc + mq * (mq + 1) / 2 + 8) * 8};
}
struct KernelPlan { int use_lds; size_t lds_bytes, slab_stride; };
OMC_HD KernelPlan plan_block(size_t bytes, bool fits) { return {fits ? 1 : 0, fits ? bytes : 0, fits ? 0 : bytes / 8 + 8}; }
#define ALTMIN_KMAX 8
OMC_HD int altmin_variant(int k) { return k == 1 ? 1 : (k <= 4 ? 2 : 3); }
OMC_HD KernelPlan altmin_plan(int n, int m, int k, int Rmax, int nolds) {
  const int var = altmin_variant(k);
  const size_t bytes = (var == 1) ? altmin1_layout(n, m, Rmax).bytes : (var == 2) ? altmink_layout(n, m, k, Rmax).bytes : altminw_layout(n, m, k, Rmax).bytes;
  return plan_block(bytes, bytes + 8 * 1024 <= ((var == 1) ? (size_t)OMC_MAX_DYN_LDS - 8 * 1024 : (size_t)128 * 1024) && !nolds);
}
struct OmcGeom {
  KernelPlan cone, ws, glob, small;
  int ws_lpp, ws_rpl2, ws_ld;
  size_t cpb_lds_bytes, cpb_slab_lds_bytes, cpb_slab_stride;
  int cp_lds_c, cp_lds_doubles, cp_keepB;
  size_t cp_scratch_stride, sub_lds;
  int mw; MwLayout mwl;
  int plain_mw;
};
OMC_HD void geom_set_mw(OmcGeom& g, int n) {
  g.mw = 1; g.mwl = mw_layout(n);
  size_t st = g.mwl.bytes / 8 + 8; if (st < g.ws.slab_stride) st = g.ws.slab_stride;
  g.cone.slab_stride = g.ws.slab_stride = (st + 3) & ~(size_t)3;
}
OMC_HD void geom_set_plain_mw(OmcGeom& g, int n) {
  const int mw = g.mw;
  geom_set_mw(g, n);
  g.mw = mw; g.plain_mw = 1;
}
OMC_HD void geom_set_cpblock(OmcGeom& g, int cl, int cs) {
  g.cpb_lds_bytes = cl > 0 ? cp_block_layout(cl, 1).doubles * 8 : 0;
  g.cpb_slab_lds_bytes = cs > 0 ? cp_block_layout(cs, 0).doubles * 8 : 0;
  g.cpb_slab_stride = cs > 0 ? cp_block_layout(cs, 0).slab : 0;
}
OMC_HD bool mw_order_ok(int n, int use_lds, int knob) { return n >= MW_MIN_ORDER && !use_lds && n >= knob && n <= MW_MAX_ORDER; }
OMC_HD OmcGeom omc_plan_geometry(int n, int np16, int k, int rmax, int Rmax, int cmax, int global_nolds, int cone_multi_min, int plain_multi_min) {
  OmcGeom g;
  const WsGeometry wg = ws_geometry(n);
  g.cone = plan_block(cone_bytes(n), cone_bytes(n) <= OMC_MAX_DYN_LDS);
  g.ws = plan_block(wg.bytes, wg.use_lds != 0);
  g.ws_lpp = wg.lpp; g.ws_rpl2 = wg.rpl >> 1; g.ws_ld = wg.ld;
  g.cone.slab_stride = g.ws.slab_stride = g.cone.slab_stride > g.ws.slab_stride ? g.cone.slab_stride : g.ws.slab_stride;
  g.sub_lds = sub_layout(np16).bytes;
  const size_t gb = glob_layout(n, k, rmax, Rmax).bytes, sb = small_layout(n, rmax, k).bytes;
  g.glob = plan_block(gb, gb + GLOB_STATIC_LDS <= OMC_MAX_DYN_LDS && !global_nolds);
  g.small = plan_block(sb, sb + SMALL_STATIC_LDS <= OMC_MAX_DYN_LDS);
  g.cp_lds_c = cmax < 64 ? cmax : 64; g.cp_keepB = g.cp_lds_c <= 40 ? 1 : 0;
  g.cp_lds_doubles = cp_reg_layout(g.cp_lds_c, g.cp_keepB).doubles;
  g.cp_scratch_stride = cmax > g.cp_lds_c ? cp_body_layout(cmax).doubles : 0;
  g.mw = g.plain_mw = 0; g.mwl = MwLayout{};
  g.cpb_lds_bytes = g.cpb_slab_lds_bytes = g.cpb_slab_stride = 0;
  if (mw_order_ok(n, wg.use_lds, cone_multi_min)) geom_set_mw(g, n);
  if (mw_order_ok(n, wg.use_lds, plain_multi_min)) geom_set_plain_mw(g, n);
  return g;
}
#endif
```

Measured before the change: 2619.

## Stage symmetric M triangle in LDS for cone subspace kernel matmuls

```diff
diff --git a/include/omc.h b/include/omc.h
--- a/include/omc.h
+++ b/include/omc.h
@@ -232,6 +232,7 @@
 #define OMC_RES_CONE 9
 #define OMC_RES_N 10
 int omc_kernel_residency(omc_instance* h, int* out);
+int omc_cone_sub_plan(omc_instance* h, int64_t* out);
 int omc_last_subspace_stats(omc_instance* h, int64_t* out);
 int omc_last_shor_subspace_stats(omc_instance* h, int64_t* out);
 int omc_tuning_set(omc_instance* h, const char* name, const char* value);
diff --git a/optimalmatrixcompletion.jl_amd/_lib.py b/optimalmatrixcompletion.jl_amd/_lib.py
--- a/optimalmatrixcompletion.jl_amd/_lib.py
+++ b/optimalmatrixcompletion.jl_amd/_lib.py
@@ -91,6 +91,8 @@
     if hasattr(lib, "omc_kernel_residency"):
         lib.omc_kernel_residency.argtypes = [vp, vp]
     lib.omc_last_subspace_stats.argtypes = [vp, vp]
+    if hasattr(lib, "omc_cone_sub_plan"):
+        lib.omc_cone_sub_plan.argtypes = [vp, vp]
     lib.omc_set_node_rho_scales.argtypes = [vp, C.c_int, vp]
     lib.omc_debug_stamps.argtypes = [vp, vp]
     lib.omc_left_singular_batch.argtypes = [vp, C.c_int, vp, vp]
diff --git a/optimalmatrixcompletion.jl_amd/api.py b/optimalmatrixcompletion.jl_amd/api.py
--- a/optimalmatrixcompletion.jl_amd/api.py
+++ b/optimalmatrixcompletion.jl_amd/api.py
@@ -440,6 +440,11 @@
         out = np.zeros(len(RESIDENCY_KERNELS), np.int32)
         _lib.check(self._lib.omc_kernel_residency(self._h, _lib.ptr(out)))
         return {nm: int(v) for nm, v in zip(RESIDENCY_KERNELS, out)}
+
+    def cone_sub_plan(self):
+        out = np.zeros(4, np.int64)
+        _lib.check(self._lib.omc_cone_sub_plan(self._h, _lib.ptr(out)))
+        return dict(mlds=bool(out[0]), lds_bytes=int(out[1]), shor_mlds=None if out[2] < 0 else bool(out[2]), shor_lds_bytes=int(out[3]))
 
     def solver_info(self):
         info = np.zeros(8)
diff --git a/optimalmatrixcompletion.jl_amd/csrc/omc_api.cpp b/optimalmatrixcompletion.jl_amd/csrc/omc_api.cpp
--- a/optimalmatrixcompletion.jl_amd/csrc/omc_api.cpp
+++ b/optimalmatrixcompletion.jl_amd/csrc/omc_api.cpp
@@ -558,6 +558,7 @@
   BIND(h->brcoef, w.rcoef, sN * Rmax * k); BIND(h->brrhs, w.rrhs, sN * Rmax); BIND(h->bcutx, w.cutx, sN * w.Lmax * n);
   if ((rc_ = put_descriptors(w, pk, B, sN, 0, L, cut_x, h->stream))) return rc_;
   w.geo = omc_plan_geometry(n, w.np16, k, rmax, Rmax, h->cmax, h->tun.global_nolds, h->tun.cone_multi_min, h->tun.plain_multi_min);
+  if (!h->tun.sub_mlds) geom_set_sub(w.geo, n, w.np16, 0);
   BIND(h->bmwstat, w.mw_stat, sB * 4, s0);
   w.mw_budget = MAX_SWEEPS; w.ev_out = nullptr;
   w.pmw_stat = nullptr;
@@ -893,6 +894,15 @@
   return 0;
 }
 
+int omc_cone_sub_plan(omc_instance* h, int64_t* out) {
+  if (!h || !out) return fail(OMC_ERR_ARGUMENT, "NULL argument");
+  if (!h->ws.geo.sub_lds) return fail(OMC_ERR_ARGUMENT, "omc_cone_sub_plan: nothing staged yet (the geometry is planned by omc_relax_stage)");
+  const bool big = h->shor_on && h->wbig.sub_enable;
+  out[0] = h->ws.geo.sub_mlds; out[1] = (int64_t)h->ws.geo.sub_lds;
+  out[2] = big ? h->wbig.geo.sub_mlds : -1; out[3] = big ? (int64_t)h->wbig.geo.sub_lds : 0;
+  return 0;
+}
+
 int omc_kernel_residency(omc_instance* h, int* out) {
   if (!h || !out) return fail(OMC_ERR_ARGUMENT, "NULL argument");
   if (!h->ws.geo.sub_lds) return fail(OMC_ERR_ARGUMENT, "omc_kernel_residency: nothing staged yet (the geometry is planned by omc_relax_stage)");
diff --git a/optimalmatrixcompletion.jl_amd/csrc/omc_api_shor.cpp b/optimalmatrixcompletion.jl_amd/csrc/omc_api_shor.cpp
--- a/optimalmatrixcompletion.jl_amd/csrc/omc_api_shor.cpp
+++ b/optimalmatrixcompletion.jl_amd/csrc/omc_api_shor.cpp
@@ -632,6 +632,7 @@
   wb.n = N; wb.np16 = NPb; wb.Mbuf = sh.MbufB; wb.Vrow = sh.VrowB; wb.vvalid = sh.vvalidB; wb.fro2 = sh.fro2B; wb.W1 = sh.P0;
   wb.sub_enable = 0; wb.cert_enable = 0; wb.ws_mode = 0; wb.clip_hi = 1e300; wb.sub_debug = 0; wb.ws_first = nullptr; wb.ws_need = nullptr; wb.ws_phase = 0;
   wb.geo = omc_plan_geometry(N, NPb, wb.k, wb.rmax, wb.Rmax, h->cmax, h->tun.global_nolds, h->tun.cone_multi_min, MW_MAX_ORDER + 1);
+  if (!h->tun.sub_mlds) geom_set_sub(wb.geo, N, NPb, 0);
   BIND(h->sbigmw, wb.mw_stat, sB * 4, s);
   if (wb.geo.ws.slab_stride) BIND(h->sbigscr, wb.cone_scratch, sB * wb.geo.ws.slab_stride);
   wb.trM = sh.trB;
diff --git a/optimalmatrixcompletion.jl_amd/csrc/omc_device.hip b/optimalmatrixcompletion.jl_amd/csrc/omc_device.hip
--- a/optimalmatrixcompletion.jl_amd/csrc/omc_device.hip
+++ b/optimalmatrixcompletion.jl_amd/csrc/omc_device.hip
@@ -1111,8 +1111,9 @@
 }
 
 
-template <int MODE>
+template <int MODE, bool MLDS = false>
 __global__ void __launch_bounds__(256, 2) k_cone_sub(OmcWS w) {
+  static_assert(!MLDS || MODE != 1, "mode 1 runs only where Z is in the global slab: no room for the triangle");
   extern __shared__ double smem[];
   __shared__ int s_flag, s_nsel, s_cond;
   __shared__ double s_shift, s_cs[SUBP];
@@ -1132,7 +1133,7 @@
       if (!w.sub_onC[b]) { if (threadIdx.x == 0) w.confirm[b] = 1; return; }
     }
   }
-  const SubLayout L = sub_layout(w.np16);
+  const SubLayout L = sub_layout(w.n, w.np16, MLDS ? 1 : 0);
   const int n = w.n, NP = w.np16, nt = NP >> 4, LD = L.LD;
   const int wv = tid >> 6, lane = tid & 63, li = lane & 15, lk = lane >> 4;
   double* Xa = smem;
@@ -1145,13 +1146,92 @@
   constexpr double sgn = (MODE == 1) ? -1.0 : 1.0;
   const double fro2 = (MODE == 1) ? w.fro2c[b] : w.fro2[b], nF = sqrt(fro2), trM = (MODE == 1) ? -w.trMc[b] : w.trM[b];
   const double tol_eff = (MODE == 2) ? 1e-11 : (MODE == 1) ? 1e-9 : fmin(1e-6, fmax(w.sub_tol, w.sub_adapt * w.rd[b] / fmax(nF, 1e-300)));
-  for (int e = tid; e < SUBP * NP; e += T) { const int j = e / NP, r = e - j * NP; Xa[(size_t)j * LD + r] = Xg[e]; }
+  const bool prof = (w.sub_debug == 2) && b == 0;
+  long long tprev = prof ? __builtin_amdgcn_s_memtime() : 0;
+#define SUBSTAMP(slot) do { if (prof) { __syncthreads(); if (tid == 0) { const long long t_ = __builtin_amdgcn_s_memtime(); w.stamps[slot] += (double)(t_ - tprev); tprev = t_; } } } while (0)
+  [[maybe_unused]] double* Mt = Xa + L.Mt;
+  if constexpr (MLDS) {
+    constexpr int MT_P = 13, MT_X = 7;
+    const int npair = (n + 1) >> 1;
+    double xv[MT_X];
+#pragma unroll
+    for (int u = 0; u < MT_X; ++u) { const int e = tid + u * T; xv[u] = Xg[e < SUBP * NP ? e : 0]; }
+    for (int p0 = wv; p0 < npair; p0 += 4 * MT_P) {
+      double v[2 * MT_P]; int at[2 * MT_P];
+#pragma unroll
+      for (int u = 0; u < MT_P; ++u) {
+        const int j = p0 + 4 * u, j2 = n - 1 - j, len = n - j;
+        const bool pv = j < npair;
+#pragma unroll
+        for (int h = 0; h < 2; ++h) {
+          const int e = lane + 64 * h, e2 = e - len;
+          const bool first = e < len, ok = pv && (first || (e2 <= j && j2 != j));
+          const int col = first ? j : j2, row = first ? j + e : j2 + e2;
+          at[2 * u + h] = ok ? ((row * (row + 1)) >> 1) + col : -1;
+          v[2 * u + h] = Mb[ok ? (unsigned)col * (unsigned)NP + (unsigned)row : 0u];
+        }
+      }
+#pragma unroll
+      for (int u = 0; u < 2 * MT_P; ++u) if (at[u] >= 0) Mt[at[u]] = v[u];
+    }
+#pragma unroll
+    for (int u = 0; u < MT_X; ++u) { const int e = tid + u * T, j = e / NP, r = e - j * NP; if (e < SUBP * NP) Xa[(size_t)j * LD + r] = xv[u]; }
+  } else {
+    for (int e = tid; e < SUBP * NP; e += T) { const int j = e / NP, r = e - j * NP; Xa[(size_t)j * LD + r] = Xg[e]; }
+  }
   if (tid < SUBP) th[tid] = thg[tid];
   __syncthreads();
+  SUBSTAMP(15);
 
   auto mul_MX = [&](double shift, bool back, bool scaled) {
     const double* Xi = Xa + (back ? L.Za : 0);
     double* Zo = back ? Xa : Za;
+    if constexpr (MLDS) {
+      for (int tb = 0; tb < nt; tb += 8) {
+        const int b0 = tb + wv;
+        if (b0 >= nt) break;
+        const bool v1 = b0 + 4 < nt;
+        const int t0 = b0, t1 = v1 ? b0 + 4 : b0;
+        double4v acc0 = {0.0, 0.0, 0.0, 0.0}, acc1 = acc0;
+        const int m0 = (t0 << 4) + li, m1 = (t1 << 4) + li, c0 = m0 < n ? m0 : n - 1, c1 = m1 < n ? m1 : n - 1;
+        const bool r0 = m0 < n, r1 = m1 < n;
+        const int rb0 = (c0 * (c0 + 1)) >> 1, rb1 = (c1 * (c1 + 1)) >> 1;
+        const double* Xb = Xi + (size_t)li * LD;
+        double a0[4], a1[4], bv[4];
+        auto fetch = [&](int k0) {
+#pragma unroll
+          for (int u = 0; u < 4; ++u) {
+            const int kk = k0 + 4 * u + lk, kc = kk < n ? kk : n - 1, kb = (kc * (kc + 1)) >> 1;
+            a0[u] = Mt[kc <= c0 ? rb0 + kc : kb + c0]; a1[u] = Mt[kc <= c1 ? rb1 + kc : kb + c1]; bv[u] = Xb[kk];
+          }
+        };
+        fetch(0);
+        for (int k0 = 0; k0 < NP; k0 += 16) {
+          double x0[4], x1[4], xb[4];
+#pragma unroll
+          for (int u = 0; u < 4; ++u) {
+            const bool vk = k0 + 4 * u + lk < n;
+            x0[u] = sgn * ((r0 && vk) ? a0[u] : 0.0); x1[u] = sgn * ((r1 && vk) ? a1[u] : 0.0); xb[u] = bv[u];
+          }
+          fetch(k0 + 16 < NP ? k0 + 16 : 0);
+          __builtin_amdgcn_sched_barrier(0);
+#pragma unroll
+          for (int u = 0; u < 4; ++u) {
+            acc0 = __builtin_amdgcn_mfma_f64_16x16x4f64(x0[u], xb[u], acc0, 0, 0, 0);
+            acc1 = __builtin_amdgcn_mfma_f64_16x16x4f64(x1[u], xb[u], acc1, 0, 0, 0);
+          }
+        }
+        const double cs = scaled ? s_cs[li] : 1.0;
+#pragma unroll
+        for (int r = 0; r < 4; ++r) {
+          const size_t a = (size_t)li * LD + lk + 4 * r;
+          const double z0 = acc0[r] + shift * Xi[a + (t0 << 4)];
+          Zo[a + (t0 << 4)] = scaled ? cs * z0 : z0;
+          if (v1) { const double z1 = acc1[r] + shift * Xi[a + (t1 << 4)]; Zo[a + (t1 << 4)] = scaled ? cs * z1 : z1; }
+        }
+      }
+      return;
+    }
     for (int tb = 0; tb < nt; tb += 12) {
       const int b0 = tb + wv;
       if (b0 >= nt) break;
@@ -1204,9 +1284,6 @@
 
   int steps = 0, ok = 0, fail = 0, nrr = 0;
   const int qmax = (MODE == 2) ? 4 * w.sub_qmax : w.sub_qmax, chunk = w.sub_chunk;
-  const bool prof = (w.sub_debug == 2) && b == 0;
-  long long tprev = prof ? __builtin_amdgcn_s_memtime() : 0;
-#define SUBSTAMP(slot) do { if (prof) { __syncthreads(); if (tid == 0) { const long long t_ = __builtin_amdgcn_s_memtime(); w.stamps[slot] += (double)(t_ - tprev); tprev = t_; } } } while (0)
   SUBSTAMP(0);
   bool skip_steps = (MODE == 2);
   while (true) {
@@ -3060,14 +3137,16 @@
   }
 }
 void omc_launch_cone_sub(const OmcWS* w, hipStream_t s) {
-  hipLaunchKernelGGL(k_cone_sub<0>, dim3(w->nB), dim3(256), w->geo.sub_lds, s, *w);
+  if (w->geo.sub_mlds) hipLaunchKernelGGL((k_cone_sub<0, true>), dim3(w->nB), dim3(256), w->geo.sub_lds, s, *w);
+  else hipLaunchKernelGGL((k_cone_sub<0, false>), dim3(w->nB), dim3(256), w->geo.sub_lds, s, *w);
 }
 void omc_launch_sep_sub(const OmcWS* w, hipStream_t s) {
   hipLaunchKernelGGL(k_sep_prepare, dim3(w->B), dim3(256), 0, s, *w);
-  hipLaunchKernelGGL(k_cone_sub<2>, dim3(w->B), dim3(256), w->geo.sub_lds, s, *w);
+  if (w->geo.sub_mlds) hipLaunchKernelGGL((k_cone_sub<2, true>), dim3(w->B), dim3(256), w->geo.sub_lds, s, *w);
+  else hipLaunchKernelGGL((k_cone_sub<2, false>), dim3(w->B), dim3(256), w->geo.sub_lds, s, *w);
 }
 void omc_launch_cert_sub(const OmcWS* w, hipStream_t s) {
-  hipLaunchKernelGGL(k_cone_sub<1>, dim3(w->B), dim3(256), w->geo.sub_lds, s, *w);
+  hipLaunchKernelGGL((k_cone_sub<1, false>), dim3(w->B), dim3(256), w->geo.sub_lds_glob, s, *w);
 }
 void omc_launch_small(const OmcWS* w, int mode, hipStream_t s) {
   if (w->geo.small.use_lds) hipLaunchKernelGGL(k_small<true>, dim3(w->nB), dim3(256), w->geo.small.lds_bytes, s, *w, mode);
@@ -3106,9 +3185,11 @@
   hipError_t e2 = hipFuncSetAttribute((const void*)k_global<true>, hipFuncAttributeMaxDynamicSharedMemorySize, OMC_MAX_DYN_LDS - 8 * 1024);
   hipError_t e3 = hipFuncSetAttribute((const void*)k_colprox, hipFuncAttributeMaxDynamicSharedMemorySize, OMC_MAX_DYN_LDS);
   hipError_t e4 = hipFuncSetAttribute((const void*)k_small<true>, hipFuncAttributeMaxDynamicSharedMemorySize, OMC_MAX_DYN_LDS);
-  (void)hipFuncSetAttribute((const void*)k_cone_sub<0>, hipFuncAttributeMaxDynamicSharedMemorySize, OMC_MAX_DYN_LDS);
-  (void)hipFuncSetAttribute((const void*)k_cone_sub<1>, hipFuncAttributeMaxDynamicSharedMemorySize, OMC_MAX_DYN_LDS);
-  (void)hipFuncSetAttribute((const void*)k_cone_sub<2>, hipFuncAttributeMaxDynamicSharedMemorySize, OMC_MAX_DYN_LDS);
+  (void)hipFuncSetAttribute((const void*)k_cone_sub<0, false>, hipFuncAttributeMaxDynamicSharedMemorySize, OMC_MAX_DYN_LDS);
+  (void)hipFuncSetAttribute((const void*)k_cone_sub<1, false>, hipFuncAttributeMaxDynamicSharedMemorySize, OMC_MAX_DYN_LDS);
+  (void)hipFuncSetAttribute((const void*)k_cone_sub<2, false>, hipFuncAttributeMaxDynamicSharedMemorySize, OMC_MAX_DYN_LDS);
+  (void)hipFuncSetAttribute((const void*)k_cone_sub<0, true>, hipFuncAttributeMaxDynamicSharedMemorySize, SUB_MLDS_BUDGET);
+  (void)hipFuncSetAttribute((const void*)k_cone_sub<2, true>, hipFuncAttributeMaxDynamicSharedMemorySize, SUB_MLDS_BUDGET);
 #define WS_ATTR(L, R) (void)hipFuncSetAttribute((const void*)k_cone_ws<L, true, R>, hipFuncAttributeMaxDynamicSharedMemorySize, OMC_MAX_DYN_LDS)
 #define WS_ATTR_ALL(L) WS_ATTR(L, 0); WS_ATTR(L, 4); WS_ATTR(L, 5); WS_ATTR(L, 6); WS_ATTR(L, 7); WS_ATTR(L, 8)
   WS_ATTR_ALL(4); WS_ATTR_ALL(8); WS_ATTR_ALL(16);
@@ -3121,9 +3202,9 @@
 }
 void omc_query_residency(const OmcWS* w, int* out) {
   const OmcGeom& g = w->geo;
-  out[OMC_RES_CONE_SUB] = residency_of((const void*)k_cone_sub<0>, 256, g.sub_lds);
-  out[OMC_RES_CONE_SUB_CERT] = residency_of((const void*)k_cone_sub<1>, 256, g.sub_lds);
-  out[OMC_RES_CONE_SUB_SEP] = residency_of((const void*)k_cone_sub<2>, 256, g.sub_lds);
+  out[OMC_RES_CONE_SUB] = g.sub_mlds ? residency_of((const void*)k_cone_sub<0, true>, 256, g.sub_lds) : residency_of((const void*)k_cone_sub<0, false>, 256, g.sub_lds);
+  out[OMC_RES_CONE_SUB_CERT] = residency_of((const void*)k_cone_sub<1, false>, 256, g.sub_lds_glob);
+  out[OMC_RES_CONE_SUB_SEP] = g.sub_mlds ? residency_of((const void*)k_cone_sub<2, true>, 256, g.sub_lds) : residency_of((const void*)k_cone_sub<2, false>, 256, g.sub_lds);
   out[OMC_RES_GLOBAL] = g.glob.use_lds ? residency_of((const void*)k_global<true>, 512, g.glob.lds_bytes) : residency_of((const void*)k_global<false>, 512, 0);
   out[OMC_RES_SMALL] = g.small.use_lds ? residency_of((const void*)k_small<true>, 256, g.small.lds_bytes) : residency_of((const void*)k_small<false>, 256, 0);
   omc_colprox_sweep_residency(w, &out[OMC_RES_COLPROX_PAIR], &out[OMC_RES_COLPROX_WIDE]);
diff --git a/optimalmatrixcompletion.jl_amd/csrc/omc_host.h b/optimalmatrixcompletion.jl_amd/csrc/omc_host.h
--- a/optimalmatrixcompletion.jl_amd/csrc/omc_host.h
+++ b/optimalmatrixcompletion.jl_amd/csrc/omc_host.h
@@ -121,6 +121,7 @@
   int shor_select_kb = 1048576;
   int streams = 4;
   int sub_debug = 0;
+  int sub_mlds = 1;
   int sub_qmax = 24;
   int timing_stride = 1;
   int ws_quiet = 1;
@@ -144,7 +145,7 @@
   {"OMC_WS_QUIET", nullptr, &Tuning::ws_quiet},
   {"OMC_STREAMS", nullptr, &Tuning::streams},                {"OMC_PLAIN_MULTI_MIN", nullptr, &Tuning::plain_multi_min},
   {"OMC_SUB_DEBUG", nullptr, &Tuning::sub_debug},            {"OMC_SUB_QMAX", nullptr, &Tuning::sub_qmax},
-  {"OMC_SMALL_CHAIN", nullptr, &Tuning::small_chain},
+  {"OMC_SMALL_CHAIN", nullptr, &Tuning::small_chain},        {"OMC_SUB_MLDS", nullptr, &Tuning::sub_mlds},
   {"OMC_TIMING_STRIDE", nullptr, &Tuning::timing_stride},
 };
 
diff --git a/optimalmatrixcompletion.jl_amd/csrc/omc_layout.h b/optimalmatrixcompletion.jl_amd/csrc/omc_layout.h
--- a/optimalmatrixcompletion.jl_amd/csrc/omc_layout.h
+++ b/optimalmatrixcompletion.jl_amd/csrc/omc_layout.h
@@ -55,10 +55,15 @@
   return {ld, Ncp, Ncp / MW_B, ev, ev + Ncp, ev + 2 * (size_t)Ncp, sel, smax, head, (head + 4) * 8, ev + 2 * (size_t)Ncp};
 }
 OMC_HD int mw_plain_launches(const MwLayout& L, int sweeps) { return sweeps * (L.nb - 1) + 4; }
-struct SubLayout { int LD, zglob; size_t Za, Cs, Hs, Gj, th, evj, red, wgt, sel, bytes; };
-OMC_HD SubLayout sub_layout(int np16) {
-  const int LD = np16 + 2, zglob = np16 > 512; const size_t blk = (size_t)SUBP * LD, Cs = (zglob ? 1 : 2) * blk, th = Cs + 4 * 256 + 2 * 16 * 17;
-  return {LD, zglob, blk, Cs, Cs + 4 * 256, Cs + 4 * 256 + 16 * 17, th, th + 16, th + 32, th + 64, th + 80, (th + 80 + 8) * 8};
+#define SUB_STATIC_LDS 512
+#define SUB_MLDS_BUDGET (80 * 1024)
+struct SubLayout { int LD, zglob, mlds; size_t Za, Cs, Hs, Gj, th, evj, red, wgt, sel, Mt, bytes; };
+OMC_HD SubLayout sub_layout(int n, int np16, int want) {
+  const int LD = np16 + 2, zglob = np16 > 512; const size_t blk = (size_t)SUBP * LD, Cs = (zglob ? 1 : 2) * blk, tri = (size_t)n * (n + 1) / 2;
+  const size_t thm = Cs + 4 * 256 + 16 * 17;
+  const int mlds = want && !zglob && (thm + 80 + 8 + tri) * 8 + SUB_STATIC_LDS <= SUB_MLDS_BUDGET;
+  const size_t th = mlds ? thm : thm + 16 * 17, Mt = th + 80 + 8;
+  return {LD, zglob, mlds, blk, Cs, Cs + 4 * 256, mlds ? Cs : Cs + 4 * 256 + 16 * 17, th, th + 16, th + 32, th + 64, th + 80, Mt, (Mt + (mlds ? tri : 0)) * 8};
 }
 #define SMALL_STATIC_LDS 1024
 #define SMALL_CS 512
@@ -126,6 +131,7 @@
   size_t cpb_lds_bytes, cpb_slab_lds_bytes, cpb_slab_stride;
   int cp_lds_c, cp_lds_doubles, cp_keepB;
   size_t cp_scratch_stride, sub_lds;
+  int sub_mlds; size_t sub_lds_glob;
   int mw; MwLayout mwl;
   int plain_mw;
 };
@@ -144,6 +150,10 @@
   g.cpb_slab_lds_bytes = cs > 0 ? cp_block_layout(cs, 0).doubles * 8 : 0;
   g.cpb_slab_stride = cs > 0 ? cp_block_layout(cs, 0).slab : 0;
 }
+OMC_HD void geom_set_sub(OmcGeom& g, int n, int np16, int want) {
+  const SubLayout L = sub_layout(n, np16, want);
+  g.sub_lds = L.bytes; g.sub_mlds = L.mlds; g.sub_lds_glob = sub_layout(n, np16, 0).bytes;
+}
 OMC_HD bool mw_order_ok(int n, int use_lds, int knob) { return n >= MW_MIN_ORDER && !use_lds && n >= knob && n <= MW_MAX_ORDER; }
 OMC_HD OmcGeom omc_plan_geometry(int n, int np16, int k, int rmax, int Rmax, int cmax, int global_nolds, int cone_multi_min, int plain_multi_min) {
   OmcGeom g;
@@ -152,7 +162,7 @@
   g.ws = plan_block(wg.bytes, wg.use_lds != 0);
   g.ws_lpp = wg.lpp; g.ws_rpl2 = wg.rpl >> 1; g.ws_ld = wg.ld;
   g.cone.slab_stride = g.ws.slab_stride = g.cone.slab_stride > g.ws.slab_stride ? g.cone.slab_stride : g.ws.slab_stride;
-  g.sub_lds = sub_layout(np16).bytes;
+  geom_set_sub(g, n, np16, 1);
   const size_t gb = glob_layout(n, k, rmax, Rmax).bytes, sb = small_layout(n, rmax, k).bytes;
   g.glob = plan_block(gb, gb + GLOB_STATIC_LDS <= OMC_MAX_DYN_LDS && !global_nolds);
   g.small = plan_block(sb, sb + SMALL_STATIC_LDS <= OMC_MAX_DYN_LDS);
```

Result: no change. 2641, median of 2 (+0.9%).
